# ruotianluo/ImageCaptioning.pytorch

Hardware: NVIDIA H100
Metric: captions/sec at beam=5 seq_len=20 (higher is better)
Workload: dtype f32 (fp32-grade: split-fp16 x3 tensor-core passes, fp32 accumulate)

## Files before the change

imagecaptioning.pytorch_b200/csrc/aoa_engine.cu:

```cuda
#include <vector>

#include "../../include/capb200.h"
#include "common.cuh"
#include "engine_common.cuh"
#include "kernels.cuh"
#include "train_common.cuh"

using namespace capb200;

namespace capb200 {
__global__ void capb_add_vec_kernel(const float* a, const float* b, float* o, int n) {
    const int i = blockIdx.x * blockDim.x + threadIdx.x;
    if (i < n) o[i] = a[i] + b[i];
}
__global__ void capb_interleave_gates_kernel(const float* src, float* dst, int H) {
    const int i = blockIdx.x * blockDim.x + threadIdx.x;
    if (i < 4 * H) dst[i] = src[(i & 3) * H + (i >> 2)];
}
}

struct capb200_aoa_engine {
    capb200_aoa_cfg cfg{};
    capb200_aoa_weights w{};
    int V1 = 0, E = 0, H = 0, heads = 0, dk = 0, F = 0, T = 0, mode = 0;
// ... 377 lines not shown
    {
        const long ldE = round_up(E, 8);
        char* tmp = nullptr;
        const size_t tmp_bytes = (size_t)V1 * ldE * (sizeof(float) + (e->tc ? 2 * sizeof(__half) : 0)) + 1024;
        CAPB_CHECK_CUDA(cudaMallocAsync(&tmp, tmp_bytes, st));
        CAPB_CHECK_CUDA(cudaMemsetAsync(tmp, 0, tmp_bytes, st));
        ActView ev;
        ev.ld = ldE;
        ev.f = reinterpret_cast<float*>(tmp);
        if (e->tc) { ev.hi = reinterpret_cast<__half*>(tmp + (size_t)V1 * ldE * sizeof(float)); ev.lo = ev.hi + (size_t)V1 * ldE; }
        int rc = 0;
        if (ldE == E) rc = relu_copy_launch(w->embed, (long)V1 * E, ev, st);
        else {
            for (int v = 0; v < V1 && !rc; ++v) {
                ActView rv = ev;
                rv.f += (long)v * ldE; if (rv.hi) { rv.hi += (long)v * ldE; rv.lo += (long)v * ldE; }
                rc = relu_copy_launch(w->embed + (long)v * E, E, rv, st);
            }
        }
        GemmProblem g;
        g.M = V1; g.N = 4 * H; g.nseg = 1;
        g.seg[0] = seg_of(ev, w->att_lstm_w_ih, E + H, e->p_ih_x, E);
        g.epi.C = e->xgate; g.epi.ldc = e->ld_xgate;
        if (!rc) {
            if (!e->tc) rc = gemm_simt_launch(g, st);
            else {
                GemmTcPlan* plan = gemm_tc_plan_create(g, e->mode == CAPB200_MODE_TC_F16X3 ? 3 : 1);
                rc = plan ? gemm_tc_plan_launch(plan, nullptr, 0, st) : 1;
                if (plan) gemm_tc_plan_destroy(plan);
            }
        }
        e->launches += 2;
        cudaFreeAsync(tmp, st);
        if (rc) return 1;
    }
    if (e->tc && !e->bound) {
        CAPB_CHECK_CUDA(cudaStreamSynchronize(st));
        CAPB_CHECK_RANGE();
    }
    e->bound = true;
    return 0;
}

int capb200_aoa_decode_beam(capb200_aoa_engine* e, const float* att, const float* mask, int B, int R, const capb200_beam_opts* opts, long long* seq,
                            float* seq_logprobs, long long* done_seq, int* done_len, float* done_p, float* done_raw, void* stream) {
    if (check_ready(e)) return 1;
    cudaStream_t st = static_cast<cudaStream_t>(stream);
    CAPB_REQUIRE(opts != nullptr && att != nullptr && seq != nullptr && B >= 1 && R >= 1, "bad argument");
    const int beam = opts->beam_size, keep = opts->sample_n;
    CAPB_REQUIRE(beam >= 1 && beam <= 16 && beam <= e->V1, "beam_size must be in 1..16 and <= V+1");
    CAPB_REQUIRE(keep == 1 || keep == beam, "sample_n must be 1 or beam_size (AttModel.py:223)");
    if (aoa_decode_workspace(e, B, B * beam, R, beam, st)) return 1;
    if (aoa_decode_prepare(e, att, mask, B, R, st)) return 1;
    auto core = [&](int nrows, int live, const int* tokens, const int* src_row, int , float* logits, long ld) {
        return aoa_decode_core(e, nrows, live, tokens, src_row, logits, ld, R, mask, st);
    };
    return beam_decode_driver(e->d, e->V1, e->T, B, beam, keep, opts->penalty_kind, opts->penalty_alpha, seq, seq_logprobs, done_seq, done_len, done_p,
                              done_raw, core, &e->launches, st, loop_graph_key(e->ws, e->wblock, mask, R, 9), to_edits(opts->edits), opts->temperature);
}

int capb200_aoa_decode_beam_diverse(capb200_aoa_engine* e, const float* att, const float* mask, int B, int R, const capb200_diverse_opts* opts,
                                    long long* seq, float* seq_logprobs, long long* done_seq, int* done_len, float* done_p, float* done_raw, void* stream) {
    if (check_ready(e)) return 1;
    cudaStream_t st = static_cast<cudaStream_t>(stream);
    CAPB_REQUIRE(opts != nullptr && att != nullptr && seq != nullptr && B >= 1 && R >= 1, "bad argument");
    if (opts->group_size == 1) return capb200_aoa_decode_beam(e, att, mask, B, R, &opts->base, seq, seq_logprobs, done_seq, done_len, done_p, done_raw, stream);
    const int beam = opts->base.beam_size;
    CAPB_REQUIRE(beam >= 2 && beam <= 16 && beam <= e->V1, "beam_size must be in 2..16 and <= V+1");
    if (aoa_decode_workspace(e, B, B * beam, R, beam, st)) return 1;
    if (aoa_decode_prepare(e, att, mask, B, R, st)) return 1;
    auto core = [&](int nrows, int rpi, const int* tokens, const int* src_row, int , float* logits, long ld) {
        return aoa_decode_core(e, nrows, rpi, tokens, src_row, logits, ld, R, mask, st);
    };
    return diverse_beam_decode_driver(e->d, e->V1, e->T, B, beam, opts->group_size, opts->diversity_lambda, opts->base.sample_n, opts->base.penalty_kind,
                                      opts->base.penalty_alpha, seq, seq_logprobs, done_seq, done_len, done_p, done_raw, core, &e->launches, st,
                                      loop_graph_key(e->ws, e->wblock, mask, R, 9), to_edits(opts->base.edits), opts->base.temperature);
}

int capb200_aoa_beam_record_logprobs(capb200_aoa_engine* e, int image, int rank, float* dst, void* stream) {
    if (check_ready(e)) return 1;
    return beam_record_logprobs(e->d, e->V1, e->T, image, rank, dst, static_cast<cudaStream_t>(stream));
}

int capb200_aoa_decode_sample(capb200_aoa_engine* e, const float* att, const float* mask, int B, int R, const capb200_sample_opts* opts,
                              const long long* tokens_in, long ld_tok, long long* seq, float* seq_logprobs, float* picked, void* stream) {
    if (check_ready(e)) return 1;
    cudaStream_t st = static_cast<cudaStream_t>(stream);
    CAPB_REQUIRE(opts != nullptr && att != nullptr && seq_logprobs != nullptr && B >= 1 && R >= 1, "bad argument");
    const int n = opts->sample_n, method = opts->method;
    CAPB_REQUIRE(n >= 1 && method >= 0 && method <= 5, "bad sampling options");
    if (method == CAPB200_SAMPLE_FORCED || method == CAPB200_SAMPLE_TEACHER) CAPB_REQUIRE(tokens_in != nullptr && ld_tok >= 1, "token matrix required");
    if (method != CAPB200_SAMPLE_TEACHER) CAPB_REQUIRE(seq != nullptr, "seq output required");
    if (method == CAPB200_SAMPLE_MULTINOMIAL) CAPB_REQUIRE(opts->temperature > 0.f, "temperature must be positive");
    const int rows = B * n;
    const int steps = (method == CAPB200_SAMPLE_TEACHER) ? opts->steps : e->T;
    const long t_out = (method == CAPB200_SAMPLE_TEACHER) ? ld_tok : e->T;
    CAPB_REQUIRE(steps >= 0 && steps <= t_out, "steps out of range");
    if (aoa_decode_workspace(e, B, rows, R, 1, st)) return 1;
    if (aoa_decode_prepare(e, att, mask, B, R, st)) return 1;
    auto core = [&](int nrows, int , const int* tokens, const int* src_row, int , float* logits, long ld) {
        return aoa_decode_core(e, nrows, n, tokens, src_row, logits, ld, R, mask, st);
    };
    return sample_decode_driver(e->d, e->V1, e->T, rows, method, opts->temperature, opts->seed, steps, tokens_in, ld_tok, seq, seq_logprobs, picked,
                                core, &e->launches, st, to_edits(opts->edits), opts->top);
}

}
// ... 252 lines not shown
```

imagecaptioning.pytorch_b200/csrc/beam.cu:

```cuda
#include "common.cuh"
#include "kernels.cuh"

namespace capb200 {

namespace {

constexpr int MAXB = 16;

__device__ __forceinline__ double apply_penalty(int kind, float alpha, int length, double p) {
    if (kind == 1) return p / (pow(5.0 + length, (double)alpha) / pow(6.0, (double)alpha));
    if (kind == 2) return p / (double)length;
    return p;
}

__device__ __forceinline__ void select_step(const BeamState& s, int img, int t, int live, int kl, int row0, int hist0, const float* __restrict__ top_val,
                                            const int* __restrict__ top_idx, const int* pen, int n_pen, float lambda, int penalty_kind,
                                            float penalty_alpha, double* __restrict__ done_p) {
    const int lane = threadIdx.x;
    const int b = s.beam, T = s.T;
    const int ncand = live * kl;
    float cv[8];
    int cf[8];
#pragma unroll
    for (int u = 0; u < 8; ++u) {
        const int c = lane + 32 * u;
        cv[u] = -INFINITY;
        cf[u] = 0x7fffffff;
        if (c < ncand) {
            const int pb = c / kl, k = c % kl;
            const long row = (long)row0 + pb;
            const int w = top_idx[row * kl + k];
            float v = top_val[row * kl + k];
            int cnt = 0;
            for (int q = 0; q < n_pen; ++q) cnt += (pen[q] == w);
            if (cnt) v = __fsub_rn(v, __fmul_rn((float)cnt, lambda));
            cv[u] = s.sums[(long)img * b + pb] + v;
            cf[u] = pb * s.V1 + w;
        }
    }
    const int* seq_old = (t & 1) ? s.seq_b : s.seq_a;
    int* seq_new = (t & 1) ? s.seq_a : s.seq_b;
    const int* hist_old = (t & 1) ? s.hist_b : s.hist_a;
    int* hist_new = (t & 1) ? s.hist_a : s.hist_b;

    float my_v = -INFINITY;
    int my_f = 0;
    for (int j = 0; j < b; ++j) {
        float bv = -INFINITY;
        int bf = 0x7fffffff, bu = -1;
#pragma unroll
        for (int u = 0; u < 8; ++u)
            if (cv[u] > bv || (cv[u] == bv && cf[u] < bf)) { bv = cv[u]; bf = cf[u]; bu = u; }
        float wv = bv;
        int wf = bf;
// ... 6 lines not shown
        if (bu >= 0 && bf == wf && bv == wv) {
#pragma unroll
            for (int u = 0; u < 8; ++u) if (u == bu) { cv[u] = -INFINITY; cf[u] = 0x7fffffff; }
        }
        if (lane == j) { my_v = wv; my_f = wf; }
    }
    __shared__ int sh_parent[MAXB], sh_word[MAXB], sh_slot[MAXB];
    const bool has = lane < b;
    const int parent = has ? my_f / s.V1 : 0;
    const int word = has ? my_f % s.V1 : 0;
    const bool ended = has && ((word == 0) || (t == T - 1));
    const unsigned em = __ballot_sync(0xffffffffu, ended);
    const int cnt0 = s.done_cnt[img];
    const int slot = cnt0 + __popc(em & ((1u << lane) - 1u));
    if (has) { sh_parent[lane] = parent; sh_word[lane] = word; sh_slot[lane] = ended ? slot : -1; }
    __syncwarp();
    for (int idx = lane; idx < b * t; idx += 32) {
        const int j = idx / t, q = idx - j * t;
        const long dst = ((long)img * b + j) * T, src = ((long)img * b + sh_parent[j]) * T;
        seq_new[dst + q] = seq_old[src + q];
        hist_new[dst + q] = hist_old[src + q];
    }
    if (em != 0u) {
        for (int idx = lane; idx < b * (t + 1); idx += 32) {
            const int j = idx / (t + 1), q = idx - j * (t + 1);
            if (sh_slot[j] < 0) continue;
            const long rec = ((long)img * b * T + sh_slot[j]) * T, src = ((long)img * b + sh_parent[j]) * T;
            s.done_seq[rec + q] = (q < t) ? seq_old[src + q] : sh_word[j];
            s.done_hist[rec + q] = (q < t) ? hist_old[src + q] : hist0 + sh_parent[j];
        }
    }
    if (has) {
        const long dst = ((long)img * b + lane) * T;
        seq_new[dst + t] = word;
        hist_new[dst + t] = hist0 + parent;
        float new_sum = my_v;
        if (ended) {
            const long rec = (long)img * b * T + slot;
            s.done_len[rec] = t + 1;
            s.done_raw[rec] = new_sum;
            done_p[rec] = apply_penalty(penalty_kind, penalty_alpha, t + 1, (double)new_sum);
            new_sum -= 1000.0f;
        }
        s.sums[(long)img * b + lane] = new_sum;
        s.tokens[(long)img * b + lane] = word;
        s.src_row[(long)img * b + lane] = row0 + parent;
    }
    if (lane == 0 && em != 0u) s.done_cnt[img] = cnt0 + __popc(em);
}

__global__ void __launch_bounds__(32) beam_step_kernel(BeamState s, int t, int live, const float* __restrict__ top_val,
                                                       const int* __restrict__ top_idx, int penalty_kind, float penalty_alpha,
                                                       double* __restrict__ done_p) {
    const int img = blockIdx.x;
    select_step(s, img, t, live, s.beam, img * live, img * live, top_val, top_idx, nullptr, 0, 0.f, penalty_kind, penalty_alpha, done_p);
}

__global__ void __launch_bounds__(32) diverse_beam_step_kernel(BeamState s, int G, int t, int k, const float* __restrict__ top_val,
                                                               const int* __restrict__ top_idx, float lambda, int rows_total, int penalty_kind,
                                                               float penalty_alpha, double* __restrict__ done_p) {
    const int i = blockIdx.x, lane = threadIdx.x;
    const int b = s.beam, T = s.T;
    __shared__ int sh_pen[MAXB];
    for (int g = 0; g < G && g <= t; ++g) {
        const int lt = t - g;
        if (lt >= T) continue;
        const int n_pen = g * b;
        __syncwarp();
        if (lane < n_pen) {
            const int pg = lane / b, j = lane - pg * b;
            const int last = min(t - pg, T - 1);
            const int* seq_pg = (last & 1) ? s.seq_a : s.seq_b;
            sh_pen[lane] = seq_pg[((long)(i * G + pg) * b + j) * T + lt];
        }
        __syncwarp();
        const int vimg = i * G + g;
        select_step(s, vimg, lt, lt == 0 ? 1 : b, k, vimg * b, g * rows_total + vimg * b, top_val, top_idx, sh_pen, n_pen, lambda, penalty_kind,
                    penalty_alpha, done_p);
    }
}

__global__ void __launch_bounds__(32) beam_finalize_kernel(BeamState s, int keep, const double* __restrict__ done_p, long long* __restrict__ out_seq,
                                                           int* __restrict__ out_len, float* __restrict__ out_p, float* __restrict__ out_raw,
                                                           int* __restrict__ out_hist) {
    const int img = blockIdx.x, lane = threadIdx.x;
    const int b = s.beam, T = s.T;
    const int cnt = s.done_cnt[img];
    const long base = (long)img * b * T;
    __shared__ unsigned char taken[MAXB * 64];
    for (int i = lane; i < cnt; i += 32) taken[i] = 0;
    __syncwarp();
    for (int k = 0; k < keep; ++k) {
        double bv = -INFINITY;
        int bi = 0x7fffffff;
        for (int i = lane; i < cnt; i += 32) {
            if (!taken[i]) {
                const double v = done_p[base + i];
                if (v > bv || (v == bv && i < bi)) { bv = v; bi = i; }
            }
        }
#pragma unroll
        for (int o = 16; o > 0; o >>= 1) {
            const double ov = __shfl_xor_sync(0xffffffffu, bv, o);
            const int oi = __shfl_xor_sync(0xffffffffu, bi, o);
            if (ov > bv || (ov == bv && oi < bi)) { bv = ov; bi = oi; }
        }
// ... 93 lines not shown
        if (vec4) {
            const float4* s4 = reinterpret_cast<const float4*>(src);
            float4* d4 = reinterpret_cast<float4*>(d);
            for (int v = threadIdx.x; v < V1 / 4; v += blockDim.x) {
                const float4 x = __ldg(s4 + v);
                float4 o;
                o.x = (x.x - mx) - lsum; o.y = (x.y - mx) - lsum; o.z = (x.z - mx) - lsum; o.w = (x.w - mx) - lsum;
                if (twice) { o.x = (o.x - m2) - l2; o.y = (o.y - m2) - l2; o.z = (o.z - m2) - l2; o.w = (o.w - m2) - l2; }
                d4[v] = o;
            }
        } else {
            for (int v = threadIdx.x; v < V1; v += blockDim.x) {
                const float lp = (src[v] - mx) - lsum;
                d[v] = twice ? (lp - m2) - l2 : lp;
            }
        }
        apply_edits();
        return;
    }
    const bool vec = ((V1 & 3) == 0) && ((ld_slab & 3) == 0) && ((step_stride & 3) == 0) && ((reinterpret_cast<uintptr_t>(slab) & 15) == 0) &&
                     ((reinterpret_cast<uintptr_t>(dst) & 15) == 0);
    if (vec) {
        const float4* s4 = reinterpret_cast<const float4*>(src);
        float4* d4 = reinterpret_cast<float4*>(d);
        for (int v = threadIdx.x; v < V1 / 4; v += blockDim.x) d4[v] = __ldg(s4 + v);
    } else {
        for (int v = threadIdx.x; v < V1; v += blockDim.x) d[v] = src[v];
    }
    apply_edits();
}

}

int beam_edit_launch(int rows, int k_in, int beam, int t, const DecodeEdits& ed, const int* prev_tokens, const float* val_in, const int* idx_in,
                     float* val_out, int* idx_out, cudaStream_t stream, int first_beam, int first_group_rows, int first_group) {
    CAPB_REQUIRE(k_in >= beam && k_in <= MAXB, "beam_size + number of active decode edits must be <= 16");
    if (rows <= 0) return 0;
    beam_edit_kernel<<<cdiv(rows, 128), 128, 0, stream>>>(rows, k_in, beam, t, ed, prev_tokens, val_in, idx_in, val_out, idx_out, first_beam,
                                                          first_group_rows, first_group);
    CAPB_CHECK_CUDA(cudaGetLastError());
    return 0;
}

int scale_rows_launch(float* x, long ld, int rows, int cols, float factor, cudaStream_t stream, int skip_beam, int skip_group_rows, int skip_group) {
    if (rows <= 0 || cols <= 0) return 0;
    long blocks = ((long)rows * cols + 255) / 256;
    if (blocks > sm_count() * 16) blocks = sm_count() * 16;
    scale_rows_kernel<<<(int)blocks, 256, 0, stream>>>(x, ld, rows, cols, factor, skip_beam, skip_group_rows, skip_group);
    CAPB_CHECK_CUDA(cudaGetLastError());
    return 0;
}

int beam_step_launch(const BeamState& s, int t, int live, const float* top_val, const int* top_idx, int penalty_kind, float penalty_alpha,
                     cudaStream_t stream) {
    CAPB_REQUIRE(s.beam >= 1 && s.beam <= MAXB, "beam size 1..16");
    CAPB_REQUIRE(s.beam * s.T <= MAXB * 64, "beam*T record capacity");
    beam_step_kernel<<<s.B, 32, 0, stream>>>(s, t, live, top_val, top_idx, penalty_kind, penalty_alpha, s.done_p);
    CAPB_CHECK_CUDA(cudaGetLastError());
    return 0;
}

int diverse_beam_step_launch(const BeamState& s, int G, int t, int k, const float* top_val, const int* top_idx, float lambda, int rows_total,
                             int penalty_kind, float penalty_alpha, cudaStream_t stream) {
    CAPB_REQUIRE(G >= 2 && s.beam >= 1 && G * s.beam <= MAXB, "group_size * beams per group must be in 2..16");
    CAPB_REQUIRE(k >= s.beam && k <= MAXB && s.beam * k <= 256, "candidate list width");
    CAPB_REQUIRE(s.beam * s.T <= MAXB * 64, "beam*T record capacity");
    CAPB_REQUIRE(lambda >= 0.f, "diversity_lambda must be >= 0 (the candidate lists rely on the penalty only lowering values)");
    diverse_beam_step_kernel<<<s.B / G, 32, 0, stream>>>(s, G, t, k, top_val, top_idx, lambda, rows_total, penalty_kind, penalty_alpha, s.done_p);
    CAPB_CHECK_CUDA(cudaGetLastError());
    return 0;
}

int beam_finalize_launch(const BeamState& s, int keep, long long* out_seq, int* out_len, float* out_p, float* out_raw, int* out_hist,
                         cudaStream_t stream) {
    CAPB_REQUIRE(keep >= 1 && keep <= s.beam, "keep must be in 1..beam");
    beam_finalize_kernel<<<s.B, 32, 0, stream>>>(s, keep, s.done_p, out_seq, out_len, out_p, out_raw, out_hist);
    CAPB_CHECK_CUDA(cudaGetLastError());
    return 0;
}

int gather_logprob_rows_launch(const float* slab, long step_stride, long ld_slab, const int* hist, int nseq, int T, int V1, float* dst,
                               const float2* stats, long stats_stride, cudaStream_t stream, const long long* seqs, const DecodeEdits* ed) {
    if (nseq <= 0) return 0;
    gather_rows_kernel<<<nseq * T, 256, 0, stream>>>(slab, step_stride, ld_slab, hist, T, V1, dst, stats, stats_stride, seqs, ed ? *ed : DecodeEdits());
    CAPB_CHECK_CUDA(cudaGetLastError());
    return 0;
}

}
```

imagecaptioning.pytorch_b200/csrc/common.cuh:

```cuda
#pragma once
#include <atomic>
#include <cstdint>
#include <cstdio>
#include <cstring>
#include <string>
#include <cuda.h>
#include <cuda_fp16.h>
#include <cuda_runtime.h>

namespace capb200 {

void set_error(const std::string& msg);
#define CAPB_CHECK_CUDA(expr)                                                                          \
    do {                                                                                               \
        cudaError_t _e = (expr);                                                                       \
        if (_e != cudaSuccess) {                                                                       \
            capb200::set_error(std::string(#expr) + " failed: " + cudaGetErrorString(_e) + " at " +    \
                               __FILE__ + ":" + std::to_string(__LINE__));                            \
            return 1;                                                                                  \
        }                                                                                              \
    } while (0)
#define CAPB_REQUIRE(cond, msg)                                                                        \
    do {                                                                                               \
        if (!(cond)) {                                                                                 \
            capb200::set_error(std::string("requirement failed: ") + #cond + " -- " + (msg));          \
            return 1;                                                                                  \
        }                                                                                              \
    } while (0)

inline int cdiv(int a, int b) { return (a + b - 1) / b; }
inline long round_up(long a, long b) { return (a + b - 1) / b * b; }

inline bool first_use_on_device(std::atomic<unsigned long long>& mask) {
    int dev = 0;
    if (cudaGetDevice(&dev) != cudaSuccess || dev < 0 || dev > 63) return true;
    const unsigned long long bit = 1ull << dev;
    return (mask.fetch_or(bit) & bit) == 0;
}

inline int sm_count() {
    static std::atomic<int> cache[64];
    int dev = 0;
    if (cudaGetDevice(&dev) != cudaSuccess || dev < 0 || dev > 63) dev = 0;
    int n = cache[dev].load();
    if (n == 0) {
        if (cudaDeviceGetAttribute(&n, cudaDevAttrMultiProcessorCount, dev) != cudaSuccess || n < 1) n = 132;
        cache[dev].store(n);
    }
    return n;
}

__device__ __forceinline__ void split_f32(float x, __half& hi, __half& lo) {
    hi = __float2half_rn(x);
    lo = __float2half_rn(x - __half2float(hi));
}

constexpr int kMaxSeg = 3;
struct GemmSeg {
    const float* A = nullptr;
    long lda = 0;
    const float* W = nullptr;
    long ldw = 0;
    const __half* A_hi = nullptr;
    const __half* A_lo = nullptr;
    long lda_h = 0;
    const __half* W_hi = nullptr;
    const __half* W_lo = nullptr;
    long ldw_h = 0;
    int K = 0;
};
struct GemmEpilogue {
    const float* bias = nullptr;
    const float* row_bias = nullptr;
    long ld_row_bias = 0;
    int rows_per_group = 1;
    const float* residual = nullptr;
    long ld_res = 0;
    int relu = 0;
    float* C = nullptr;
    long ldc = 0;
    __half* C_hi = nullptr;
    __half* C_lo = nullptr;
    long ldcs = 0;
    int lstm = 0;
    int H = 0;
    const float* c_prev = nullptr;
    long ld_cprev = 0;
    const int* src_row = nullptr;
    float* c_out = nullptr;
    long ld_cout = 0;
    const float* gather_bias = nullptr;
    long ld_gb = 0;
    const int* gather_idx = nullptr;
    float* h_f = nullptr;
    __half* h_hi = nullptr;
    __half* h_lo = nullptr;
    long ld_h = 0;
    unsigned long long* trace = nullptr;
};

__device__ __forceinline__ float fast_sigmoid(float x) { return __fdividef(1.0f, 1.0f + __expf(-x)); }
__device__ __forceinline__ float fast_tanh(float x) {
    const float e = __expf(2.0f * x);
    return 1.0f - __fdividef(2.0f, 1.0f + e);
}
__device__ __forceinline__ void fast_tanh4(const float (&x)[4], float (&t)[4]) {
    float y[4];
#pragma unroll
    for (int i = 0; i < 4; ++i) y[i] = 1.0f + __expf(fminf(2.0f * x[i], 20.0f));
    const float p01 = y[0] * y[1], p23 = y[2] * y[3];
    const float r = __fdividef(1.0f, p01 * p23);
    const float r01 = r * p23, r23 = r * p01;
    t[0] = fmaf(-2.0f, r01 * y[1], 1.0f);
    t[1] = fmaf(-2.0f, r01 * y[0], 1.0f);
    t[2] = fmaf(-2.0f, r23 * y[3], 1.0f);
    t[3] = fmaf(-2.0f, r23 * y[2], 1.0f);
}
struct GemmProblem {
    int M = 0, N = 0, nseg = 0;
    GemmSeg seg[kMaxSeg];
    GemmEpilogue epi;
};

enum NumericMode : int {
    kModeSimtFp32 = 0,
    kModeTcF16x3 = 1,
    kModeTcF16x1 = 2,
};

int gemm_simt_launch(const GemmProblem& p, cudaStream_t stream);

struct GemmTcPlan;
GemmTcPlan* gemm_tc_plan_create(const GemmProblem& p, int passes);
int gemm_tc_tile_n(int M, int N);
int gemm_tc_tile_m(int M, int N, int bn);
void gemm_tc_plan_destroy(GemmTcPlan* plan);
int gemm_tc_plan_launch(GemmTcPlan* plan, const GemmEpilogue* epi_override, int M_override, cudaStream_t stream);
bool gemm_tc_supported(const GemmProblem& p, std::string* why);

int split_planes_launch(const float* x, long ldx, int rows, int cols, __half* hi, __half* lo, long ldh, cudaStream_t stream);
int* range_flag_ptr();
int range_flag_read(int reset);
#define CAPB_CHECK_RANGE()                                                                                              \
    do {                                                                                                                \
        if (capb200::range_flag_read(0)) {                                                                              \
            capb200::set_error("a value with |x| >= 65504 (or inf/nan) reached a split-fp16 conversion in an earlier call: results of the "   \
                               "tensor-core modes are invalid for such inputs/weights (DESIGN.md section 3); capb200_range_status(1) clears the flag"); \
            return 1;                                                                                                   \
        }                                                                                                               \
    } while (0)
int split_planes_interleave_launch(const float* x, long ldx, int H, int cols, __half* hi, __half* lo, long ldh, cudaStream_t stream);

}
```

imagecaptioning.pytorch_b200/csrc/engine.cu:

```cuda
#include <map>
#include <mutex>
#include <vector>

#include "../../include/capb200.h"
#include "common.cuh"
#include "kernels.cuh"
#include "engine_common.cuh"
#include "train_common.cuh"

namespace capb200 {

static thread_local std::string g_last_error;
void set_error(const std::string& msg) { g_last_error = msg; }
const char* last_error_cstr() { return g_last_error.c_str(); }

__global__ void capb_fill_int_kernel(int* p, int n, int v) {
    const int i = blockIdx.x * blockDim.x + threadIdx.x;
    if (i < n) p[i] = v;
}
__global__ void capb_load_token_column_kernel(const long long* src, long ld, int col, int n, int* dst) {
    const int i = blockIdx.x * blockDim.x + threadIdx.x;
    if (i < n) dst[i] = (int)src[(long)i * ld + col];
}
__global__ void capb_store_token_column_kernel(const int* src, int n, long long* dst, long ld, int col) {
// ... 159 lines not shown
    const bool attn = attends(e);
    const bool tc = e->tc;
    if (tc) {
        e->in_fc = carve_planes(a, B, e->cfg.fc_feat_size);
        if (attn) e->in_att = carve_planes(a, (long)B * R, e->cfg.att_feat_size);
    }
    e->fc_e.carve(a, B, updown ? H : E, tc);
    if (attn) {
        e->att_e.carve(a, (long)B * R, H, tc);
        e->p_att.carve(a, (long)B * R, A, false);
        e->att_res.carve(a, rows, H, tc);
        e->att_h.carve(a, rows, A, false);
    }
    if (updown) {
        e->g_fc.carve(a, B, 4 * H, false);
        e->h1_in.carve(a, rows, H, tc);
        e->h1_out.carve(a, rows, H, tc);
    }
    e->xt.carve(a, rows, E, tc);
    e->h0_in.carve(a, rows, H, tc);
    e->h0_out.carve(a, rows, H, tc);
    e->gates.carve(a, rows, 5 * H, false);
    e->ld_c = round_up(H, 8);
    for (int i = 0; i < 2; ++i) {
        e->c0[i] = a.take<float>((long)rows * e->ld_c);
        e->c1[i] = a.take<float>((long)rows * e->ld_c);
    }
    e->img_of_row = a.take<int>(rows);
    e->att_score = a.take<float>((long)rows * (R > 0 ? R : 1));
    e->d.carve(a, B, rows, beam, T);
}

int ensure_workspace(capb200_engine* e, int B, int rows, int R, int beam, cudaStream_t st) {
    if (B <= e->capB && rows <= e->capRows && R <= e->capR && beam <= e->capBeam && e->ws != nullptr) return 0;
    const int nB = B > e->capB ? B : e->capB, nRows = rows > e->capRows ? rows : e->capRows;
    const int nR = R > e->capR ? R : e->capR, nBeam = beam > e->capBeam ? beam : e->capBeam;
    Arena dry;
    layout_workspace(e, dry, nB, nRows, nR, nBeam);
    const size_t need = dry.off + 256;
    CAPB_CHECK_CUDA(cudaStreamSynchronize(st));
    destroy_plans(e);
    if (e->ws) CAPB_CHECK_CUDA(cudaFree(e->ws));
    e->ws = nullptr;
    CAPB_CHECK_CUDA(cudaMalloc(&e->ws, need));
    e->ws_bytes = need;
    Arena real;
    real.base = e->ws;
    layout_workspace(e, real, nB, nRows, nR, nBeam);
    e->capB = nB; e->capRows = nRows; e->capR = nR; e->capBeam = nBeam;
    CAPB_CHECK_CUDA(cudaMemsetAsync(e->ws, 0, need, st));
    return fill_int_launch(e->d.neg1, nRows, -1, st);
}

int run_gemm_inner(capb200_engine* e, int id, GemmProblem& g, int plan_rows, cudaStream_t st) {
    e->launches++;
    if (!e->tc) return gemm_simt_launch(g, st);
    if (e->plans[id] == nullptr) {
        GemmProblem planned = g;
        planned.M = plan_rows;
        e->plans[id] = gemm_tc_plan_create(planned, e->mode == CAPB200_MODE_TC_F16X3 ? 3 : 1);
        if (e->plans[id] == nullptr) return 1;
    }
    return gemm_tc_plan_launch(e->plans[id], &g.epi, g.M, st);
}

int run_gemm(capb200_engine* e, int id, GemmProblem& g, int plan_rows, cudaStream_t st) {
    if (!e->profiling) return run_gemm_inner(e, id, g, plan_rows, st);
    if (e->ev_used + 2 > e->ev_pool.size()) {
        for (int i = 0; i < 64; ++i) {
            cudaEvent_t ev;
            CAPB_CHECK_CUDA(cudaEventCreate(&ev));
            e->ev_pool.push_back(ev);
        }
    }
    double k_total = 0;
    for (int s = 0; s < g.nseg; ++s) k_total += g.seg[s].K;
    CAPB_CHECK_CUDA(cudaEventRecord(e->ev_pool[e->ev_used], st));
    const int rc = run_gemm_inner(e, id, g, plan_rows, st);
    CAPB_CHECK_CUDA(cudaEventRecord(e->ev_pool[e->ev_used + 1], st));
    e->ev_used += 2;
    e->ev_ids.push_back(id);
    e->ev_flops.push_back(2.0 * g.M * g.N * k_total);
    return rc;
}

int prepare(capb200_engine* e, const float* fc, const float* att, const float* mask, int B, int R, cudaStream_t st) {
    CAPB_NVTX("capb200 prepare_feature (fc_embed, att_embed, ctx2att)");
    const int H = e->H, E = e->E, A = e->A;
    const bool updown = e->cfg.family == CAPB200_FAMILY_UPDOWN;
    const capb200_weights& w = e->w;
    ActView fc_in;  fc_in.f = const_cast<float*>(fc);  fc_in.ld = e->cfg.fc_feat_size;
    if (e->tc && e->cfg.family != CAPB200_FAMILY_ATT2IN2) {
        e->launches++;
        if (split_planes_launch(fc, e->cfg.fc_feat_size, B, e->cfg.fc_feat_size, e->in_fc.hi, e->in_fc.lo, e->in_fc.ld, st)) return 1;
    }
    if (e->cfg.family != CAPB200_FAMILY_ATT2IN2) {
        GemmProblem g;
        g.M = B; g.N = updown ? H : E; g.nseg = 1;
        g.seg[0] = seg_of(fc_in, w.fc_embed_w, e->cfg.fc_feat_size, e->p_fc, e->cfg.fc_feat_size);
        g.seg[0].A_hi = e->in_fc.hi; g.seg[0].A_lo = e->in_fc.lo; g.seg[0].lda_h = e->in_fc.ld;
        g.epi.bias = w.fc_embed_b; g.epi.relu = updown ? 1 : 0;
        g.epi.C = e->fc_e.v.f; g.epi.ldc = e->fc_e.v.ld; g.epi.C_hi = e->fc_e.v.hi; g.epi.C_lo = e->fc_e.v.lo; g.epi.ldcs = e->fc_e.v.ld;
        if (run_gemm(e, G_FC, g, e->capB, st)) return 1;
    }
    if (!attends(e)) return 0;
    ActView att_in; att_in.f = const_cast<float*>(att); att_in.ld = e->cfg.att_feat_size;
    if (e->tc) {
        e->launches++;
        if (split_planes_launch(att, e->cfg.att_feat_size, B * R, e->cfg.att_feat_size, e->in_att.hi, e->in_att.lo, e->in_att.ld, st)) return 1;
    }
    {
        GemmProblem g;
        g.M = B * R; g.N = H; g.nseg = 1;
        g.seg[0] = seg_of(att_in, w.att_embed_w, e->cfg.att_feat_size, e->p_attw, e->cfg.att_feat_size);
        g.seg[0].A_hi = e->in_att.hi; g.seg[0].A_lo = e->in_att.lo; g.seg[0].lda_h = e->in_att.ld;
        g.epi.bias = w.att_embed_b; g.epi.relu = 1;
        g.epi.C = e->att_e.v.f; g.epi.ldc = e->att_e.v.ld; g.epi.C_hi = e->att_e.v.hi; g.epi.C_lo = e->att_e.v.lo; g.epi.ldcs = e->att_e.v.ld;
        if (run_gemm(e, G_ATT, g, e->capB * e->capR, st)) return 1;
    }
    if (mask != nullptr) {
        e->launches++;
        if (mask_rows_launch(e->att_e.v, B, R, H, mask, R, st)) return 1;
    }
    {
        GemmProblem g;
        g.M = B * R; g.N = A; g.nseg = 1;
        g.seg[0] = seg_of(e->att_e.v, w.ctx2att_w, H, e->p_ctx, H);
        g.epi.bias = w.ctx2att_b;
        g.epi.C = e->p_att.v.f; g.epi.ldc = e->p_att.v.ld;
        if (run_gemm(e, G_CTX, g, e->capB * e->capR, st)) return 1;
    }
    if (!updown) return 0;
    {
        GemmProblem g;
        g.M = B; g.N = 4 * H; g.nseg = 1;
        g.seg[0] = seg_of(e->fc_e.v, w.att_lstm_w_ih + H, E + 2 * H, e->p_a_ih_fc, H);
        g.epi.bias = e->tc ? e->bsum_att_il : e->bsum_att;
        g.epi.C = e->g_fc.v.f; g.epi.ldc = e->g_fc.v.ld;
        if (run_gemm(e, G_GFC, g, e->capB, st)) return 1;
    }
    return 0;
}

int core_step(capb200_engine* e, int rows, int rpi, const int* tokens, const int* src_row, float* logits, long ld_logits, int n_images, int R,
              const float* mask, cudaStream_t st) {
    const int H = e->H, E = e->E, A = e->A, V1 = e->V1;
    const capb200_weights& w = e->w;
    if (e->cfg.family == CAPB200_FAMILY_UPDOWN) {
        StateCopy s0, s1;
        s0.src = e->h0_out.v.f; s0.ld_src = e->h0_out.v.ld; s0.dst = e->h0_in.v;
        s1.src = e->h1_out.v.f; s1.ld_src = e->h1_out.v.ld; s1.dst = e->h1_in.v;
        const bool xg = e->use_xgate;
        e->launches++;
        if (state_gather_embed_launch(rows, tokens, src_row, w.embed, E, xg ? 0 : E, 1, e->xt.v, H, 2, s0, s1, st)) return 1;
        const int cur = e->core_cur, nxt = cur ^ 1;
        {
            GemmProblem g;
            g.M = rows; g.N = 4 * H;
            g.seg[0] = seg_of(e->h1_in.v, w.att_lstm_w_ih, E + 2 * H, e->p_a_ih_h, H);
            g.seg[1] = seg_of(e->h0_in.v, w.att_lstm_w_hh, H, e->p_a_hh, H);
            g.nseg = 2;
            if (!xg) { g.seg[2] = seg_of(e->xt.v, w.att_lstm_w_ih + 2 * H, E + 2 * H, e->p_a_ih_x, E); g.nseg = 3; }
            g.epi.row_bias = e->g_fc.v.f; g.epi.ld_row_bias = e->g_fc.v.ld; g.epi.rows_per_group = rpi;
            if (e->tc) {
                g.epi.lstm = 1; g.epi.H = H;
                g.epi.c_prev = e->c0[cur]; g.epi.ld_cprev = e->ld_c; g.epi.src_row = src_row;
                g.epi.c_out = e->c0[nxt]; g.epi.ld_cout = e->ld_c;
                g.epi.gather_bias = xg ? e->xgate : nullptr; g.epi.ld_gb = e->ld_xgate; g.epi.gather_idx = tokens;
                g.epi.h_f = e->h0_out.v.f; g.epi.h_hi = e->h0_out.v.hi; g.epi.h_lo = e->h0_out.v.lo; g.epi.ld_h = e->h0_out.v.ld;
            } else {
                g.epi.C = e->gates.v.f; g.epi.ldc = e->gates.v.ld;
            }
            if (run_gemm(e, G_LSTM1, g, e->capRows, st)) return 1;
        }
        if (!e->tc) {
            e->launches++;
            if (lstm_pointwise_launch(rows, H, e->gates.v.f, e->gates.v.ld, src_row, e->c0[cur], e->ld_c, e->c0[nxt], e->ld_c, e->h0_out.v,
                                      xg ? e->xgate : nullptr, e->ld_xgate, tokens, st)) return 1;
        }
        {
            GemmProblem g;
            g.M = rows; g.N = A; g.nseg = 1;
            g.seg[0] = seg_of(e->h0_out.v, w.h2att_w, H, e->p_h2att, H);
            g.epi.bias = w.h2att_b;
            g.epi.C = e->att_h.v.f; g.epi.ldc = e->att_h.v.ld;
            if (run_gemm(e, G_H2ATT, g, e->capRows, st)) return 1;
        }
        const bool split = e->split_lang && e->tc && e->side != nullptr;
        if (split) {
            CAPB_CHECK_CUDA(cudaEventRecord(e->ev_fork, st));
            CAPB_CHECK_CUDA(cudaStreamWaitEvent(e->side, e->ev_fork, 0));
            GemmProblem g;
            g.M = rows; g.N = 4 * H; g.nseg = 2;
            g.seg[0] = seg_of(e->h0_out.v, w.lang_lstm_w_ih + H, 2 * H, e->p_l_ih_h, H);
            g.seg[1] = seg_of(e->h1_in.v, w.lang_lstm_w_hh, H, e->p_l_hh, H);
            g.epi.bias = e->bsum_lang_il;
            g.epi.C = e->gates.v.f; g.epi.ldc = e->gates.v.ld;
            if (run_gemm(e, G_LSTM2A, g, e->capRows, e->side)) return 1;
            CAPB_CHECK_CUDA(cudaEventRecord(e->ev_join, e->side));
        }
        e->launches += 2;
        if (additive_attention_launch(n_images, rpi, R, A, H, e->att_h.v.f, e->att_h.v.ld, e->p_att.v.f, e->p_att.v.ld, e->att_e.v.f, e->att_e.v.ld,
                                      mask, R, w.alpha_w, w.alpha_b, e->att_score, e->att_res.v, st)) return 1;
        if (split) {
            CAPB_CHECK_CUDA(cudaStreamWaitEvent(st, e->ev_join, 0));
            GemmProblem g;
            g.M = rows; g.N = 4 * H; g.nseg = 1;
            g.seg[0] = seg_of(e->att_res.v, w.lang_lstm_w_ih, 2 * H, e->p_l_ih_a, H);
            g.epi.residual = e->gates.v.f; g.epi.ld_res = e->gates.v.ld;
            g.epi.lstm = 1; g.epi.H = H;
            g.epi.c_prev = e->c1[cur]; g.epi.ld_cprev = e->ld_c; g.epi.src_row = src_row;
            g.epi.c_out = e->c1[nxt]; g.epi.ld_cout = e->ld_c;
            g.epi.h_f = e->h1_out.v.f; g.epi.h_hi = e->h1_out.v.hi; g.epi.h_lo = e->h1_out.v.lo; g.epi.ld_h = e->h1_out.v.ld;
            if (run_gemm(e, G_LSTM2B, g, e->capRows, st)) return 1;
        } else {
            GemmProblem g;
            g.M = rows; g.N = 4 * H; g.nseg = 3;
            g.seg[0] = seg_of(e->att_res.v, w.lang_lstm_w_ih, 2 * H, e->p_l_ih_a, H);
            g.seg[1] = seg_of(e->h0_out.v, w.lang_lstm_w_ih + H, 2 * H, e->p_l_ih_h, H);
            g.seg[2] = seg_of(e->h1_in.v, w.lang_lstm_w_hh, H, e->p_l_hh, H);
            if (e->tc) {
                g.epi.bias = e->bsum_lang_il;
                g.epi.lstm = 1; g.epi.H = H;
                g.epi.c_prev = e->c1[cur]; g.epi.ld_cprev = e->ld_c; g.epi.src_row = src_row;
                g.epi.c_out = e->c1[nxt]; g.epi.ld_cout = e->ld_c;
                g.epi.h_f = e->h1_out.v.f; g.epi.h_hi = e->h1_out.v.hi; g.epi.h_lo = e->h1_out.v.lo; g.epi.ld_h = e->h1_out.v.ld;
            } else {
                g.epi.bias = e->bsum_lang;
                g.epi.C = e->gates.v.f; g.epi.ldc = e->gates.v.ld;
            }
            if (run_gemm(e, G_LSTM2, g, e->capRows, st)) return 1;
        }
        if (!e->tc) {
            e->launches++;
            if (lstm_pointwise_launch(rows, H, e->gates.v.f, e->gates.v.ld, src_row, e->c1[cur], e->ld_c, e->c1[nxt], e->ld_c, e->h1_out.v,
                                      nullptr, 0, nullptr, st)) return 1;
        }
        e->core_cur = nxt;
        {
            GemmProblem g;
            g.M = rows; g.N = V1; g.nseg = 1;
            g.seg[0] = seg_of(e->h1_out.v, w.logit_w, H, e->p_logit, H);
            g.epi.bias = w.logit_b;
            g.epi.C = logits; g.epi.ldc = ld_logits;
            if (run_gemm(e, G_LOGIT, g, e->capRows, st)) return 1;
        }
        return 0;
    }
    if (e->cfg.family == CAPB200_FAMILY_ATT2IN2) {
        StateCopy s0, s1;
        s0.src = e->h0_out.v.f; s0.ld_src = e->h0_out.v.ld; s0.dst = e->h0_in.v;
        e->launches++;
        if (state_gather_embed_launch(rows, tokens, src_row, w.embed, E, E, 1, e->xt.v, H, 1, s0, s1, st)) return 1;
        const int cur = e->core_cur, nxt = cur ^ 1;
        {
            GemmProblem g;
            g.M = rows; g.N = A; g.nseg = 1;
            g.seg[0] = seg_of(e->h0_in.v, w.h2att_w, H, e->p_h2att, H);
            g.epi.bias = w.h2att_b;
            g.epi.C = e->att_h.v.f; g.epi.ldc = e->att_h.v.ld;
            if (run_gemm(e, G_H2ATT, g, e->capRows, st)) return 1;
        }
        e->launches += 2;
        if (additive_attention_launch(n_images, rpi, R, A, H, e->att_h.v.f, e->att_h.v.ld, e->p_att.v.f, e->p_att.v.ld, e->att_e.v.f, e->att_e.v.ld,
                                      mask, R, w.alpha_w, w.alpha_b, e->att_score, e->att_res.v, st)) return 1;
        {
            GemmProblem g;
            g.M = rows; g.N = 5 * H; g.nseg = 2;
            g.seg[0] = seg_of(e->xt.v, w.i2h_w, E, e->p_i2h, E);
            g.seg[1] = seg_of(e->h0_in.v, w.h2h_w, H, e->p_h2h, H);
            g.epi.bias = e->bsum_core;
            g.epi.C = e->gates.v.f; g.epi.ldc = e->gates.v.ld;
            if (run_gemm(e, G_CORE, g, e->capRows, st)) return 1;
        }
        {
            GemmProblem g;
            g.M = rows; g.N = 2 * H; g.nseg = 1;
            g.seg[0] = seg_of(e->att_res.v, w.a2c_w, H, e->p_a2c, H);
            g.epi.residual = e->gates.v.f + 3 * H; g.epi.ld_res = e->gates.v.ld;
            g.epi.C = e->gates.v.f + 3 * H; g.epi.ldc = e->gates.v.ld;
            if (run_gemm(e, G_A2C, g, e->capRows, st)) return 1;
        }
        e->launches++;
        if (maxout_pointwise_launch(rows, H, e->gates.v.f, e->gates.v.ld, src_row, e->c0[cur], e->ld_c, e->c0[nxt], e->ld_c, e->h0_out.v, st)) return 1;
        e->core_cur = nxt;
        GemmProblem g;
        g.M = rows; g.N = V1; g.nseg = 1;
        g.seg[0] = seg_of(e->h0_out.v, w.logit_w, H, e->p_logit, H);
        g.epi.bias = w.logit_b;
        g.epi.C = logits; g.epi.ldc = ld_logits;
        return run_gemm(e, G_LOGIT, g, e->capRows, st);
    }
    const bool fresh = (src_row == e->d.neg1);
    for (int pass = fresh ? 0 : 1; pass < 2; ++pass) {
        StateCopy s0, s1;
        s0.src = e->h0_out.v.f; s0.ld_src = e->h0_out.v.ld; s0.dst = e->h0_in.v;
        const int* srcs = (pass == 0) ? e->d.neg1 : (fresh ? nullptr : src_row);
        e->launches++;
// ... 8 lines not shown
        g.seg[0] = seg_of(e->xt.v, w.i2h_w, E, e->p_i2h, E);
        g.seg[1] = seg_of(e->h0_in.v, w.h2h_w, H, e->p_h2h, H);
        g.epi.bias = e->bsum_core;
        g.epi.C = e->gates.v.f; g.epi.ldc = e->gates.v.ld;
        if (run_gemm(e, G_CORE, g, e->capRows, st)) return 1;
        e->launches++;
        if (maxout_pointwise_launch(rows, H, e->gates.v.f, e->gates.v.ld, srcs, e->c0[cur], e->ld_c, e->c0[nxt], e->ld_c, e->h0_out.v, st)) return 1;
        e->core_cur = nxt;
    }
    GemmProblem g;
    g.M = rows; g.N = V1; g.nseg = 1;
    g.seg[0] = seg_of(e->h0_out.v, w.logit_w, H, e->p_logit, H);
    g.epi.bias = w.logit_b;
    g.epi.C = logits; g.epi.ldc = ld_logits;
    return run_gemm(e, G_LOGIT, g, e->capRows, st);
}

int check_ready(capb200_engine* e) {
    CAPB_REQUIRE(e != nullptr, "null engine");
    CAPB_REQUIRE(e->bound, "capb200_engine_bind_weights has not been called");
    CAPB_CHECK_RANGE();
    return 0;
}

}

namespace capb200 {

int lstm_member_info(capb200_engine* e, MemberInfo* m) {
    if (check_ready(e)) return 1;
    m->family = e->cfg.family;
    m->V1 = e->V1; m->T = e->T;
    m->attends = attends(e);
    m->graph_ok = !e->profiling;
    m->ws = e->ws; m->wblock = e->wblock;
    m->fresh = e->d.neg1;
    m->launches = &e->launches;
    return 0;
}

int lstm_decode_workspace(capb200_engine* e, int B, int rows, int R, int beam, int rows_per_image, cudaStream_t st) {
    if (ensure_workspace(e, B, rows, R, beam, st)) return 1;
    if (!attends(e)) { iota_div_kernel<<<cdiv(rows, 256), 256, 0, st>>>(e->img_of_row, rows, rows_per_image); e->launches++; }
    return 0;
}

int lstm_decode_prepare(capb200_engine* e, const float* fc, const float* att, const float* mask, int B, int R, cudaStream_t st) {
    if (prepare(e, fc, att, mask, B, R, st)) return 1;
    e->core_cur = 0;
    return 0;
}

int lstm_decode_core(capb200_engine* e, int rows, int rpi, const int* tokens, const int* src_row, float* logits, long ld, int B, int R,
                     const float* mask, cudaStream_t st) {
    return core_step(e, rows, rpi, tokens, src_row, logits, ld, B, R, mask, st);
}

}

extern "C" {

const char* capb200_last_error(void) { return g_last_error.c_str(); }
int capb200_abi_version(void) { return CAPB200_ABI_VERSION; }
int capb200_range_status(int reset) { return range_flag_read(reset); }

capb200_engine* capb200_engine_create(const capb200_model_cfg* cfg) {
    if (cfg == nullptr) { set_error("null cfg"); return nullptr; }
    if (cfg->family != CAPB200_FAMILY_UPDOWN && cfg->family != CAPB200_FAMILY_NEWFC && cfg->family != CAPB200_FAMILY_ATT2IN2) {
        set_error("unknown model family");
        return nullptr;
    }
    if (cfg->numeric_mode < 0 || cfg->numeric_mode > 2) { set_error("unknown numeric mode"); return nullptr; }
    if (cfg->seq_length < 1 || cfg->seq_length > 64) { set_error("seq_length must be in 1..64"); return nullptr; }
    int ndev = 0;
    if (cudaGetDeviceCount(&ndev) != cudaSuccess || ndev == 0) {
        set_error("no CUDA device: the capb200 engine has no CPU fallback");
        return nullptr;
    }
    capb200_engine* e = new capb200_engine();
    e->cfg = *cfg;
    e->V1 = cfg->vocab_size + 1;
    e->E = cfg->input_encoding_size;
    e->H = cfg->rnn_size;
    e->A = cfg->att_hid_size;
    e->T = cfg->seq_length;
    e->mode = cfg->numeric_mode;
    e->tc = cfg->numeric_mode != CAPB200_MODE_SIMT_FP32;
    if (e->tc && getenv("CAPB200_SPLIT_LANG") != nullptr && atoi(getenv("CAPB200_SPLIT_LANG")) != 0) {
        if (create_side_stream(&e->side) == cudaSuccess &&
            cudaEventCreateWithFlags(&e->ev_fork, cudaEventDisableTiming) == cudaSuccess &&
            cudaEventCreateWithFlags(&e->ev_join, cudaEventDisableTiming) == cudaSuccess) e->split_lang = true;
        else (void)cudaGetLastError();
    }
    return e;
}

void capb200_engine_destroy(capb200_engine* e) {
    if (e == nullptr) return;
    destroy_plans(e);
    for (cudaEvent_t ev : e->ev_pool) cudaEventDestroy(ev);
    cudaFree(e->wblock);
    cudaFree(e->ws);
    e->d.release();
    cudaFree(e->tape);
    e->sg.destroy();
    tf32_context_destroy(e->tf32);
    if (e->ev_fork) cudaEventDestroy(e->ev_fork);
    if (e->ev_join) cudaEventDestroy(e->ev_join);
// ... 124 lines not shown
        }
        int rc = 0;
        if (ldE == E) {
            rc = relu_copy_launch(w->embed, n, ev, st);
        } else {
            CAPB_CHECK_CUDA(cudaMemsetAsync(tmp, 0, tmp_bytes, st));
            for (int v = 0; v < V1 && !rc; ++v) {
                ActView rv = ev;
                rv.f += (long)v * ldE; if (rv.hi) { rv.hi += (long)v * ldE; rv.lo += (long)v * ldE; }
                rc = relu_copy_launch(w->embed + (long)v * E, E, rv, st);
            }
        }
        GemmProblem g;
        g.M = V1; g.N = 4 * H; g.nseg = 1;
        g.seg[0] = seg_of(ev, w->att_lstm_w_ih + 2 * H, E + 2 * H, e->p_a_ih_x, E);
        g.epi.C = e->xgate; g.epi.ldc = e->ld_xgate;
        if (!rc) {
            if (!e->tc) {
                rc = gemm_simt_launch(g, st);
            } else {
                GemmTcPlan* plan = gemm_tc_plan_create(g, e->mode == CAPB200_MODE_TC_F16X3 ? 3 : 1);
                rc = plan ? gemm_tc_plan_launch(plan, nullptr, 0, st) : 1;
                if (plan) gemm_tc_plan_destroy(plan);
            }
        }
        e->launches += 2;
        cudaFreeAsync(tmp, st);
        if (rc) return 1;
    }
    if (e->tc && !e->bound) {
        CAPB_CHECK_CUDA(cudaStreamSynchronize(st));
        CAPB_CHECK_RANGE();
    }
    e->bound = true;
    return 0;
}

int capb200_decode_beam(capb200_engine* e, const float* fc, const float* att, const float* mask, int B, int R, const capb200_beam_opts* opts,
                        long long* seq, float* seq_logprobs, long long* done_seq, int* done_len, float* done_p, float* done_raw, void* stream) {
    if (check_ready(e)) return 1;
    cudaStream_t st = static_cast<cudaStream_t>(stream);
    CAPB_REQUIRE(opts != nullptr && (fc != nullptr || e->cfg.family == CAPB200_FAMILY_ATT2IN2) && seq != nullptr, "null argument");
    const int beam = opts->beam_size, keep = opts->sample_n;
    CAPB_REQUIRE(beam >= 1 && beam <= 16 && beam <= e->V1, "beam_size must be in 1..16 and <= V+1");
    CAPB_REQUIRE(keep == 1 || keep == beam, "sample_n must be 1 or beam_size (AttModel.py:223)");
    CAPB_REQUIRE(B >= 1, "empty batch");
    const bool attn = attends(e);
    if (attn) CAPB_REQUIRE(att != nullptr && R >= 1, "attention features required");
    if (!attn) R = 1;
    const int T = e->T, V1 = e->V1;
    const int rows = B * beam;
    if (lstm_decode_workspace(e, B, rows, R, beam, 1, st)) return 1;
    if (lstm_decode_prepare(e, fc, att, mask, B, R, st)) return 1;
    auto core = [&](int nrows, int live, const int* tokens, const int* src_row, int , float* logits, long ld) {
        return lstm_decode_core(e, nrows, live, tokens, src_row, logits, ld, B, R, mask, st);
    };
    return beam_decode_driver(e->d, V1, T, B, beam, keep, opts->penalty_kind, opts->penalty_alpha, seq, seq_logprobs, done_seq, done_len, done_p,
                              done_raw, core, &e->launches, st, e->profiling ? 0ull : loop_graph_key(e->ws, e->wblock, mask, R, (int)e->cfg.family),
                              to_edits(opts->edits), opts->temperature);
}

int capb200_decode_beam_diverse(capb200_engine* e, const float* fc, const float* att, const float* mask, int B, int R, const capb200_diverse_opts* opts,
                                long long* seq, float* seq_logprobs, long long* done_seq, int* done_len, float* done_p, float* done_raw, void* stream) {
    if (check_ready(e)) return 1;
    cudaStream_t st = static_cast<cudaStream_t>(stream);
    CAPB_REQUIRE(opts != nullptr && (fc != nullptr || e->cfg.family == CAPB200_FAMILY_ATT2IN2) && seq != nullptr, "null argument");
    CAPB_REQUIRE(attends(e), "diverse beam search runs on UpDown and Att2in2 (NewFC's fresh-state pass is chosen per call, not per row)");
    if (opts->group_size == 1) return capb200_decode_beam(e, fc, att, mask, B, R, &opts->base, seq, seq_logprobs, done_seq, done_len, done_p, done_raw, stream);
    const int beam = opts->base.beam_size;
    CAPB_REQUIRE(beam >= 2 && beam <= 16 && beam <= e->V1, "beam_size must be in 2..16 and <= V+1");
    CAPB_REQUIRE(B >= 1, "empty batch");
    CAPB_REQUIRE(att != nullptr && R >= 1, "attention features required");
    const int rows = B * beam;
    if (lstm_decode_workspace(e, B, rows, R, beam, 1, st)) return 1;
    if (lstm_decode_prepare(e, fc, att, mask, B, R, st)) return 1;
    auto core = [&](int nrows, int rpi, const int* tokens, const int* src_row, int , float* logits, long ld) {
        return lstm_decode_core(e, nrows, rpi, tokens, src_row, logits, ld, B, R, mask, st);
    };
    return diverse_beam_decode_driver(e->d, e->V1, e->T, B, beam, opts->group_size, opts->diversity_lambda, opts->base.sample_n, opts->base.penalty_kind,
                                      opts->base.penalty_alpha, seq, seq_logprobs, done_seq, done_len, done_p, done_raw, core, &e->launches, st,
                                      e->profiling ? 0ull : loop_graph_key(e->ws, e->wblock, mask, R, (int)e->cfg.family), to_edits(opts->base.edits),
                                      opts->base.temperature);
}

int capb200_beam_record_logprobs(capb200_engine* e, int image, int rank, float* dst, void* stream) {
    if (check_ready(e)) return 1;
    return beam_record_logprobs(e->d, e->V1, e->T, image, rank, dst, static_cast<cudaStream_t>(stream));
}

int capb200_decode_sample(capb200_engine* e, const float* fc, const float* att, const float* mask, int B, int R, const capb200_sample_opts* opts,
                          const long long* tokens_in, long ld_tok, long long* seq, float* seq_logprobs, float* picked, void* stream) {
    if (check_ready(e)) return 1;
    cudaStream_t st = static_cast<cudaStream_t>(stream);
    CAPB_REQUIRE(opts != nullptr && (fc != nullptr || e->cfg.family == CAPB200_FAMILY_ATT2IN2) && seq_logprobs != nullptr, "null argument");
    const int n = opts->sample_n;
    CAPB_REQUIRE(n >= 1 && B >= 1, "empty batch");
    const bool attn = attends(e);
    if (attn) CAPB_REQUIRE(att != nullptr && R >= 1, "attention features required");
    if (!attn) R = 1;
    const int method = opts->method;
    CAPB_REQUIRE(method >= 0 && method <= 5, "unknown sampling method");
    if (method == CAPB200_SAMPLE_FORCED || method == CAPB200_SAMPLE_TEACHER) CAPB_REQUIRE(tokens_in != nullptr && ld_tok >= 1, "token matrix required");
    if (method != CAPB200_SAMPLE_TEACHER) CAPB_REQUIRE(seq != nullptr, "seq output required");
    if (method == CAPB200_SAMPLE_MULTINOMIAL || method >= CAPB200_SAMPLE_TOPK) CAPB_REQUIRE(opts->temperature > 0.f, "temperature must be positive");
    const int T = e->T, V1 = e->V1;
    const int rows = B * n;
    const int steps = (method == CAPB200_SAMPLE_TEACHER) ? opts->steps : T;
    const long t_out = (method == CAPB200_SAMPLE_TEACHER) ? ld_tok : T;
// ... 815 lines not shown
```

imagecaptioning.pytorch_b200/csrc/engine_common.cuh:

```cuda
#pragma once
#include <cstdio>
#include <cstdlib>
#include <cstring>

#include "../../include/capb200.h"
#include "common.cuh"
#include "kernels.cuh"
#include "nvtx.cuh"

struct capb200_cider_table {
    capb200::CiderTable* t = nullptr;
};

namespace capb200 {

struct Planes {
    __half* hi = nullptr;
    __half* lo = nullptr;
    long ld = 0;
};

struct Arena {
    char* base = nullptr;
    size_t off = 0;
// ... 165 lines not shown
int run_beam_loop(DecodeBuffers& d, const unsigned long long (&key)[8], bool use_graph, long* launches, cudaStream_t st, Loop run_loop) {
    static const bool graphs_off = getenv("CAPB200_NO_GRAPH") != nullptr;
    const bool debug = getenv("CAPB200_GRAPH_DEBUG") != nullptr;
    const bool try_graph = use_graph && !graphs_off && !d.graph_broken;
    if (try_graph && d.loop_exec != nullptr && memcmp(key, d.loop_key, sizeof(key)) == 0) {
        CAPB_CHECK_CUDA(cudaGraphLaunch(d.loop_exec, st));
        *launches += d.loop_launches;
        if (debug) fprintf(stderr, "capb200: beam loop replayed from its CUDA graph\n");
    } else if (try_graph && memcmp(key, d.seen_key, sizeof(key)) == 0) {
        if (d.loop_exec != nullptr) { cudaGraphExecDestroy(d.loop_exec); d.loop_exec = nullptr; }
        const long l0 = *launches;
        cudaGraph_t graph = nullptr;
        bool ok = cudaStreamBeginCapture(st, cudaStreamCaptureModeThreadLocal) == cudaSuccess;
        const int rc = ok ? run_loop() : 1;
        if (ok) ok = cudaStreamEndCapture(st, &graph) == cudaSuccess && graph != nullptr && rc == 0;
        if (ok) ok = cudaGraphInstantiate(&d.loop_exec, graph, 0) == cudaSuccess;
        if (graph != nullptr) cudaGraphDestroy(graph);
        if (!ok) {
            (void)cudaGetLastError();
            d.loop_exec = nullptr;
            d.graph_broken = true;
            *launches = l0;
            if (run_loop()) return 1;
        } else {
            d.loop_launches = *launches - l0;
            memcpy(d.loop_key, key, sizeof(key));
            CAPB_CHECK_CUDA(cudaGraphLaunch(d.loop_exec, st));
            if (debug) fprintf(stderr, "capb200: beam loop captured into a CUDA graph (%ld launches)\n", d.loop_launches);
        }
    } else {
        memcpy(d.seen_key, key, sizeof(key));
        if (run_loop()) return 1;
    }
    return 0;
}

template <class CoreFn>
int beam_decode_driver(DecodeBuffers& d, int V1, int T, int B, int beam, int keep, int penalty_kind, float penalty_alpha, long long* seq,
                       float* seq_logprobs, long long* done_seq, int* done_len, float* done_p, float* done_raw, CoreFn core, long* launches,
                       cudaStream_t st, unsigned long long graph_key = 0, const DecodeEdits& ed = DecodeEdits(), float temperature = 1.0f) {
    const int rows = B * beam;
    const bool edits = ed.any();
    const int k_in = beam + ed.kinds();
    CAPB_REQUIRE(!ed.trigrams, "block_trigrams applies to _sample only (AttModel.py:306)");
    CAPB_REQUIRE(k_in <= 16, "beam_size + number of active decode edits (decoding_constraint, remove_bad_endings, UNK suppression) must be <= 16");
    if (temperature == 0.f) temperature = 1.0f;
    CAPB_REQUIRE(temperature > 0.f, "temperature must be positive");
    if (grow_buffer(reinterpret_cast<void**>(&d.slab), &d.slab_bytes, (size_t)T * rows * V1 * sizeof(float), st)) return 1;
    d.slab_step_stride = (long)rows * V1;
    d.last_B = B;
    d.last_beam = beam;
    BeamState s = d.bs;
    s.B = B; s.beam = beam; s.T = T; s.V1 = V1;
    auto run_loop = [&]() -> int {
        CAPB_NVTX("capb200 beam loop (T steps: core, vocab stats, beam step)");
        CAPB_CHECK_CUDA(cudaMemsetAsync(s.sums, 0, sizeof(float) * B * beam, st));
        CAPB_CHECK_CUDA(cudaMemsetAsync(s.done_cnt, 0, sizeof(int) * B, st));
        CAPB_CHECK_CUDA(cudaMemsetAsync(d.tokens, 0, sizeof(int) * rows, st));
        for (int t = 0; t < T; ++t) {
            const int live = (t == 0) ? 1 : beam;
            const int nrows = B * live;
            float* logits = d.slab + (long)t * d.slab_step_stride;
            if (core(nrows, live, d.tokens, t == 0 ? d.neg1 : d.src_row, t, logits, (long)V1)) return 1;
            if (t > 0 && temperature != 1.0f) {
                if (scale_rows_launch(logits, V1, nrows, V1, 1.0f / temperature, st)) return 1;
                *launches += 1;
            }
            VocabStepArgs va;
            va.rows = nrows; va.V1 = V1; va.logits = logits; va.ld = V1;
            va.twice = (t > 0) ? 1 : 0;
            va.topk = edits ? k_in : beam; va.top_val = d.top_val; va.top_idx = d.top_idx;
            va.stats = d.slab_stats + (long)t * rows;
            if (vocab_step_launch(va, st)) return 1;
            const float* tv = d.top_val;
            const int* ti = d.top_idx;
            if (edits) {
                if (beam_edit_launch(nrows, k_in, beam, t, ed, d.tokens, d.top_val, d.top_idx, d.top_val_e, d.top_idx_e, st)) return 1;
                tv = d.top_val_e; ti = d.top_idx_e;
                *launches += 1;
            }
            if (beam_step_launch(s, t, live, tv, ti, penalty_kind, penalty_alpha, st)) return 1;
            *launches += 2;
        }
        return 0;
    };
    unsigned long long key[8] = {graph_key, (unsigned long long)B, (unsigned long long)beam, (unsigned long long)T, (unsigned long long)V1,
                                 (unsigned long long)penalty_kind, 0ull, (unsigned long long)reinterpret_cast<uintptr_t>(d.slab)};
    memcpy(&key[6], &penalty_alpha, sizeof(float));
    memcpy(reinterpret_cast<char*>(&key[6]) + 4, &temperature, sizeof(float));
    key[5] ^= ((unsigned long long)(ed.constraint & 1) << 8) ^ ((unsigned long long)(unsigned)(ed.unk_col + 1) << 16) ^ ((unsigned long long)ed.n_bad << 48);
    key[0] ^= (unsigned long long)reinterpret_cast<uintptr_t>(ed.bad) * 0x9E3779B97F4A7C15ull;
    d.last_edits = ed;
    d.last_stats = d.slab_stats;
    if (run_beam_loop(d, key, graph_key != 0, launches, st, run_loop)) return 1;
    CAPB_NVTX("capb200 beam finalize + log-prob rows");
    if (beam_finalize_launch(s, beam, d.rec_seq, d.rec_len, d.rec_p, d.rec_raw, d.rec_hist, st)) return 1;
    *launches += 1;
    if (keep == beam) {
        CAPB_CHECK_CUDA(cudaMemcpyAsync(seq, d.rec_seq, sizeof(long long) * B * beam * T, cudaMemcpyDeviceToDevice, st));
        if (seq_logprobs) {
            *launches += 1;
            if (gather_logprob_rows_launch(d.slab, d.slab_step_stride, V1, d.rec_hist, B * beam, T, V1, seq_logprobs, d.slab_stats, rows, st, d.rec_seq, &ed)) return 1;
        }
    } else {
        *launches += 1;
        if (beam_finalize_launch(s, 1, seq, d.tmp_len, d.tmp_p, d.tmp_raw, d.out_hist, st)) return 1;
        if (seq_logprobs) {
            *launches += 1;
            if (gather_logprob_rows_launch(d.slab, d.slab_step_stride, V1, d.out_hist, B, T, V1, seq_logprobs, d.slab_stats, rows, st, seq, &ed)) return 1;
        }
    }
    if (done_seq) CAPB_CHECK_CUDA(cudaMemcpyAsync(done_seq, d.rec_seq, sizeof(long long) * B * beam * T, cudaMemcpyDeviceToDevice, st));
    if (done_len) CAPB_CHECK_CUDA(cudaMemcpyAsync(done_len, d.rec_len, sizeof(int) * B * beam, cudaMemcpyDeviceToDevice, st));
    if (done_p) CAPB_CHECK_CUDA(cudaMemcpyAsync(done_p, d.rec_p, sizeof(float) * B * beam, cudaMemcpyDeviceToDevice, st));
    if (done_raw) CAPB_CHECK_CUDA(cudaMemcpyAsync(done_raw, d.rec_raw, sizeof(float) * B * beam, cudaMemcpyDeviceToDevice, st));
    return 0;
}

template <class CoreFn>
int diverse_beam_decode_driver(DecodeBuffers& d, int V1, int T, int B, int beam, int G, float lambda, int keep, int penalty_kind, float penalty_alpha,
                               long long* seq, float* seq_logprobs, long long* done_seq, int* done_len, float* done_p, float* done_raw, CoreFn core,
                               long* launches, cudaStream_t st, unsigned long long graph_key, const DecodeEdits& ed, float temperature) {
    CAPB_REQUIRE(G >= 2 && beam % G == 0, "diverse beam search needs group_size >= 2 dividing beam_size");
    CAPB_REQUIRE(lambda >= 0.f, "diversity_lambda must be >= 0");
    const int bdash = beam / G, rows = B * beam, steps = T + G - 1;
    CAPB_REQUIRE(keep == 1 || keep == bdash, "sample_n must be 1 or beam_size / group_size (AttModel.py:223)");
    const bool edits = ed.any();
    const int k_in = beam + ed.kinds();
    CAPB_REQUIRE(!ed.trigrams, "block_trigrams applies to _sample only (AttModel.py:306)");
    CAPB_REQUIRE(k_in <= 16, "beam_size + number of active decode edits (decoding_constraint, remove_bad_endings, UNK suppression) must be <= 16");
    if (temperature == 0.f) temperature = 1.0f;
    CAPB_REQUIRE(temperature > 0.f, "temperature must be positive");
    if (grow_buffer(reinterpret_cast<void**>(&d.slab), &d.slab_bytes, (size_t)steps * rows * V1 * sizeof(float), st)) return 1;
    if (grow_buffer(reinterpret_cast<void**>(&d.dbs_stats), &d.dbs_stats_bytes, (size_t)steps * rows * sizeof(float2), st)) return 1;
    if (grow_buffer(reinterpret_cast<void**>(&d.dbs_done_cnt), &d.dbs_done_bytes, (size_t)B * G * sizeof(int), st)) return 1;
    d.slab_step_stride = (long)rows * V1;
    d.last_B = B;
    d.last_beam = beam;
    d.last_edits = ed;
    d.last_stats = d.dbs_stats;
    BeamState s = d.bs;
    s.B = B * G; s.beam = bdash; s.T = T; s.V1 = V1;
// ... 75 lines not shown
                         cudaStream_t st, const DecodeEdits& ed = DecodeEdits(), float top = 0.f) {
    const bool teacher = method == 3, forced = method == 2;
    CAPB_NVTX("capb200 sample / teacher-forcing loop");
    CAPB_REQUIRE(ed.unk_col < 0, "UNK suppression is a beam-search option (CaptionModel.py:159-162)");
    if (method == 4) CAPB_REQUIRE(top >= 1.f, "top-k sampling needs k >= 1");
    if (method == 5) CAPB_REQUIRE(top > 0.f && top < 1.f, "nucleus sampling needs 0 < p < 1");
    const long t_out = teacher ? ld_tok : T;
    CAPB_CHECK_CUDA(cudaMemsetAsync(d.tokens, 0, sizeof(int) * rows, st));
    for (int t = 0; t < steps; ++t) {
        if (teacher) { if (load_token_column_launch(tokens_in, ld_tok, t, rows, d.tokens, st)) return 1; *launches += 1; }
        else if (forced) { if (load_token_column_launch(tokens_in, ld_tok, t, rows, d.forced, st)) return 1; *launches += 1; }
        float* logits = seq_logprobs + (long)t * V1;
        if (core(rows, 0, d.tokens, t == 0 ? d.neg1 : nullptr, t, logits, t_out * V1)) return 1;
        VocabStepArgs va;
        va.rows = rows; va.V1 = V1; va.logits = logits; va.ld = t_out * V1;
        va.twice = 0;
        if (!teacher) {
            va.select = (method == 0) ? 1 : (method == 1 ? 2 : (method == 2 ? 3 : method));
            va.top = top;
            va.edits = ed;
            va.prev_tokens = d.tokens;
            va.temperature = temperature;
            va.seed = seed;
            va.step = (unsigned long long)t;
            va.forced = d.forced;
            va.unfinished = d.unfinished;
            va.first_step = (t == 0);
            va.tokens_out = d.tokens;
            va.seq_out = seq; va.ld_seq = T; va.t = t;
            va.picked_lp = picked ? picked + t : nullptr;
            va.ld_picked = T;
        }
        *launches += 1;
        if (vocab_step_launch(va, st)) return 1;
    }
    return 0;
}

struct MemberInfo {
    int family = 0;
    int V1 = 0, T = 0;
    bool attends = true;
    bool graph_ok = true;
    const void* ws = nullptr;
    const void* wblock = nullptr;
    const int* fresh = nullptr;
    long* launches = nullptr;
};

int lstm_member_info(capb200_engine* e, MemberInfo* m);
int lstm_decode_workspace(capb200_engine* e, int B, int rows, int R, int beam, int rows_per_image, cudaStream_t st);
int lstm_decode_prepare(capb200_engine* e, const float* fc, const float* att, const float* mask, int B, int R, cudaStream_t st);
int lstm_decode_core(capb200_engine* e, int rows, int rpi, const int* tokens, const int* src_row, float* logits, long ld, int B, int R,
                     const float* mask, cudaStream_t st);
int aoa_member_info(capb200_aoa_engine* e, MemberInfo* m);
int aoa_decode_workspace(capb200_aoa_engine* e, int B, int rows, int R, int beam, cudaStream_t st);
int aoa_decode_prepare(capb200_aoa_engine* e, const float* att, const float* mask, int B, int R, cudaStream_t st);
int aoa_decode_core(capb200_aoa_engine* e, int rows, int rpi, const int* tokens, const int* src_row, float* logits, long ld, int R,
                    const float* mask, cudaStream_t st);

struct StepGraph {
    cudaGraphExec_t exec = nullptr;
    unsigned long long key = 0, seen = 0, cap_seed = 0;
    long launches = 0, replays = 0;
    char* stage = nullptr;
    size_t stage_bytes = 0;
    bool broken = false;
    cudaStream_t stream = nullptr;
    cudaEvent_t ev_in = nullptr, ev_out = nullptr;
    cudaStream_t enter(cudaStream_t caller) {
        if (stream == nullptr) {
            if (cudaStreamCreateWithFlags(&stream, cudaStreamNonBlocking) != cudaSuccess || cudaEventCreateWithFlags(&ev_in, cudaEventDisableTiming) != cudaSuccess ||
                cudaEventCreateWithFlags(&ev_out, cudaEventDisableTiming) != cudaSuccess) { (void)cudaGetLastError(); broken = true; return caller; }
        }
        if (cudaEventRecord(ev_in, caller) != cudaSuccess || cudaStreamWaitEvent(stream, ev_in, 0) != cudaSuccess) { (void)cudaGetLastError(); broken = true; return caller; }
        return stream;
    }
    int leave(cudaStream_t caller, cudaStream_t used) {
        if (used == caller) return 0;
        CAPB_CHECK_CUDA(cudaEventRecord(ev_out, used));
        CAPB_CHECK_CUDA(cudaStreamWaitEvent(caller, ev_out, 0));
        return 0;
    }
    static bool enabled() { static const bool v = !(getenv("CAPB200_SCST_GRAPH") != nullptr && atoi(getenv("CAPB200_SCST_GRAPH")) == 0); return v; }
    void reset() { if (exec) cudaGraphExecDestroy(exec); exec = nullptr; key = 0; }
    void destroy() {
        if (getenv("CAPB200_GRAPH_DEBUG") != nullptr && (exec || replays)) fprintf(stderr, "capb200: step graph replayed %ld times\n", replays);
        reset(); if (stage) cudaFree(stage); stage = nullptr; stage_bytes = 0;
        if (ev_in) cudaEventDestroy(ev_in);
        if (ev_out) cudaEventDestroy(ev_out);
        if (stream) cudaStreamDestroy(stream);
        ev_in = ev_out = nullptr; stream = nullptr;
    }
    int stage_inputs(int n, const void* const* src, const size_t* bytes, size_t* off, cudaStream_t st) {
        size_t need = 256;
        for (int i = 0; i < n; ++i) { off[i] = need; need += (bytes[i] + 255) & ~size_t(255); }
        if (need > stage_bytes) {
            CAPB_CHECK_CUDA(cudaStreamSynchronize(st));
            reset();
            if (stage) CAPB_CHECK_CUDA(cudaFree(stage));
            stage = nullptr;
            CAPB_CHECK_CUDA(cudaMalloc(&stage, need));
            stage_bytes = need;
        }
        for (int i = 0; i < n; ++i)
            if (src[i] != nullptr && bytes[i]) CAPB_CHECK_CUDA(cudaMemcpyAsync(stage + off[i], src[i], bytes[i], cudaMemcpyDeviceToDevice, st));
        return 0;
// ... 103 lines not shown
```

imagecaptioning.pytorch_b200/csrc/ensemble.cu:

```cuda
#include <cmath>

#include "../../include/capb200.h"
#include "common.cuh"
#include "engine_common.cuh"
#include "kernels.cuh"

using namespace capb200;

struct capb200_ensemble {
    char* ws = nullptr;
    int capB = 0, capRows = 0, capBeam = 0, capT = 0;
    DecodeBuffers d;
    float* mix = nullptr;
    size_t mix_bytes = 0;
    int V1 = 0, T = 0;
    long launches = 0;
};

namespace capb200 {

constexpr int kMixThreads = 256;

struct MixWeights {
    float w[CAPB200_ENSEMBLE_MAX_MEMBERS];
// ... 162 lines not shown
    return mix_launch(s->mix, member_stride, rows, V1, E.mw, logits, ld, st);
}

unsigned long long graph_key(const capb200_ensemble* s, const Members& E, const float* mask) {
    unsigned long long h = 1469598103934665603ull;
    auto mix = [&](unsigned long long v) { h ^= v; h *= 1099511628211ull; };
    mix(reinterpret_cast<uintptr_t>(s->ws)); mix(reinterpret_cast<uintptr_t>(s->mix)); mix((unsigned long long)E.K);
    for (int k = 0; k < E.K; ++k) {
        const Member& m = E.m[k];
        if (!m.info.graph_ok) return 0;
        unsigned bits = 0;
        memcpy(&bits, &E.mw.w[k], sizeof(float));
        mix(loop_graph_key(m.info.ws, m.info.wblock, mask, m.R, m.family));
        mix((unsigned long long)bits);
    }
    return h | 1ull;
}

}
}

extern "C" {

capb200_ensemble* capb200_ensemble_create(void) { return new capb200_ensemble(); }

void capb200_ensemble_destroy(capb200_ensemble* s) {
    if (s == nullptr) return;
    if (s->ws != nullptr || s->mix != nullptr) {
        s->d.release();
        cudaFree(s->ws);
        cudaFree(s->mix);
    }
    delete s;
}

long capb200_ensemble_launch_count(const capb200_ensemble* s) { return s ? s->launches : 0; }

int capb200_ensemble_decode_beam(capb200_ensemble* s, const capb200_ensemble_member* members, int K, const float* fc, const float* att,
                                 const float* mask, int B, int R, const capb200_beam_opts* opts, long long* seq, float* seq_logprobs,
                                 long long* done_seq, int* done_len, float* done_p, float* done_raw, void* stream) {
    CAPB_REQUIRE(s != nullptr && opts != nullptr && seq != nullptr, "null argument");
    Members E;
    if (resolve(members, K, fc, att, R, E)) return 1;
    cudaStream_t st = static_cast<cudaStream_t>(stream);
    const int V1 = E.m[0].info.V1, T = E.m[0].info.T;
    const int beam = opts->beam_size, keep = opts->sample_n;
    CAPB_REQUIRE(beam >= 1 && beam <= 16 && beam <= V1, "beam_size must be in 1..16 and <= V+1");
    CAPB_REQUIRE(keep == 1 || keep == beam, "sample_n must be 1 or beam_size (AttModel.py:223)");
    CAPB_REQUIRE(B >= 1, "empty batch");
    const int rows = B * beam;
    if (setup(s, E, fc, att, mask, B, rows, beam, 1, st)) return 1;
    s->V1 = V1; s->T = T;
    const long stride = (long)rows * V1;
    auto core = [&](int nrows, int live, const int* tokens, const int* src_row, int , float* logits, long ld) {
        return step(s, E, nrows, live, tokens, src_row, logits, ld, stride, B, mask, st);
    };
    return beam_decode_driver(s->d, V1, T, B, beam, keep, opts->penalty_kind, opts->penalty_alpha, seq, seq_logprobs, done_seq, done_len, done_p,
                              done_raw, core, &s->launches, st, graph_key(s, E, mask), to_edits(opts->edits), opts->temperature);
}

int capb200_ensemble_beam_record_logprobs(capb200_ensemble* s, int image, int rank, float* dst, void* stream) {
    CAPB_REQUIRE(s != nullptr && dst != nullptr, "null argument");
    return beam_record_logprobs(s->d, s->V1, s->T, image, rank, dst, static_cast<cudaStream_t>(stream));
}

int capb200_ensemble_decode_sample(capb200_ensemble* s, const capb200_ensemble_member* members, int K, const float* fc, const float* att,
                                   const float* mask, int B, int R, const capb200_sample_opts* opts, const long long* tokens_in, long ld_tok,
                                   long long* seq, float* seq_logprobs, float* picked, void* stream) {
    CAPB_REQUIRE(s != nullptr && opts != nullptr && seq_logprobs != nullptr, "null argument");
    Members E;
    if (resolve(members, K, fc, att, R, E)) return 1;
    cudaStream_t st = static_cast<cudaStream_t>(stream);
    const int V1 = E.m[0].info.V1, T = E.m[0].info.T;
    const int n = opts->sample_n, method = opts->method;
    CAPB_REQUIRE(n >= 1 && B >= 1, "empty batch");
    CAPB_REQUIRE(method >= 0 && method <= 5, "unknown sampling method");
    if (method == CAPB200_SAMPLE_FORCED || method == CAPB200_SAMPLE_TEACHER) CAPB_REQUIRE(tokens_in != nullptr && ld_tok >= 1, "token matrix required");
    if (method != CAPB200_SAMPLE_TEACHER) CAPB_REQUIRE(seq != nullptr, "seq output required");
    if (method == CAPB200_SAMPLE_MULTINOMIAL || method >= CAPB200_SAMPLE_TOPK) CAPB_REQUIRE(opts->temperature > 0.f, "temperature must be positive");
    const int rows = B * n;
    const int steps = (method == CAPB200_SAMPLE_TEACHER) ? opts->steps : T;
    const long t_out = (method == CAPB200_SAMPLE_TEACHER) ? ld_tok : T;
    CAPB_REQUIRE(steps >= 0 && steps <= t_out, "steps out of range");
    if (setup(s, E, fc, att, mask, B, rows, 1, n, st)) return 1;
    const long stride = (long)rows * V1;
    auto core = [&](int nrows, int , const int* tokens, const int* src_row, int , float* logits, long ld) {
        return step(s, E, nrows, n, tokens, src_row, logits, ld, stride, B, mask, st);
    };
    return sample_decode_driver(s->d, V1, T, rows, method, opts->temperature, opts->seed, steps, tokens_in, ld_tok, seq, seq_logprobs, picked, core,
                                &s->launches, st, to_edits(opts->edits), opts->top);
}

}
```

imagecaptioning.pytorch_b200/csrc/gemm_tc.cu:

```cuda
#include <cstdlib>
#include <cstring>

#include "common.cuh"
#include "ptx.cuh"

namespace capb200 {

namespace {

constexpr int BM = 128;
constexpr int BK = 64;
constexpr int kConsumers = 2;
constexpr int kThreads = 128 * (1 + kConsumers);

struct TcParams {
    CUtensorMap a_hi[kMaxSeg];
    CUtensorMap a_lo[kMaxSeg];
    CUtensorMap w_hi[kMaxSeg];
    CUtensorMap w_lo[kMaxSeg];
    int kblocks[kMaxSeg];
    int nseg;
    int M, N;
    float* C;
    long ldc;
// ... 132 lines not shown
        for (int i = 0; i < BN / 8; ++i) {
            const int du = 8 * (i / 4) + i % 4;
            cp[i] = (cprev != nullptr && u0 + du < p.H) ? cprev[du] : 0.0f;
        }
    }
    if (TRACE && slot >= 0) {
        float s = 0.0f;
#pragma unroll
        for (int i = 0; i < BN / 8; ++i) s += cp[i];
        asm volatile("" ::"f"(s));
        CAPB_TRACE(slot);
    }
    __syncwarp();
#pragma unroll
    for (int j = 0; j < BN / 8; ++j) {
        float* v = acc + 4 * j;
        const float s0 = __shfl_xor_sync(0xffffffffu, odd ? v[0] : v[2], 1);
        const float s1 = __shfl_xor_sync(0xffffffffu, odd ? v[1] : v[3], 1);
        const float gi = odd ? s0 : v[0], gf = odd ? s1 : v[1], gg = odd ? v[2] : s0, go = odd ? v[3] : s1;
        v[0] = gi; v[1] = gf; v[2] = gg; v[3] = go;
    }
#pragma unroll
    for (int k = 0; k < kRuns; ++k) {
#pragma unroll
        for (int t = 0; t < 2; ++t) {
            float* x = acc + 4 * (4 * k + t);
            float* y = acc + 4 * (4 * k + 2 + t);
#pragma unroll
            for (int g = 0; g < 4; ++g) {
                const float keep = upper ? y[g] : x[g];
                const float recv = __shfl_xor_sync(0xffffffffu, upper ? x[g] : y[g], 2);
                x[g] = upper ? recv : keep;
                y[g] = upper ? keep : recv;
            }
        }
    }
    float cn[BN / 8], hn[BN / 8];
#pragma unroll
    for (int i = 0; i < BN / 8; ++i) {
        const int k = i / 4, o = i % 4;
        const float* g = acc + 4 * (4 * k + (o >> 1) + 2 * (o & 1));
        cn[i] = fast_sigmoid(g[1]) * cp[i] + fast_sigmoid(g[0]) * fast_tanh(g[2]);
        hn[i] = fast_sigmoid(g[3]) * fast_tanh(cn[i]);
    }
    if (TRACE && slot >= 0) {
        float s = 0.0f;
#pragma unroll
        for (int i = 0; i < BN / 8; ++i) s += hn[i];
        asm volatile("" ::"f"(s));
        CAPB_TRACE(slot + 1);
    }
    if (row_ok) {
        float* const c_out = p.c_out + (long)row * p.ld_cout + u0;
        float* const h_f = p.h_f + (long)row * p.ld_h + u0;
        __half* const h_hi = p.h_hi + (long)row * p.ld_h + u0;
        __half* const h_lo = p.h_lo + (long)row * p.ld_h + u0;
        const bool planes = p.h_hi != nullptr;
        const uintptr_t a16 = reinterpret_cast<uintptr_t>(c_out) | reinterpret_cast<uintptr_t>(h_f);
        const uintptr_t a8 = planes ? reinterpret_cast<uintptr_t>(h_hi) | reinterpret_cast<uintptr_t>(h_lo) : 0;
        if (full && (a16 & 15) == 0 && (a8 & 7) == 0) {
#pragma unroll
            for (int k = 0; k < kRuns; ++k) {
                const float* c = cn + 4 * k;
                const float* h = hn + 4 * k;
                *reinterpret_cast<float4*>(c_out + 8 * k) = make_float4(c[0], c[1], c[2], c[3]);
                *reinterpret_cast<float4*>(h_f + 8 * k) = make_float4(h[0], h[1], h[2], h[3]);
                if (planes) {
                    __half hh[4], hl[4];
#pragma unroll
                    for (int o = 0; o < 4; ++o) split_f32(h[o], hh[o], hl[o]);
                    const __half2 hi01 = __halves2half2(hh[0], hh[1]), hi23 = __halves2half2(hh[2], hh[3]);
                    const __half2 lo01 = __halves2half2(hl[0], hl[1]), lo23 = __halves2half2(hl[2], hl[3]);
                    *reinterpret_cast<uint2*>(h_hi + 8 * k) = make_uint2(*reinterpret_cast<const uint32_t*>(&hi01), *reinterpret_cast<const uint32_t*>(&hi23));
                    *reinterpret_cast<uint2*>(h_lo + 8 * k) = make_uint2(*reinterpret_cast<const uint32_t*>(&lo01), *reinterpret_cast<const uint32_t*>(&lo23));
                }
            }
        } else {
#pragma unroll
            for (int i = 0; i < BN / 8; ++i) {
                const int du = 8 * (i / 4) + i % 4;
                if (u0 + du < p.H) {
                    c_out[du] = cn[i];
                    h_f[du] = hn[i];
                    if (planes) {
                        __half hh, hl;
                        split_f32(hn[i], hh, hl);
                        h_hi[du] = hh;
                        h_lo[du] = hl;
                    }
                }
            }
        }
    }
    if (TRACE && slot >= 0) CAPB_TRACE(slot + 2);
}

template <int BN, bool PLANES>
__device__ __forceinline__ void epi_store(const TcParams& p, const float* acc, int r0, int c0) {
    const int ncol = p.N - c0;
#pragma unroll
    for (int h = 0; h < 2; ++h) {
        const int row = r0 + 8 * h;
        if (row >= p.M) continue;
        if (p.C != nullptr) {
            float* const dst = p.C + (long)row * p.ldc + c0;
            if (ncol >= BN && (reinterpret_cast<uintptr_t>(dst) & 7) == 0) {
#pragma unroll
                for (int j = 0; j < BN / 8; ++j) *reinterpret_cast<float2*>(dst + 8 * j) = make_float2(acc[4 * j + 2 * h], acc[4 * j + 2 * h + 1]);
            } else {
#pragma unroll
                for (int j = 0; j < BN / 8; ++j) {
                    if (8 * j < ncol) dst[8 * j] = acc[4 * j + 2 * h];
                    if (8 * j + 1 < ncol) dst[8 * j + 1] = acc[4 * j + 2 * h + 1];
                }
            }
        }
        if (PLANES) {
            __half* const dh = p.C_hi + (long)row * p.ldcs + c0;
            __half* const dl = p.C_lo + (long)row * p.ldcs + c0;
            if (ncol >= BN && ((reinterpret_cast<uintptr_t>(dh) | reinterpret_cast<uintptr_t>(dl)) & 3) == 0) {
#pragma unroll
                for (int j = 0; j < BN / 8; ++j) {
                    __half h0, l0, h1, l1;
                    split_f32(acc[4 * j + 2 * h], h0, l0);
                    split_f32(acc[4 * j + 2 * h + 1], h1, l1);
                    *reinterpret_cast<__half2*>(dh + 8 * j) = __halves2half2(h0, h1);
                    *reinterpret_cast<__half2*>(dl + 8 * j) = __halves2half2(l0, l1);
                }
            } else {
#pragma unroll
                for (int j = 0; j < BN / 8; ++j) {
#pragma unroll
                    for (int e = 0; e < 2; ++e) {
                        __half hi, lo;
                        split_f32(acc[4 * j + 2 * h + e], hi, lo);
                        if (8 * j + e < ncol) { dh[8 * j + e] = hi; dl[8 * j + e] = lo; }
                    }
                }
            }
        }
    }
}

template <int BN, int EPI, bool TRACE>
__device__ __forceinline__ void epilogue_tile(const TcParams& p, float* acc, int m0, int n0, int tid, int slot) {
    const int warp = tid >> 5, lane = tid & 31;
    const int r0 = m0 + warp * 16 + (lane >> 2);
    const int c0 = n0 + 2 * (lane & 3);
    epi_adds<BN>(p, acc, r0, c0);
    if (EPI == kEpiLstm) epi_lstm<BN, TRACE>(p, acc, r0, c0, lane, slot);
    else epi_store<BN, EPI == kEpiPlanes>(p, acc, r0, c0);
}

template <int BN, int EPI, bool TRACE>
__device__ __forceinline__ void epilogue_rows128(const TcParams& p, float* acc0, const float* acc1, int m0, int n0, int tid, int slot) {
#pragma unroll 1
    for (int h = 0; h < 2; ++h) {
        epilogue_tile<BN, EPI, TRACE>(p, acc0, m0 + 64 * h, n0, tid, h == 0 ? slot : -1);
#pragma unroll
        for (int i = 0; i < BN / 2; ++i) acc0[i] = acc1[i];
    }
}

template <int PASSES>
__device__ __forceinline__ void init_ring(const TcParams& p, uint64_t* full_bar, uint64_t* empty_bar, int stages, int readers) {
    for (int s = 0; s < p.nseg; ++s) {
        ptx::prefetch_tmap(&p.a_hi[s]);
        ptx::prefetch_tmap(&p.w_hi[s]);
        if (PASSES == 3) {
            ptx::prefetch_tmap(&p.a_lo[s]);
            ptx::prefetch_tmap(&p.w_lo[s]);
        }
    }
    for (int i = 0; i < stages; ++i) {
        ptx::mbar_init(&full_bar[i], 1);
        ptx::mbar_init(&empty_bar[i], readers);
    }
}

template <typename Cfg>
__device__ __forceinline__ void fill_stage(const TcParams& p, uint8_t* st, uint64_t* bar, int s, int kb, int m0, int n0) {
    uint8_t* a_hi = st;
    uint8_t* a_lo = st + Cfg::kABytes;
    uint8_t* w_hi = st + Cfg::kABytes * Cfg::kPlanes;
    uint8_t* w_lo = w_hi + Cfg::kWBytes;
    ptx::mbar_arrive_expect_tx(bar, Cfg::kStageBytes);
#pragma unroll
    for (int r = 0; r < Cfg::kTileM; r += BM) ptx::tma_load_2d(a_hi + r * BK * 2, &p.a_hi[s], bar, kb * BK, m0 + r);
    ptx::tma_load_2d(w_hi, &p.w_hi[s], bar, kb * BK, n0);
    if (Cfg::kPasses == 3) {
#pragma unroll
        for (int r = 0; r < Cfg::kTileM; r += BM) ptx::tma_load_2d(a_lo + r * BK * 2, &p.a_lo[s], bar, kb * BK, m0 + r);
        ptx::tma_load_2d(w_lo, &p.w_lo[s], bar, kb * BK, n0);
    }
}

template <int BN, int PASSES>
__device__ __forceinline__ void mma_kblock(float* acc0, float* acc1, uint32_t a_hi, uint32_t a_lo, uint32_t w_hi, uint32_t w_lo) {
    constexpr uint32_t kHalf = 64 * 128;
#pragma unroll
    for (int i = 0; i < BN / 2; ++i) { ptx::reg_fence(acc0[i]); ptx::reg_fence(acc1[i]); }
    ptx::wgmma_fence();
#pragma unroll
    for (int k = 0; k < BK / 16; ++k) {
        const uint32_t koff = k * 32;
        const uint64_t dwh = ptx::make_smem_desc_sw128(w_hi + koff);
        if (PASSES == 3) {
            const uint64_t dwl = ptx::make_smem_desc_sw128(w_lo + koff);
            wgmma_f16<BN>(acc0, ptx::make_smem_desc_sw128(a_hi + koff), dwl, 1);
            wgmma_f16<BN>(acc1, ptx::make_smem_desc_sw128(a_hi + kHalf + koff), dwl, 1);
            wgmma_f16<BN>(acc0, ptx::make_smem_desc_sw128(a_lo + koff), dwh, 1);
            wgmma_f16<BN>(acc1, ptx::make_smem_desc_sw128(a_lo + kHalf + koff), dwh, 1);
            wgmma_f16<BN>(acc0, ptx::make_smem_desc_sw128(a_hi + koff), dwh, 1);
            wgmma_f16<BN>(acc1, ptx::make_smem_desc_sw128(a_hi + kHalf + koff), dwh, 1);
        } else {
            wgmma_f16<BN>(acc0, ptx::make_smem_desc_sw128(a_hi + koff), dwh, 1);
            wgmma_f16<BN>(acc1, ptx::make_smem_desc_sw128(a_hi + kHalf + koff), dwh, 1);
        }
    }
    ptx::wgmma_commit();
    ptx::wgmma_wait<0>();
#pragma unroll
    for (int i = 0; i < BN / 2; ++i) { ptx::reg_fence(acc0[i]); ptx::reg_fence(acc1[i]); }
}

template <int BN, int PASSES, int EPI, bool TRACE = false>
__global__ void __launch_bounds__(kThreads, 1) gemm_tc_kernel(const __grid_constant__ TcParams p) {
    using Cfg = TcCfg<BN, PASSES>;
    extern __shared__ uint8_t smem_raw[];
    uint8_t* smem = reinterpret_cast<uint8_t*>((reinterpret_cast<uintptr_t>(smem_raw) + 1023) & ~uintptr_t(1023));
    uint64_t* full_bar = reinterpret_cast<uint64_t*>(smem + Cfg::kStages * Cfg::kStageBytes);
    uint64_t* empty_bar = full_bar + Cfg::kStages;
    uint64_t* turn_bar = empty_bar + Cfg::kStages;

    const int wg = threadIdx.x >> 7;
    const int n_tiles = p.tiles_m * p.tiles_n;

    if (threadIdx.x == 0) {
        init_ring<PASSES>(p, full_bar, empty_bar, Cfg::kStages, 1);
        for (int c = 0; c < kConsumers; ++c) ptx::mbar_init(&turn_bar[c], 1);
        ptx::fence_mbar_init();
    }
    __syncthreads();
    if (threadIdx.x == 0) CAPB_TRACE(0);

    if (wg == 0) {
        ptx::setmaxnreg_dec<40>();
        if (threadIdx.x == 0) {
            int stage = 0;
            uint32_t phase = 0;
            for (int t = blockIdx.x; t < n_tiles; t += gridDim.x) {
                const int m0 = (t % p.tiles_m) * BM;
                const int n0 = (t / p.tiles_m) * BN;
                for (int s = 0; s < p.nseg; ++s) {
                    for (int kb = 0; kb < p.kblocks[s]; ++kb) {
                        ptx::mbar_wait(&empty_bar[stage], phase ^ 1);
                        fill_stage<Cfg>(p, smem + stage * Cfg::kStageBytes, &full_bar[stage], s, kb, m0, n0);
                        if (++stage == Cfg::kStages) { stage = 0; phase ^= 1; }
                    }
                }
            }
        }
    } else {
        ptx::setmaxnreg_inc<232>();
        const int cw = wg - 1;
        const int tid = threadIdx.x & 127;
        int kb_tile = 0;
        for (int s = 0; s < p.nseg; ++s) kb_tile += p.kblocks[s];
        int mine = 0;
        for (int it = cw, t = blockIdx.x + cw * gridDim.x; t < n_tiles; it += 2, t += 2 * gridDim.x, ++mine) {
            const int m0 = (t % p.tiles_m) * BM;
            const int n0 = (t / p.tiles_m) * BN;
            if (it > 0) ptx::mbar_wait(&turn_bar[cw], (cw == 1 ? mine : mine - 1) & 1);
            if (TRACE && it == 1 && tid == 0) CAPB_TRACE(4);
            const long g0 = (long)it * kb_tile;
            int stage = (int)(g0 % Cfg::kStages);
            uint32_t phase = (uint32_t)(g0 / Cfg::kStages) & 1;
            float acc0[BN / 2], acc1[BN / 2];
#pragma unroll
            for (int i = 0; i < BN / 2; ++i) { acc0[i] = 0.0f; acc1[i] = 0.0f; }
            for (int s = 0; s < p.nseg; ++s) {
                for (int kb = 0; kb < p.kblocks[s]; ++kb) {
                    ptx::mbar_wait(&full_bar[stage], phase);
                    if (TRACE && it == 0 && s == 0 && kb == 0 && tid == 0) CAPB_TRACE(1);
                    const uint32_t st = ptx::smem_u32(smem + stage * Cfg::kStageBytes);
                    const uint32_t w_hi = st + Cfg::kABytes * Cfg::kPlanes;
                    mma_kblock<BN, PASSES>(acc0, acc1, st, st + Cfg::kABytes, w_hi, w_hi + Cfg::kWBytes);
                    if (tid == 0) ptx::mbar_arrive(&empty_bar[stage]);
                    if (++stage == Cfg::kStages) { stage = 0; phase ^= 1; }
                }
            }
            if (tid == 0) ptx::mbar_arrive(&turn_bar[cw ^ 1]);
            if (TRACE && it < 2 && tid == 0) CAPB_TRACE(2 + it);
            epilogue_rows128<BN, EPI, TRACE>(p, acc0, acc1, m0, n0, tid, (TRACE && it < 2 && tid == 0) ? 9 + 3 * it : -1);
            if (TRACE && it < 2 && tid == 0) CAPB_TRACE(6 + it);
        }
    }
    __syncthreads();
    if (threadIdx.x == 0) CAPB_TRACE(8);
}

template <int BN, int PASSES, int EPI, bool TRACE = false>
__global__ void __launch_bounds__(kThreads, 1) gemm_tc256_kernel(const __grid_constant__ TcParams p) {
    using Cfg = TcCfg<BN, PASSES, 2 * BM>;
    extern __shared__ uint8_t smem_raw[];
    uint8_t* smem = reinterpret_cast<uint8_t*>((reinterpret_cast<uintptr_t>(smem_raw) + 1023) & ~uintptr_t(1023));
    uint64_t* full_bar = reinterpret_cast<uint64_t*>(smem + Cfg::kStages * Cfg::kStageBytes);
    uint64_t* empty_bar = full_bar + Cfg::kStages;

    const int wg = threadIdx.x >> 7;
    const int n_tiles = p.tiles_m * p.tiles_n;

    if (threadIdx.x == 0) {
        init_ring<PASSES>(p, full_bar, empty_bar, Cfg::kStages, kConsumers);
        ptx::fence_mbar_init();
    }
    __syncthreads();
    if (threadIdx.x == 0) CAPB_TRACE(0);

    if (wg == 0) {
        ptx::setmaxnreg_dec<40>();
        if (threadIdx.x == 0) {
            int stage = 0;
            uint32_t phase = 0;
            for (int t = blockIdx.x; t < n_tiles; t += gridDim.x) {
                const int m0 = (t % p.tiles_m) * Cfg::kTileM;
                const int n0 = (t / p.tiles_m) * BN;
                for (int s = 0; s < p.nseg; ++s) {
                    for (int kb = 0; kb < p.kblocks[s]; ++kb) {
                        ptx::mbar_wait(&empty_bar[stage], phase ^ 1);
                        fill_stage<Cfg>(p, smem + stage * Cfg::kStageBytes, &full_bar[stage], s, kb, m0, n0);
                        if (++stage == Cfg::kStages) { stage = 0; phase ^= 1; }
                    }
                }
                if (TRACE && t == (int)blockIdx.x) CAPB_TRACE(5);
            }
        }
    } else {
        ptx::setmaxnreg_inc<232>();
        const int cw = wg - 1;
        const int tid = threadIdx.x & 127;
        const uint32_t a_rows = cw * BM * BK * 2;
        int stage = 0;
        uint32_t phase = 0;
        for (int it = 0, t = blockIdx.x; t < n_tiles; ++it, t += gridDim.x) {
            const int m0 = (t % p.tiles_m) * Cfg::kTileM + BM * cw;
            const int n0 = (t / p.tiles_m) * BN;
            float acc0[BN / 2], acc1[BN / 2];
#pragma unroll
            for (int i = 0; i < BN / 2; ++i) { acc0[i] = 0.0f; acc1[i] = 0.0f; }
            for (int s = 0; s < p.nseg; ++s) {
                for (int kb = 0; kb < p.kblocks[s]; ++kb) {
                    ptx::mbar_wait(&full_bar[stage], phase);
                    if (TRACE && it == 0 && s == 0 && kb == 0 && cw == 0 && tid == 0) CAPB_TRACE(1);
                    const uint32_t st = ptx::smem_u32(smem + stage * Cfg::kStageBytes);
                    const uint32_t w_hi = st + Cfg::kABytes * Cfg::kPlanes;
                    mma_kblock<BN, PASSES>(acc0, acc1, st + a_rows, st + Cfg::kABytes + a_rows, w_hi, w_hi + Cfg::kWBytes);
                    if (tid == 0) ptx::mbar_arrive(&empty_bar[stage]);
                    if (++stage == Cfg::kStages) { stage = 0; phase ^= 1; }
                }
            }
            if (TRACE && it == 0 && tid == 0) CAPB_TRACE(2 + cw);
            epilogue_rows128<BN, EPI, TRACE>(p, acc0, acc1, m0, n0, tid, (TRACE && it == 0 && tid == 0) ? 9 + 3 * cw : -1);
            if (TRACE && it == 0 && tid == 0) CAPB_TRACE(6 + cw);
        }
    }
    __syncthreads();
    if (threadIdx.x == 0) CAPB_TRACE(8);
}

typedef CUresult (*EncodeTiledFn)(CUtensorMap*, CUtensorMapDataType, cuuint32_t, void*, const cuuint64_t*, const cuuint64_t*,
                                  const cuuint32_t*, const cuuint32_t*, CUtensorMapInterleave, CUtensorMapSwizzle,
                                  CUtensorMapL2promotion, CUtensorMapFloatOOBfill);

EncodeTiledFn get_encode_fn() {
    static EncodeTiledFn fn = nullptr;
    if (fn == nullptr) {
        void* sym = nullptr;
        cudaDriverEntryPointQueryResult qres;
        if (cudaGetDriverEntryPoint("cuTensorMapEncodeTiled", &sym, cudaEnableDefault, &qres) != cudaSuccess || sym == nullptr) {
            return nullptr;
        }
        fn = reinterpret_cast<EncodeTiledFn>(sym);
    }
    return fn;
}

bool encode_plane(CUtensorMap* map, const __half* base, long rows, long K, long pitch, int box_rows, std::string* err) {
    EncodeTiledFn fn = get_encode_fn();
    if (fn == nullptr) { *err = "cuTensorMapEncodeTiled entry point not available"; return false; }
    cuuint64_t gdim[2] = {static_cast<cuuint64_t>(K), static_cast<cuuint64_t>(rows)};
    cuuint64_t gstride[1] = {static_cast<cuuint64_t>(pitch) * 2};
    cuuint32_t box[2] = {static_cast<cuuint32_t>(BK), static_cast<cuuint32_t>(box_rows)};
    cuuint32_t estr[2] = {1, 1};
    CUresult r = fn(map, CU_TENSOR_MAP_DATA_TYPE_FLOAT16, 2, const_cast<__half*>(base), gdim, gstride, box, estr,
                    CU_TENSOR_MAP_INTERLEAVE_NONE, CU_TENSOR_MAP_SWIZZLE_128B, CU_TENSOR_MAP_L2_PROMOTION_L2_256B,
                    CU_TENSOR_MAP_FLOAT_OOB_FILL_NONE);
    if (r != CUDA_SUCCESS) { *err = "cuTensorMapEncodeTiled failed with CUresult " + std::to_string((int)r); return false; }
    return true;
}

template <int BN, int PASSES, int EPI, bool TRACE, int TM>
int launch_cfg(const TcParams& prm, cudaStream_t stream) {
    using Cfg = TcCfg<BN, PASSES, TM>;
    void (*kernel)(TcParams);
    if constexpr (TM == BM) kernel = gemm_tc_kernel<BN, PASSES, EPI, TRACE>;
    else kernel = gemm_tc256_kernel<BN, PASSES, EPI, TRACE>;
    static std::atomic<unsigned long long> attr_set{0};
    if (first_use_on_device(attr_set)) {
        CAPB_CHECK_CUDA(cudaFuncSetAttribute(kernel, cudaFuncAttributeMaxDynamicSharedMemorySize, Cfg::kSmemBytes));
    }
    TcParams prm2 = prm;
    prm2.tiles_n = cdiv(prm.N, BN);
    prm2.tiles_m = cdiv(prm.M, TM);
    const int n_tiles = prm2.tiles_n * prm2.tiles_m;
    const int sms = sm_count();
    kernel<<<n_tiles < sms ? n_tiles : sms, kThreads, Cfg::kSmemBytes, stream>>>(prm2);
    CAPB_CHECK_CUDA(cudaGetLastError());
    return 0;
}

template <int EPI, int TM>
int launch_width(int bn, int passes, const TcParams& prm, cudaStream_t stream) {
    if (prm.trace != nullptr) {
        if (bn == 160) return launch_cfg<160, 3, EPI, true, TM>(prm, stream);
        if constexpr (TM == BM) if (bn == 64) return launch_cfg<64, 3, EPI, true, TM>(prm, stream);
        return launch_cfg<128, 3, EPI, true, TM>(prm, stream);
    }
    if (bn == 160) return passes == 3 ? launch_cfg<160, 3, EPI, false, TM>(prm, stream) : launch_cfg<160, 1, EPI, false, TM>(prm, stream);
    if constexpr (TM == BM) {
        if (bn == 64) return passes == 3 ? launch_cfg<64, 3, EPI, false, TM>(prm, stream) : launch_cfg<64, 1, EPI, false, TM>(prm, stream);
    }
    return passes == 3 ? launch_cfg<128, 3, EPI, false, TM>(prm, stream) : launch_cfg<128, 1, EPI, false, TM>(prm, stream);
}

template <int EPI>
int launch_kind(int bm, int bn, int passes, const TcParams& prm, cudaStream_t stream) {
    return bm == 2 * BM ? launch_width<EPI, 2 * BM>(bn, passes, prm, stream) : launch_width<EPI, BM>(bn, passes, prm, stream);
}

}

struct GemmTcPlan {
    TcParams prm;
    int passes;
    int bn;
};

static void fill_epilogue(TcParams& t, const GemmEpilogue& e) {
    t.C = e.C; t.ldc = e.ldc;
    t.C_hi = e.C_hi; t.C_lo = e.C_lo; t.ldcs = e.ldcs;
    t.bias = e.bias; t.row_bias = e.row_bias; t.ld_row_bias = e.ld_row_bias;
    t.rows_per_group = e.rows_per_group < 1 ? 1 : e.rows_per_group;
    t.relu = e.relu;
    t.residual = e.residual; t.ld_res = e.ld_res;
    t.lstm = e.lstm; t.H = e.H;
    t.c_prev = e.c_prev; t.ld_cprev = e.ld_cprev; t.src_row = e.src_row;
    t.c_out = e.c_out; t.ld_cout = e.ld_cout;
    t.gather_bias = e.gather_bias; t.ld_gb = e.ld_gb; t.gather_idx = e.gather_idx;
    t.h_f = e.h_f; t.h_hi = e.h_hi; t.h_lo = e.h_lo; t.ld_h = e.ld_h;
    t.trace = e.trace;
}

bool gemm_tc_supported(const GemmProblem& p, std::string* why) {
    auto bad = [&](const char* m) { if (why) *why = m; return false; };
    if (p.nseg < 1 || p.nseg > kMaxSeg) return bad("1..3 K-segments");
    for (int s = 0; s < p.nseg; ++s) {
        const GemmSeg& g = p.seg[s];
        if (g.A_hi == nullptr || g.W_hi == nullptr) return bad("split planes missing");
        if ((g.lda_h & 7) || (g.ldw_h & 7)) return bad("plane pitch must be a multiple of 8 elements (16 bytes)");
        if ((reinterpret_cast<uintptr_t>(g.A_hi) & 15) || (reinterpret_cast<uintptr_t>(g.W_hi) & 15)) return bad("plane base must be 16-byte aligned");
        if (g.K < 1) return bad("empty K-segment");
    }
    return true;
}

int gemm_tc_tile_n(int M, int N) {
    const int sms = sm_count();
    const int tiles_m = cdiv(M, BM);
    if (tiles_m * cdiv(N, 128) < sms / 2 && N > 64) return 64;
    const long cost128 = (long)cdiv(tiles_m * cdiv(N, 128), sms) * 128;
    const long cost160 = (long)cdiv(tiles_m * cdiv(N, 160), sms) * 160;
    return cost160 < cost128 ? 160 : 128;
}

int gemm_tc_tile_m(int M, int N, int bn) {
    if (bn == 64) return BM;
    const char* force = getenv("CAPB200_GEMM_BM");
    if (force != nullptr && strcmp(force, "128") == 0) return BM;
    if (force != nullptr && strcmp(force, "256") == 0) return 2 * BM;
    const int sms = sm_count();
    const int tiles_n = cdiv(N, bn);
    return cdiv(M, 2 * BM) * tiles_n <= sms && cdiv(M, BM) * tiles_n > sms ? 2 * BM : BM;
}

GemmTcPlan* gemm_tc_plan_create(const GemmProblem& p, int passes) {
    std::string why;
    if (!gemm_tc_supported(p, &why)) { set_error("gemm_tc: unsupported problem: " + why); return nullptr; }
    if (passes != 1 && passes != 3) { set_error("gemm_tc: passes must be 1 or 3"); return nullptr; }
    GemmTcPlan* plan = new GemmTcPlan();
    memset(&plan->prm, 0, sizeof(TcParams));
    plan->passes = passes;
    plan->bn = gemm_tc_tile_n(p.M, p.N);
    TcParams& t = plan->prm;
    t.nseg = p.nseg;
    t.M = p.M;
    t.N = p.N;
    std::string err;
    for (int s = 0; s < p.nseg; ++s) {
        const GemmSeg& g = p.seg[s];
        t.kblocks[s] = cdiv(g.K, BK);
        bool ok = encode_plane(&t.a_hi[s], g.A_hi, p.M, g.K, g.lda_h, BM, &err) &&
                  encode_plane(&t.w_hi[s], g.W_hi, p.N, g.K, g.ldw_h, plan->bn, &err);
        if (ok && passes == 3) {
            if (g.A_lo == nullptr || g.W_lo == nullptr) { err = "lo planes missing for 3-pass mode"; ok = false; }
            ok = ok && encode_plane(&t.a_lo[s], g.A_lo, p.M, g.K, g.lda_h, BM, &err) &&
                 encode_plane(&t.w_lo[s], g.W_lo, p.N, g.K, g.ldw_h, plan->bn, &err);
        }
        if (!ok) { set_error("gemm_tc: " + err); delete plan; return nullptr; }
    }
    fill_epilogue(t, p.epi);
    return plan;
}

void gemm_tc_plan_destroy(GemmTcPlan* plan) { delete plan; }

int gemm_tc_plan_launch(GemmTcPlan* plan, const GemmEpilogue* epi_override, int M_override, cudaStream_t stream) {
    if (M_override > plan->prm.M) { set_error("gemm_tc: M override exceeds the planned row count"); return 1; }
    const int M = M_override > 0 ? M_override : plan->prm.M;
    TcParams prm = plan->prm;
    if (epi_override != nullptr) fill_epilogue(prm, *epi_override);
    prm.M = M;
    if (prm.lstm && (prm.N != 4 * prm.H || prm.c_out == nullptr || prm.h_f == nullptr)) {
        set_error("gemm_tc: fused LSTM epilogue needs N == 4H, c_out and h_f");
        return 1;
    }
    if (prm.M <= 0 || prm.N <= 0) return 0;
    const int kind = prm.lstm ? kEpiLstm : prm.C_hi != nullptr ? kEpiPlanes : kEpiStore;
    if (prm.trace != nullptr && plan->passes != 3) { set_error("gemm_tc: the traced kernel is the 3-pass one"); return 1; }
    const int bm = gemm_tc_tile_m(prm.M, prm.N, plan->bn);
    if (kind == kEpiLstm) return launch_kind<kEpiLstm>(bm, plan->bn, plan->passes, prm, stream);
    if (kind == kEpiPlanes) return launch_kind<kEpiPlanes>(bm, plan->bn, plan->passes, prm, stream);
    return launch_kind<kEpiStore>(bm, plan->bn, plan->passes, prm, stream);
}

}
```

imagecaptioning.pytorch_b200/csrc/kernels.cuh:

```cuda
#pragma once
#include "common.cuh"

namespace capb200 {

struct ActView {
    float* f = nullptr;
    __half* hi = nullptr;
    __half* lo = nullptr;
    long ld = 0;
};

struct StateCopy {
    const float* src = nullptr;
    long ld_src = 0;
    ActView dst;
};

int state_gather_embed_launch(int rows, const int* tokens, const int* src_row, const float* emb, long ld_emb, int E, int relu,
                              ActView xt, int H, int nstate, StateCopy sc0, StateCopy sc1, cudaStream_t stream);
int lstm_pointwise_launch(int rows, int H, const float* gates, long ld_g, const int* src_row, const float* c_prev, long ld_cp,
                          float* c_out, long ld_co, ActView h_out, const float* gather_bias, long ld_gb, const int* gather_idx,
                          cudaStream_t stream);
int relu_copy_launch(const float* x, long n, ActView out_flat, cudaStream_t stream);
int lstm_ln_launch(int rows, int H, const float* gates, long ld_g, const float* c_prev, long ld_cp, float* c_out, long ld_co, float* h_out, long ld_h,
                   const float* ln_a, const float* ln_b, float eps, float* ln_out, long ld_ln, cudaStream_t stream);
int maxout_pointwise_launch(int rows, int H, const float* sums, long ld_s, const int* src_row, const float* c_prev, long ld_cp,
                            float* c_out, long ld_co, ActView h_out, cudaStream_t stream);
int additive_attention_launch(int n_images, int rpi, int R, int A, int H, const float* att_h, long ld_ah, const float* p_att, long ld_pa,
                              const float* att, long ld_at, const float* mask, long ld_mask, const float* alpha_w, const float* alpha_b,
                              float* score_scratch , ActView out, cudaStream_t stream, float* alpha_out = nullptr );
int mask_rows_launch(ActView x, int n_images, int R, int cols, const float* mask, long ld_mask, cudaStream_t stream);
int ss_select_launch(int rows, int V1, const float* prev_logp, long ld, const long long* labels, long ld_labels, int col, unsigned long long seed, float prob,
                     int* tok_out, cudaStream_t stream);

struct DecodeEdits {
    int constraint = 0;
    int unk_col = -1;
    int n_bad = 0;
    const int* bad = nullptr;
    int trigrams = 0;
    int trigram_rows = 0;
    __host__ __device__ bool any() const { return constraint != 0 || unk_col >= 0 || n_bad > 0 || trigrams != 0; }
    __host__ __device__ int kinds() const { return (constraint ? 1 : 0) + (unk_col >= 0 ? 1 : 0) + (n_bad > 0 ? 1 : 0); }
};

struct VocabStepArgs {
    int rows = 0;
    int V1 = 0;
    float* logits = nullptr;
    long ld = 0;
    int twice = 0;
    float2* stats = nullptr;
    int topk = 0;
    float* top_val = nullptr;
    int* top_idx = nullptr;
    int select = 0;
    float top = 0.f;
    DecodeEdits edits;
    const int* prev_tokens = nullptr;
    float temperature = 1.0f;
    unsigned long long seed = 0;
    unsigned long long step = 0;
    const int* forced = nullptr;
    int* unfinished = nullptr;
    int first_step = 0;
    int* tokens_out = nullptr;
    long long* seq_out = nullptr;
    long ld_seq = 0;
    int t = 0;
    float* picked_lp = nullptr;
    long ld_picked = 1;
    int first_beam = 0, first_group_rows = 1, first_group = -1;
    __host__ __device__ int row_twice(int r) const {
        return twice && !(first_beam > 0 && (r % first_beam) / first_group_rows == first_group);
    }
};
int vocab_step_launch(const VocabStepArgs& a, cudaStream_t stream);
int beam_edit_launch(int rows, int k_in, int beam, int t, const DecodeEdits& ed, const int* prev_tokens, const float* val_in, const int* idx_in,
                     float* val_out, int* idx_out, cudaStream_t stream, int first_beam = 0, int first_group_rows = 1, int first_group = -1);
int scale_rows_launch(float* x, long ld, int rows, int cols, float factor, cudaStream_t stream, int skip_beam = 0, int skip_group_rows = 1,
                      int skip_group = -1);

struct BeamState {
    int B = 0, beam = 0, T = 0, V1 = 0;
    float* sums = nullptr;
    int* seq_a = nullptr;
    int* seq_b = nullptr;
    int* hist_a = nullptr;
    int* hist_b = nullptr;
    int* done_cnt = nullptr;
    int* done_seq = nullptr;
    int* done_hist = nullptr;
    int* done_len = nullptr;
    double* done_p = nullptr;
    float* done_raw = nullptr;
    int* tokens = nullptr;
    int* src_row = nullptr;
};
int beam_step_launch(const BeamState& s, int t, int live, const float* top_val, const int* top_idx, int penalty_kind, float penalty_alpha,
                     cudaStream_t stream);
int diverse_beam_step_launch(const BeamState& s, int G, int t, int k, const float* top_val, const int* top_idx, float lambda, int rows_total,
                             int penalty_kind, float penalty_alpha, cudaStream_t stream);
int beam_finalize_launch(const BeamState& s, int keep, long long* out_seq, int* out_len, float* out_p, float* out_raw, int* out_hist,
                         cudaStream_t stream);
int gather_logprob_rows_launch(const float* slab, long step_stride, long ld_slab, const int* hist, int nseq, int T, int V1, float* dst,
                               const float2* stats, long stats_stride, cudaStream_t stream, const long long* seqs = nullptr,
                               const DecodeEdits* ed = nullptr);

int layer_norm_launch(int rows, int D, const float* x, long ld_x, const float* a, const float* b, float eps, ActView out, cudaStream_t st);
int embed_pe_launch(int rows, int D, const int* tokens, const float* lut, const float* pe_row, float scale, ActView out, cudaStream_t st);
int enc_self_attention_launch(int B, int R, int heads, int dk, const float* q, const float* k, const float* v, long ld, const float* mask,
                              long ld_mask, ActView out, cudaStream_t st);
int dec_self_attention_launch(int rows, int heads, int dk, int t, const float* qkv, long ld_qkv, float* kcache, float* vcache, long step_stride,
                              long ld_c, const int* anc, long ld_anc, const long long* labels, long ld_lab, ActView out, cudaStream_t st);
int cross_attention_launch(int rows, int rpi, int heads, int dk, int R, const float* q, long ld_q, const float* kk, const float* vv, long ld_kv,
                           const float* mask, long ld_mask, ActView out, cudaStream_t st);

int glu_launch(int rows, int H, const float* t, long ld_t, const float* residual, long ld_res, ActView out, cudaStream_t st);
int masked_mean_launch(int B, int R, int H, const float* x, long ld_x, const float* mask, long ld_mask, ActView out, cudaStream_t st);

int gemm_generic_launch(int ta, int tb, int M, int N, int K, const float* A, long lda, const float* B, long ldb, float* C, long ldc, int accumulate,
                        const float* bias, cudaStream_t st);
int gemm_skinny_launch(int M, int N, int nseg, const float* const* A, const long* lda, const float* const* B, const long* ldb, const int* K, const int* tb,
                       float* C, long ldc, const float* bias, const float* row_bias, long ld_rb, int rpg, int accumulate, float* scratch,
                       size_t scratch_floats, int mode, cudaStream_t st);
int gemm_wgrad_launch(int M, int N, int K, const float* dY, long ld_dy, const float* X, long ld_x, float* G, long ld_g, int accumulate, int mode,
                      cudaStream_t st);
int colsum_launch(int rows, int cols, const float* x, long ld, float* out, int accumulate, cudaStream_t st);
struct Tf32Context;
Tf32Context* tf32_context_create();
void tf32_context_destroy(Tf32Context* c);
void tf32_context_new_step(Tf32Context* c);
long tf32_context_launches(const Tf32Context* c);
bool gemm_tf32_supported(int nseg, const float* const* X, const long* ldx, const float* const* W, const long* ldw, const int* K);
int gemm_tf32_launch(Tf32Context* ctx, int M, int N, int nseg, const float* const* X, const long* ldx, const float* const* W, const long* ldw, const int* K,
                     float* C, long ldc, const float* bias, const float* row_bias, long ld_rb, int rpg, int accumulate, cudaStream_t st);
const float* tf32_transposed(Tf32Context* ctx, const float* src, long ld_src, int rows, int cols, bool per_step, long* ld_dst, cudaStream_t st);
int dropout_apply_launch(float* x, int rows, int cols, long ld, unsigned long long seed, unsigned site, unsigned step, float p, cudaStream_t st);
int dropout_mask_launch(float* m, long n, unsigned long long seed, unsigned site, unsigned step, float p, cudaStream_t st);
int dropout_copy_launch(const float* x, long ld_x, float* y, long ld_y, int rows, int cols, unsigned long long seed, unsigned site, unsigned step, float p,
                        cudaStream_t st);
int embed_relu_dropout_launch(int rows, int E, const int* tokens, const float* emb, float* xt, unsigned long long seed, unsigned step, float p,
                              cudaStream_t st);
int scst_dlogits_launch(const float* logp, long ld_row, const long long* seq, const float* reward, const float* mask_sum, float upstream, int N, int T, int V1,
                        float* dl, cudaStream_t st, const float* row_coef = nullptr);
int scst_drop_worst_launch(const long long* seq, const float* row_loss, int N, int T, int keep, float upstream, float* row_msum, float* row_coef, float* loss,
                           cudaStream_t st);
int xe_loss_backward_launch(const float* logp, long ld_row, const long long* labels, long ld_l, const float* masks, long ld_m, int N, int steps, int Ls, int V1,
                            float smoothing, float upstream, float* mask_sum, float* item_loss, float* dl, float* loss, cudaStream_t st, int keep = 0,
                            float* row_loss = nullptr, float* row_msum = nullptr, float* row_coef = nullptr);
int lstm_cell_backward_launch(int rows, int H, const float* gates, const float* c_prev, const float* c_new, const float* dh, const float* dh_extra,
                              long ld_extra, unsigned drop_site, unsigned drop_step, unsigned long long seed, float p, float* dc_carry, float* dgates,
                              cudaStream_t st);
// ... 82 lines not shown
```

imagecaptioning.pytorch_b200/csrc/pointwise.cu:

```cuda
#include "common.cuh"
#include "kernels.cuh"

namespace capb200 {

static int pw_blocks(long total) {
    long b = (total + 255) / 256;
    return (int)(b > sm_count() * 8 ? sm_count() * 8 : b);
}

namespace {

__device__ __forceinline__ float sigmoidf_(float x) { return fast_sigmoid(x); }

__device__ __forceinline__ void store_act(const ActView& o, long row, int col, float v) {
    o.f[row * o.ld + col] = v;
    if (o.hi != nullptr) {
        __half h, l;
        split_f32(v, h, l);
        o.hi[row * o.ld + col] = h;
        o.lo[row * o.ld + col] = l;
    }
}

__global__ void state_gather_embed_kernel(int rows, const int* __restrict__ tokens, const int* __restrict__ src_row,
                                          const float* __restrict__ emb, long ld_emb, int E, int relu, ActView xt,
                                          int H, int nstate, StateCopy sc0, StateCopy sc1) {
    const int r = blockIdx.x;
    if (r >= rows) return;
    const int tok = tokens[r];
    const float* e = emb + (long)tok * ld_emb;
    for (int c = threadIdx.x; c < E; c += blockDim.x) {
        float v = __ldg(e + c);
        if (relu) v = fmaxf(v, 0.f);
        store_act(xt, r, c, v);
    }
    const int src = src_row ? src_row[r] : r;
    const bool vec = (H & 3) == 0 && (sc0.ld_src & 3) == 0 && (sc0.dst.ld & 3) == 0 && (nstate < 2 || ((sc1.ld_src & 3) == 0 && (sc1.dst.ld & 3) == 0));
    if (vec) {
        for (int c4 = threadIdx.x; c4 < (H >> 2); c4 += blockDim.x) {
            float4 v0 = make_float4(0.f, 0.f, 0.f, 0.f), v1 = v0;
            if (src >= 0) {
                v0 = *reinterpret_cast<const float4*>(sc0.src + (long)src * sc0.ld_src + 4 * c4);
                if (nstate > 1) v1 = *reinterpret_cast<const float4*>(sc1.src + (long)src * sc1.ld_src + 4 * c4);
            }
            for (int s = 0; s < nstate; ++s) {
                const ActView& o = (s == 0) ? sc0.dst : sc1.dst;
                const float4 v = (s == 0) ? v0 : v1;
                *reinterpret_cast<float4*>(o.f + (long)r * o.ld + 4 * c4) = v;
                if (o.hi != nullptr) {
                    __align__(8) __half h[4];
                    __align__(8) __half l[4];
                    split_f32(v.x, h[0], l[0]); split_f32(v.y, h[1], l[1]); split_f32(v.z, h[2], l[2]); split_f32(v.w, h[3], l[3]);
                    *reinterpret_cast<uint2*>(o.hi + (long)r * o.ld + 4 * c4) = *reinterpret_cast<const uint2*>(h);
                    *reinterpret_cast<uint2*>(o.lo + (long)r * o.ld + 4 * c4) = *reinterpret_cast<const uint2*>(l);
                }
            }
        }
        return;
    }
    for (int s = 0; s < nstate; ++s) {
        const StateCopy& sc = (s == 0) ? sc0 : sc1;
        for (int c = threadIdx.x; c < H; c += blockDim.x) {
            const float v = (src < 0) ? 0.f : sc.src[(long)src * sc.ld_src + c];
            store_act(sc.dst, r, c, v);
        }
    }
}

__global__ void lstm_pointwise_kernel(int rows, int H, const float* __restrict__ gates, long ld_g, const int* __restrict__ src_row,
                                      const float* __restrict__ c_prev, long ld_cp, float* __restrict__ c_out, long ld_co, ActView h_out,
                                      const float* __restrict__ gather_bias, long ld_gb, const int* __restrict__ gather_idx) {
    const long total = (long)rows * H;
    for (long i = blockIdx.x * (long)blockDim.x + threadIdx.x; i < total; i += (long)gridDim.x * blockDim.x) {
        const int r = (int)(i / H), c = (int)(i % H);
        const float* g = gates + (long)r * ld_g;
        float gi = g[c], gf = g[H + c], gg = g[2 * H + c], go = g[3 * H + c];
        if (gather_bias != nullptr) {
            const float* gb = gather_bias + (long)gather_idx[r] * ld_gb;
            gi += __ldg(gb + c); gf += __ldg(gb + H + c); gg += __ldg(gb + 2 * H + c); go += __ldg(gb + 3 * H + c);
        }
        const int src = src_row ? src_row[r] : r;
        const float cp = (src < 0 || c_prev == nullptr) ? 0.f : c_prev[(long)src * ld_cp + c];
        const float cn = sigmoidf_(gf) * cp + sigmoidf_(gi) * fast_tanh(gg);
        const float hn = sigmoidf_(go) * fast_tanh(cn);
        c_out[(long)r * ld_co + c] = cn;
        store_act(h_out, r, c, hn);
    }
}

// ... 11 lines not shown
        hv[u] = 0.f;
        if (c < H) {
            const float gi = g[c], gf = g[H + c], gg = g[2 * H + c], go = g[3 * H + c];
            const float cp = c_prev == nullptr ? 0.f : c_prev[(long)r * ld_cp + c];
            const float cn = sigmoidf_(gf) * cp + sigmoidf_(gi) * fast_tanh(gg);
            const float hn = sigmoidf_(go) * fast_tanh(cn);
            c_out[(long)r * ld_co + c] = cn;
            h_out[(long)r * ld_h + c] = hn;
            hv[u] = hn;
            s += hn;
        }
    }
    auto bsum = [&](float v) {
#pragma unroll
        for (int o = 16; o > 0; o >>= 1) v += __shfl_xor_sync(0xffffffffu, v, o);
        __syncthreads();
        if ((threadIdx.x & 31) == 0) sh[threadIdx.x >> 5] = v;
        __syncthreads();
        return ((sh[0] + sh[1]) + (sh[2] + sh[3])) + ((sh[4] + sh[5]) + (sh[6] + sh[7]));
    };
    const float mean = bsum(s) / (float)H;
    float q = 0.f;
#pragma unroll
    for (int u = 0; u < 8; ++u) { const int c = threadIdx.x + 256 * u; if (c < H) { const float d = hv[u] - mean; q = fmaf(d, d, q); } }
    const float stdv = sqrtf(bsum(q) / (float)(H - 1));
    const float inv = 1.0f / (stdv + eps);
#pragma unroll
    for (int u = 0; u < 8; ++u) { const int c = threadIdx.x + 256 * u; if (c < H) ln_out[(long)r * ld_ln + c] = __ldg(ln_a + c) * (hv[u] - mean) * inv + __ldg(ln_b + c); }
}

__global__ void maxout_pointwise_kernel(int rows, int H, const float* __restrict__ sums, long ld_s, const int* __restrict__ src_row,
                                        const float* __restrict__ c_prev, long ld_cp, float* __restrict__ c_out, long ld_co, ActView h_out) {
    const long total = (long)rows * H;
    for (long i = blockIdx.x * (long)blockDim.x + threadIdx.x; i < total; i += (long)gridDim.x * blockDim.x) {
        const int r = (int)(i / H), c = (int)(i % H);
        const float* s = sums + (long)r * ld_s;
        const float gi = sigmoidf_(s[c]), gf = sigmoidf_(s[H + c]), go = sigmoidf_(s[2 * H + c]);
        const float gg = fmaxf(s[3 * H + c], s[4 * H + c]);
        const int src = src_row ? src_row[r] : r;
        const float cp = (src < 0 || c_prev == nullptr) ? 0.f : c_prev[(long)src * ld_cp + c];
        const float cn = gf * cp + gi * gg;
        const float hn = go * fast_tanh(cn);
        c_out[(long)r * ld_co + c] = cn;
        store_act(h_out, r, c, hn);
    }
}

constexpr int ATT_JB = 5;
constexpr int ATT_SW = 8;
template <int NA>
__global__ void __launch_bounds__(ATT_SW * 32, NA <= 16 ? 5 : 2) att_score_kernel(int rpi, int R, int A, const float* __restrict__ att_h, long ld_ah,
                                                                const float* __restrict__ p_att, long ld_pa, const float* __restrict__ alpha_w,
                                                                const float* __restrict__ alpha_b_ptr, float* __restrict__ score) {
    extern __shared__ float s_ah[];
    constexpr int AP = NA * 32;
    float* s_w = s_ah + ATT_JB * AP;
    constexpr float kC = 2.885390081777927f;
    const int img = blockIdx.y;
    const int warp = threadIdx.x >> 5, lane = threadIdx.x & 31;
    const int r = blockIdx.x * ATT_SW + warp;
    const float alpha_b = __ldg(alpha_b_ptr);
    float pv[NA];
    const bool live = r < R;
    const float* pr = p_att + ((long)img * R + (live ? r : 0)) * ld_pa;
    for (int i = threadIdx.x; i < AP; i += ATT_SW * 32) s_w[i] = (i < A) ? __ldg(alpha_w + i) : 0.f;
    __syncthreads();
    float wsum = 0.f;
#pragma unroll
    for (int k = 0; k < NA; ++k) {
        const int a = (NA % 4 == 0) ? 128 * (k >> 2) + 4 * lane + (k & 3) : lane + 32 * k;
        pv[k] = (live && a < A) ? __ldg(pr + a) * kC : 0.f;
        wsum += s_w[a];
    }
    for (int j0 = 0; j0 < rpi; j0 += ATT_JB) {
        const int nj = min(ATT_JB, rpi - j0);
        __syncthreads();
        for (int i = threadIdx.x; i < nj * AP; i += ATT_SW * 32) {
            const int j = i / AP, a = i - j * AP;
            s_ah[i] = (a < A) ? att_h[((long)img * rpi + j0 + j) * ld_ah + a] * kC : 0.f;
        }
        __syncthreads();
        if (live) {
            float part[ATT_JB];
#pragma unroll
            for (int j = 0; j < ATT_JB; ++j) {
                part[j] = 0.f;
                if (j < nj) {
                    if (NA % 4 == 0) {
                        float acc = 0.f;
#pragma unroll
                        for (int g = 0; g < NA / 4; ++g) {
                            const float4 ah = *reinterpret_cast<const float4*>(&s_ah[j * AP + 128 * g + 4 * lane]);
                            const float z[4] = {pv[4 * g] + ah.x, pv[4 * g + 1] + ah.y, pv[4 * g + 2] + ah.z, pv[4 * g + 3] + ah.w};
                            float y[4];
#pragma unroll
                            for (int u = 0; u < 4; ++u) {
                                float e;
                                asm("ex2.approx.ftz.f32 %0, %1;" : "=f"(e) : "f"(fminf(z[u], 28.0f)));
                                y[u] = 1.0f + e;
                            }
                            const float p01 = y[0] * y[1], p23 = y[2] * y[3];
                            float rr;
                            asm("rcp.approx.ftz.f32 %0, %1;" : "=f"(rr) : "f"(p01 * p23));
                            const float r01 = rr * p23, r23 = rr * p01;
                            const float4 w4 = *reinterpret_cast<const float4*>(&s_w[128 * g + 4 * lane]);
                            acc = fmaf(w4.x, r01 * y[1], acc);
                            acc = fmaf(w4.y, r01 * y[0], acc);
                            acc = fmaf(w4.z, r23 * y[3], acc);
                            acc = fmaf(w4.w, r23 * y[2], acc);
                        }
                        part[j] = fmaf(-2.0f, acc, wsum);
                    } else {
#pragma unroll
                        for (int k = 0; k < NA; ++k) {
                            float e;
                            asm("ex2.approx.ftz.f32 %0, %1;" : "=f"(e) : "f"(fminf(pv[k] + s_ah[j * AP + lane + 32 * k], 28.0f)));
                            part[j] = fmaf(s_w[lane + 32 * k], 1.0f - __fdividef(2.0f, 1.0f + e), part[j]);
                        }
                    }
                }
            }
#pragma unroll
            for (int j = 0; j < ATT_JB; ++j) {
                float v = part[j];
#pragma unroll
                for (int o = 16; o > 0; o >>= 1) v += __shfl_xor_sync(0xffffffffu, v, o);
                if (lane == 0 && j < nj) score[((long)img * rpi + j0 + j) * R + r] = v + alpha_b;
            }
        }
    }
}

constexpr int ATT_CT = 256;
__global__ void __launch_bounds__(ATT_CT) att_combine_kernel(int rpi, int R, int H, const float* __restrict__ score, const float* __restrict__ att,
                                                             long ld_at, const float* __restrict__ mask, long ld_mask, ActView out,
                                                             float* __restrict__ alpha_out) {
    extern __shared__ float s_w[];
    const int img = blockIdx.x;
    const int c = blockIdx.y * ATT_CT + threadIdx.x;
    const int warp = threadIdx.x >> 5, lane = threadIdx.x & 31;
    for (int j0 = 0; j0 < rpi; j0 += ATT_JB) {
        const int nj = min(ATT_JB, rpi - j0);
        __syncthreads();
        if (warp < nj) {
            const float* sc = score + ((long)img * rpi + j0 + warp) * R;
            float* w = s_w + warp * R;
            float mx = -INFINITY;
            for (int r = lane; r < R; r += 32) mx = fmaxf(mx, sc[r]);
#pragma unroll
            for (int o = 16; o > 0; o >>= 1) mx = fmaxf(mx, __shfl_xor_sync(0xffffffffu, mx, o));
            float sum = 0.f;
            for (int r = lane; r < R; r += 32) { const float e = expf(sc[r] - mx); w[r] = e; sum += e; }
#pragma unroll
            for (int o = 16; o > 0; o >>= 1) sum += __shfl_xor_sync(0xffffffffu, sum, o);
            const float inv = 1.0f / sum;
            float msum = 0.f;
            for (int r = lane; r < R; r += 32) {
                float v = w[r] * inv;
                if (mask != nullptr) { v *= mask[(long)img * ld_mask + r]; msum += v; }
                w[r] = v;
            }
            if (mask != nullptr) {
#pragma unroll
                for (int o = 16; o > 0; o >>= 1) msum += __shfl_xor_sync(0xffffffffu, msum, o);
                for (int r = lane; r < R; r += 32) w[r] = w[r] / msum;
            }
        }
        __syncthreads();
        if (alpha_out != nullptr && blockIdx.y == 0) {
            for (int i = threadIdx.x; i < nj * R; i += ATT_CT) alpha_out[((long)img * rpi + j0) * R + i] = s_w[i];
        }
        if (c < H) {
            float acc[ATT_JB];
#pragma unroll
            for (int j = 0; j < ATT_JB; ++j) acc[j] = 0.f;
            const float* ap = att + (long)img * R * ld_at + c;
            for (int r = 0; r < R; ++r) {
                const float v = __ldg(ap + (long)r * ld_at);
#pragma unroll
                for (int j = 0; j < ATT_JB; ++j)
                    if (j < nj) acc[j] = fmaf(s_w[j * R + r], v, acc[j]);
            }
#pragma unroll
            for (int j = 0; j < ATT_JB; ++j)
                if (j < nj) store_act(out, (long)img * rpi + j0 + j, c, acc[j]);
        }
    }
}

__global__ void relu_copy_kernel(const float* __restrict__ x, long n, ActView out_flat) {
    for (long i = blockIdx.x * (long)blockDim.x + threadIdx.x; i < n; i += (long)gridDim.x * blockDim.x) {
        const float v = fmaxf(__ldg(x + i), 0.f);
        out_flat.f[i] = v;
        if (out_flat.hi) { __half h, l; split_f32(v, h, l); out_flat.hi[i] = h; out_flat.lo[i] = l; }
    }
}

}

int relu_copy_launch(const float* x, long n, ActView out_flat, cudaStream_t stream) {
    relu_copy_kernel<<<pw_blocks(n), 256, 0, stream>>>(x, n, out_flat);
    CAPB_CHECK_CUDA(cudaGetLastError());
    return 0;
}

int state_gather_embed_launch(int rows, const int* tokens, const int* src_row, const float* emb, long ld_emb, int E, int relu,
                              ActView xt, int H, int nstate, StateCopy sc0, StateCopy sc1, cudaStream_t stream) {
    if (rows <= 0) return 0;
    state_gather_embed_kernel<<<rows, 256, 0, stream>>>(rows, tokens, src_row, emb, ld_emb, E, relu, xt, H, nstate, sc0, sc1);
    CAPB_CHECK_CUDA(cudaGetLastError());
    return 0;
}


int lstm_pointwise_launch(int rows, int H, const float* gates, long ld_g, const int* src_row, const float* c_prev, long ld_cp,
                          float* c_out, long ld_co, ActView h_out, const float* gather_bias, long ld_gb, const int* gather_idx,
                          cudaStream_t stream) {
    if (rows <= 0) return 0;
    lstm_pointwise_kernel<<<pw_blocks((long)rows * H), 256, 0, stream>>>(rows, H, gates, ld_g, src_row, c_prev, ld_cp, c_out, ld_co, h_out,
                                                                          gather_bias, ld_gb, gather_idx);
    CAPB_CHECK_CUDA(cudaGetLastError());
    return 0;
}

int lstm_ln_launch(int rows, int H, const float* gates, long ld_g, const float* c_prev, long ld_cp, float* c_out, long ld_co, float* h_out, long ld_h,
                   const float* ln_a, const float* ln_b, float eps, float* ln_out, long ld_ln, cudaStream_t stream) {
    if (rows <= 0) return 0;
    CAPB_REQUIRE(H <= 2048, "lstm_ln: hidden size above 2048");
    lstm_ln_kernel<<<rows, 256, 0, stream>>>(H, gates, ld_g, c_prev, ld_cp, c_out, ld_co, h_out, ld_h, ln_a, ln_b, eps, ln_out, ld_ln);
    CAPB_CHECK_CUDA(cudaGetLastError());
    return 0;
}

int maxout_pointwise_launch(int rows, int H, const float* sums, long ld_s, const int* src_row, const float* c_prev, long ld_cp,
                            float* c_out, long ld_co, ActView h_out, cudaStream_t stream) {
    if (rows <= 0) return 0;
    maxout_pointwise_kernel<<<pw_blocks((long)rows * H), 256, 0, stream>>>(rows, H, sums, ld_s, src_row, c_prev, ld_cp, c_out, ld_co, h_out);
    CAPB_CHECK_CUDA(cudaGetLastError());
    return 0;
}

int additive_attention_launch(int n_images, int rpi, int R, int A, int H, const float* att_h, long ld_ah, const float* p_att, long ld_pa,
                              const float* att, long ld_at, const float* mask, long ld_mask, const float* alpha_w, const float* alpha_b,
                              float* score_scratch, ActView out, cudaStream_t stream, float* alpha_out) {
    if (n_images <= 0 || rpi <= 0) return 0;
    CAPB_REQUIRE(A <= 1024, "attention: att_hid_size above 1024");
    CAPB_REQUIRE(score_scratch != nullptr, "attention: score scratch missing");
    const int na = cdiv(A, 32);
    dim3 sgrid(cdiv(R, ATT_SW), n_images);
#define CAPB_ATT_CASE(NA_)                                                                                                             \
    att_score_kernel<NA_><<<sgrid, ATT_SW * 32, sizeof(float) * (ATT_JB + 1) * NA_ * 32, stream>>>(rpi, R, A, att_h, ld_ah, p_att, ld_pa, alpha_w, \
                                                                                               alpha_b, score_scratch)
    if (na <= 2) CAPB_ATT_CASE(2);
    else if (na <= 4) CAPB_ATT_CASE(4);
    else if (na <= 8) CAPB_ATT_CASE(8);
    else if (na <= 16) CAPB_ATT_CASE(16);
    else CAPB_ATT_CASE(32);
#undef CAPB_ATT_CASE
    CAPB_CHECK_CUDA(cudaGetLastError());
    const size_t smem = sizeof(float) * (size_t)ATT_JB * R;
    CAPB_REQUIRE(smem <= 48 * 1024, "attention: too many regions");
    dim3 grid(n_images, cdiv(H, ATT_CT));
    att_combine_kernel<<<grid, ATT_CT, smem, stream>>>(rpi, R, H, score_scratch, att, ld_at, mask, ld_mask, out, alpha_out);
    CAPB_CHECK_CUDA(cudaGetLastError());
    return 0;
}

}
```

imagecaptioning.pytorch_b200/csrc/ptx.cuh:

```cuda
#pragma once
#include <cstdint>
#include <cuda.h>
#include <cuda_runtime.h>

namespace capb200 {
namespace ptx {

__device__ __forceinline__ uint32_t smem_u32(const void* p) {
    return static_cast<uint32_t>(__cvta_generic_to_shared(p));
}

__device__ __forceinline__ uint32_t elect_one() {
    uint32_t pred = 0;
    asm volatile(
        "{\n\t"
        ".reg .pred P;\n\t"
        "elect.sync _|P, 0xffffffff;\n\t"
        "selp.b32 %0, 1, 0, P;\n\t"
        "}\n"
        : "=r"(pred));
    return pred;
}

__device__ __forceinline__ void mbar_init(uint64_t* bar, uint32_t count) {
    asm volatile("mbarrier.init.shared::cta.b64 [%0], %1;" ::"r"(smem_u32(bar)), "r"(count) : "memory");
}
__device__ __forceinline__ void fence_mbar_init() {
    asm volatile("fence.mbarrier_init.release.cluster;" ::: "memory");
}
__device__ __forceinline__ void fence_proxy_async_smem() {
    asm volatile("fence.proxy.async.shared::cta;" ::: "memory");
}
__device__ __forceinline__ void mbar_arrive_expect_tx(uint64_t* bar, uint32_t bytes) {
    asm volatile("mbarrier.arrive.expect_tx.shared::cta.b64 _, [%0], %1;" ::"r"(smem_u32(bar)), "r"(bytes) : "memory");
}
__device__ __forceinline__ void mbar_arrive(uint64_t* bar) {
    asm volatile("mbarrier.arrive.shared::cta.b64 _, [%0];" ::"r"(smem_u32(bar)) : "memory");
}
__device__ __forceinline__ bool mbar_try_wait(uint64_t* bar, uint32_t parity) {
    uint32_t ok;
    asm volatile(
        "{\n\t"
        ".reg .pred P;\n\t"
        "mbarrier.try_wait.parity.shared::cta.b64 P, [%1], %2;\n\t"
        "selp.b32 %0, 1, 0, P;\n\t"
        "}\n"
        : "=r"(ok)
        : "r"(smem_u32(bar)), "r"(parity)
        : "memory");
    return ok != 0;
}
__device__ __forceinline__ void mbar_wait(uint64_t* bar, uint32_t parity) {
    uint32_t spins = 0;
    while (!mbar_try_wait(bar, parity)) {
        if (++spins > 200000000u) { __trap(); }
    }
}

template <int N>
__device__ __forceinline__ void setmaxnreg_dec() { asm volatile("setmaxnreg.dec.sync.aligned.u32 %0;" ::"n"(N)); }
template <int N>
__device__ __forceinline__ void setmaxnreg_inc() { asm volatile("setmaxnreg.inc.sync.aligned.u32 %0;" ::"n"(N)); }

__device__ __forceinline__ void prefetch_tmap(const CUtensorMap* m) {
    asm volatile("prefetch.tensormap [%0];" ::"l"(reinterpret_cast<uint64_t>(m)) : "memory");
}
__device__ __forceinline__ void tma_load_2d(void* smem_dst, const CUtensorMap* m, uint64_t* bar, int32_t c_inner, int32_t c_outer) {
    asm volatile(
        "cp.async.bulk.tensor.2d.shared::cluster.global.mbarrier::complete_tx::bytes [%0], [%1, {%3, %4}], [%2];"
        ::"r"(smem_u32(smem_dst)), "l"(reinterpret_cast<uint64_t>(m)), "r"(smem_u32(bar)), "r"(c_inner), "r"(c_outer)
        : "memory");
}

__device__ __forceinline__ void bulk_load_1d(void* smem_dst, const void* gsrc, uint32_t bytes, uint64_t* bar) {
    asm volatile("cp.async.bulk.shared::cluster.global.mbarrier::complete_tx::bytes [%0], [%1], %2, [%3];"
                 ::"r"(smem_u32(smem_dst)), "l"(reinterpret_cast<uint64_t>(gsrc)), "r"(bytes), "r"(smem_u32(bar)) : "memory");
}

__device__ __forceinline__ uint32_t cluster_ctaid_x() { uint32_t v; asm volatile("mov.u32 %0, %%cluster_ctaid.x;" : "=r"(v)); return v; }
__device__ __forceinline__ uint32_t cluster_ctaid_y() { uint32_t v; asm volatile("mov.u32 %0, %%cluster_ctaid.y;" : "=r"(v)); return v; }
__device__ __forceinline__ uint32_t cluster_ctarank() { uint32_t v; asm volatile("mov.u32 %0, %%cluster_ctarank;" : "=r"(v)); return v; }
__device__ __forceinline__ void cluster_sync_all() {
    asm volatile("barrier.cluster.arrive.release.aligned;" ::: "memory");
    asm volatile("barrier.cluster.wait.acquire.aligned;" ::: "memory");
}

__device__ __forceinline__ void wgmma_fence() { asm volatile("wgmma.fence.sync.aligned;" ::: "memory"); }
__device__ __forceinline__ void wgmma_commit() { asm volatile("wgmma.commit_group.sync.aligned;" ::: "memory"); }
template <int N>
__device__ __forceinline__ void wgmma_wait() { asm volatile("wgmma.wait_group.sync.aligned %0;" ::"n"(N) : "memory"); }
__device__ __forceinline__ void reg_fence(float& r) { asm volatile("" : "+f"(r)::"memory"); }

__device__ __forceinline__ uint64_t make_smem_desc_sw128(uint32_t smem_addr) {
    uint64_t d = 0;
    d |= static_cast<uint64_t>((smem_addr & 0x3FFFFu) >> 4);
    d |= static_cast<uint64_t>(1) << 16;
    d |= static_cast<uint64_t>(1024u >> 4) << 32;
    d |= static_cast<uint64_t>(1) << 62;
    return d;
}

__device__ __forceinline__ void wgmma_f16_n32(float* d, uint64_t desc_a, uint64_t desc_b, int scale_d) {
    asm volatile(
        "{\n\t.reg .pred p;\n\tsetp.ne.b32 p, %18, 0;\n\t"
        "wgmma.mma_async.sync.aligned.m64n32k16.f32.f16.f16 "
        "{"
        "%0, %1, %2, %3, %4, %5, %6, %7, %8, %9, %10, %11, %12, %13, %14, %15"
        "}, %16, %17, p, 1, 1, 0, 0;\n\t}\n"
        : "+f"(d[0]), "+f"(d[1]), "+f"(d[2]), "+f"(d[3]), "+f"(d[4]), "+f"(d[5]), "+f"(d[6]), "+f"(d[7]),
          "+f"(d[8]), "+f"(d[9]), "+f"(d[10]), "+f"(d[11]), "+f"(d[12]), "+f"(d[13]), "+f"(d[14]), "+f"(d[15])
        : "l"(desc_a), "l"(desc_b), "r"(scale_d));
}
__device__ __forceinline__ void wgmma_f16_n64(float* d, uint64_t desc_a, uint64_t desc_b, int scale_d) {
    asm volatile(
        "{\n\t.reg .pred p;\n\tsetp.ne.b32 p, %34, 0;\n\t"
        "wgmma.mma_async.sync.aligned.m64n64k16.f32.f16.f16 "
        "{"
        "%0, %1, %2, %3, %4, %5, %6, %7, %8, %9, %10, %11, %12, %13, %14, %15, "
        "%16, %17, %18, %19, %20, %21, %22, %23, %24, %25, %26, %27, %28, %29, %30, %31"
// ... 99 lines not shown
```

imagecaptioning.pytorch_b200/csrc/tfm_engine.cu:

```cuda
#include <vector>

#include "../../include/capb200.h"
#include "common.cuh"
#include "engine_common.cuh"
#include "train_common.cuh"
#include "kernels.cuh"

using namespace capb200;

namespace capb200 {
const char* last_error_cstr();
}

struct capb200_tfm_engine {
    capb200_tfm_cfg cfg{};
    capb200_tfm_weights w{};
    int V1 = 0, D = 0, Dff = 0, H = 0, dk = 0, NE = 0, ND = 0, F = 0, T = 0, mode = 0;
    bool tc = false, bound = false;
    long launches = 0;

    char* wblock = nullptr;
    float *enc_qkv_w[CAPB200_TFM_MAX_LAYERS] = {}, *enc_qkv_b[CAPB200_TFM_MAX_LAYERS] = {};
    float *dec_qkv_w[CAPB200_TFM_MAX_LAYERS] = {}, *dec_qkv_b[CAPB200_TFM_MAX_LAYERS] = {};
    float *dec_skv_w[CAPB200_TFM_MAX_LAYERS] = {}, *dec_skv_b[CAPB200_TFM_MAX_LAYERS] = {};
// ... 254 lines not shown
    e->w = *w;
    const int D = e->D, Dff = e->Dff;
    if (e->wblock == nullptr) {
        Arena dry;
        layout_weights(e, dry);
        CAPB_CHECK_CUDA(cudaMalloc(&e->wblock, dry.off + 256));
        Arena real;
        real.base = e->wblock;
        layout_weights(e, real);
    }
    const long dd = (long)D * D;
    for (int l = 0; l < e->NE; ++l) {
        const capb200_mha_weights& a = w->enc[l].self_attn;
        if (concat_rows(e->enc_qkv_w[l], a.q_w, a.k_w, a.v_w, dd, st) || concat_rows(e->enc_qkv_b[l], a.q_b, a.k_b, a.v_b, D, st)) return 1;
    }
    for (int l = 0; l < e->ND; ++l) {
        const capb200_mha_weights& a = w->dec[l].self_attn;
        const capb200_mha_weights& s = w->dec[l].src_attn;
        if (concat_rows(e->dec_qkv_w[l], a.q_w, a.k_w, a.v_w, dd, st) || concat_rows(e->dec_qkv_b[l], a.q_b, a.k_b, a.v_b, D, st)) return 1;
        if (concat_rows(e->dec_skv_w[l], s.k_w, s.v_w, nullptr, dd, st) || concat_rows(e->dec_skv_b[l], s.k_b, s.v_b, nullptr, D, st)) return 1;
    }
    if (e->tc) {
        int rc = pack(e, w->att_embed_w, D, e->F, e->p_att, st) | pack(e, w->gen_w, e->V1, D, e->p_gen, st);
        for (int l = 0; l < e->NE; ++l) {
            rc |= pack(e, e->enc_qkv_w[l], 3 * D, D, e->pe_qkv[l], st) | pack(e, w->enc[l].self_attn.o_w, D, D, e->pe_o[l], st);
            rc |= pack(e, w->enc[l].w1_w, Dff, D, e->pe_w1[l], st) | pack(e, w->enc[l].w2_w, D, Dff, e->pe_w2[l], st);
        }
        for (int l = 0; l < e->ND; ++l) {
            rc |= pack(e, e->dec_qkv_w[l], 3 * D, D, e->pd_qkv[l], st) | pack(e, w->dec[l].self_attn.o_w, D, D, e->pd_o[l], st);
            rc |= pack(e, w->dec[l].src_attn.q_w, D, D, e->pd_qs[l], st) | pack(e, e->dec_skv_w[l], 2 * D, D, e->pd_skv[l], st);
            rc |= pack(e, w->dec[l].src_attn.o_w, D, D, e->pd_os[l], st);
            rc |= pack(e, w->dec[l].w1_w, Dff, D, e->pd_w1[l], st) | pack(e, w->dec[l].w2_w, D, Dff, e->pd_w2[l], st);
        }
        if (rc) return 1;
        if (!e->bound) {
            CAPB_CHECK_CUDA(cudaStreamSynchronize(st));
            CAPB_CHECK_RANGE();
        }
    }
    e->bound = true;
    return 0;
}

int capb200_tfm_decode_beam(capb200_tfm_engine* e, const float* att, const float* mask, int B, int R, const capb200_beam_opts* opts, long long* seq,
                            float* seq_logprobs, long long* done_seq, int* done_len, float* done_p, float* done_raw, void* stream) {
    if (check_ready(e)) return 1;
    cudaStream_t st = static_cast<cudaStream_t>(stream);
    CAPB_REQUIRE(opts != nullptr && att != nullptr && seq != nullptr && B >= 1 && R >= 1, "bad argument");
    const int beam = opts->beam_size, keep = opts->sample_n;
    CAPB_REQUIRE(beam >= 1 && beam <= 16 && beam <= e->V1, "beam_size must be in 1..16 and <= V+1");
    CAPB_REQUIRE(keep == 1 || keep == beam, "sample_n must be 1 or beam_size (AttModel.py:223)");
    if (ensure_workspace(e, B, B * beam, R, beam, st)) return 1;
    if (prepare(e, att, mask, B, R, st)) return 1;
    auto core = [&](int nrows, int live, const int* tokens, const int* , int t, float* logits, long ld) {
        const int* anc = (t == 0) ? nullptr : beam_ancestors(e->d.bs, t);
        return core_step(e, nrows, live, tokens, anc, nullptr, 0, t, logits, ld, R, mask, st);
    };
    return beam_decode_driver(e->d, e->V1, e->T, B, beam, keep, opts->penalty_kind, opts->penalty_alpha, seq, seq_logprobs, done_seq, done_len, done_p,
                              done_raw, core, &e->launches, st, loop_graph_key(e->ws, e->wblock, mask, R, 7), to_edits(opts->edits), opts->temperature);
}

int capb200_tfm_beam_record_logprobs(capb200_tfm_engine* e, int image, int rank, float* dst, void* stream) {
    if (check_ready(e)) return 1;
    return beam_record_logprobs(e->d, e->V1, e->T, image, rank, dst, static_cast<cudaStream_t>(stream));
}

int capb200_tfm_decode_sample(capb200_tfm_engine* e, const float* att, const float* mask, int B, int R, const capb200_sample_opts* opts,
                              const long long* tokens_in, long ld_tok, long long* seq, float* seq_logprobs, float* picked, void* stream) {
    if (check_ready(e)) return 1;
    cudaStream_t st = static_cast<cudaStream_t>(stream);
    CAPB_REQUIRE(opts != nullptr && att != nullptr && seq_logprobs != nullptr && B >= 1 && R >= 1, "bad argument");
    const int n = opts->sample_n, method = opts->method;
    CAPB_REQUIRE(n >= 1 && method >= 0 && method <= 5, "bad sampling options");
    if (method == CAPB200_SAMPLE_FORCED || method == CAPB200_SAMPLE_TEACHER) CAPB_REQUIRE(tokens_in != nullptr && ld_tok >= 1, "token matrix required");
    if (method != CAPB200_SAMPLE_TEACHER) CAPB_REQUIRE(seq != nullptr, "seq output required");
    if (method == CAPB200_SAMPLE_MULTINOMIAL) CAPB_REQUIRE(opts->temperature > 0.f, "temperature must be positive");
    const int rows = B * n;
    const int steps = (method == CAPB200_SAMPLE_TEACHER) ? opts->steps : e->T;
    const long t_out = (method == CAPB200_SAMPLE_TEACHER) ? ld_tok : e->T;
    CAPB_REQUIRE(steps >= 0 && steps <= t_out && steps <= e->T + 1 && steps <= 31, "steps out of range");
    if (ensure_workspace(e, B, rows, R, 1, st)) return 1;
    if (prepare(e, att, mask, B, R, st)) return 1;
    const long long* labels = (method == CAPB200_SAMPLE_TEACHER) ? tokens_in : nullptr;
    auto core = [&](int nrows, int , const int* tokens, const int* , int t, float* logits, long ld) {
        return core_step(e, nrows, n, tokens, nullptr, labels, ld_tok, t, logits, ld, R, mask, st);
    };
    return sample_decode_driver(e->d, e->V1, e->T, rows, method, opts->temperature, opts->seed, steps, tokens_in, ld_tok, seq, seq_logprobs, picked,
                                core, &e->launches, st, to_edits(opts->edits), opts->top);
}

}


namespace {

constexpr int TML = CAPB200_TFM_MAX_LAYERS;

struct TTape : StepTape {
    float *X[TML + 1], *eln0[TML], *eqkv[TML], *eatt[TML], *xm[TML], *eln1[TML], *ehd[TML], *mem, *skv[TML];
    float *Y[TML + 1], *dln0[TML], *dqkv[TML], *datt[TML], *ym1[TML], *dln1[TML], *dqs[TML], *probs[TML], *dcatt[TML], *ym2[TML], *dln2[TML], *dhd[TML];
    float *yln_tm, *yln_nm;
    int* tok;
    float* key_mask;
    float *d_yln_nm, *dY, *d_tmp, *d_h, *d_ln, *d_att, *d_qs, *d_qkv, *d_skv[TML], *d_mem, *dX, *tmp, *stats;
};

void layout_ttape(TTape& tp, Arena& a, int B, int R, int N, int T, int D, int Dff, int heads, int V1, int NE, int ND, long glp_floats) {
// ... 268 lines not shown
```

imagecaptioning.pytorch_b200/csrc/vocab.cu:

```cuda
#include <cstdlib>

#include "common.cuh"
#include "kernels.cuh"
#include "ptx.cuh"

namespace capb200 {

static __device__ unsigned long long g_vocab_seed_salt = 0ull;
int dropout_salt_set_vocab(unsigned long long salt, cudaStream_t st) {
    return cudaMemcpyToSymbolAsync(g_vocab_seed_salt, &salt, sizeof(salt), 0, cudaMemcpyHostToDevice, st) == cudaSuccess ? 0 : 1;
}

namespace {

constexpr int VT = 256;

template <int NT = VT>
__device__ __forceinline__ float block_max(float v, float* scratch) {
#pragma unroll
    for (int o = 16; o > 0; o >>= 1) v = fmaxf(v, __shfl_xor_sync(0xffffffffu, v, o));
    __syncthreads();
    if ((threadIdx.x & 31) == 0) scratch[threadIdx.x >> 5] = v;
    __syncthreads();
    float r = scratch[0];
// ... 348 lines not shown
                };
                for (int v = threadIdx.x; v < n4; v += VT) {
                    const float4 x = g4[v];
                    consider(x.x, 4 * v); consider(x.y, 4 * v + 1); consider(x.z, 4 * v + 2); consider(x.w, 4 * v + 3);
                }
            }
        }
        if (threadIdx.x == 0) {
            const float lp = (ov - mx) - lsum;
            a.top_val[(long)r * a.topk + k] = a.row_twice(r) ? (lp - m2) - l2 : lp;
            a.top_idx[(long)r * a.topk + k] = oi;
        }
    }
}

constexpr int VT2 = 128;
__device__ __forceinline__ float block_max4(float v, float* scratch) {
#pragma unroll
    for (int o = 16; o > 0; o >>= 1) v = fmaxf(v, __shfl_xor_sync(0xffffffffu, v, o));
    __syncthreads();
    if ((threadIdx.x & 31) == 0) scratch[threadIdx.x >> 5] = v;
    __syncthreads();
    return fmaxf(fmaxf(scratch[0], scratch[1]), fmaxf(scratch[2], scratch[3]));
}
__device__ __forceinline__ float block_sum4(float v, float* scratch) {
#pragma unroll
    for (int o = 16; o > 0; o >>= 1) v += __shfl_xor_sync(0xffffffffu, v, o);
    __syncthreads();
    if ((threadIdx.x & 31) == 0) scratch[threadIdx.x >> 5] = v;
    __syncthreads();
    return (scratch[0] + scratch[1]) + (scratch[2] + scratch[3]);
}
__device__ __forceinline__ void block_argmax4(float v, int i, float* sval, int* sidx, float& out_v, int& out_i) {
#pragma unroll
    for (int o = 16; o > 0; o >>= 1) {
        const float ov = __shfl_xor_sync(0xffffffffu, v, o);
        const int oi = __shfl_xor_sync(0xffffffffu, i, o);
        if (ov > v || (ov == v && oi < i)) { v = ov; i = oi; }
    }
    __syncthreads();
    if ((threadIdx.x & 31) == 0) { sval[threadIdx.x >> 5] = v; sidx[threadIdx.x >> 5] = i; }
    __syncthreads();
    out_v = sval[0];
    out_i = sidx[0];
#pragma unroll
    for (int w = 1; w < VT2 / 32; ++w) {
        const float ov = sval[w];
        const int oi = sidx[w];
        if (ov > out_v || (ov == out_v && oi < out_i)) { out_v = ov; out_i = oi; }
    }
}

__global__ void __launch_bounds__(VT2) vocab_stats_online128_kernel(const VocabStepArgs a) {
    __shared__ float s_red[VT2 / 32];
    __shared__ int s_idx[VT2 / 32];
    const int r = blockIdx.x;
    const int n4 = a.V1 >> 2;
    const float4* g4 = reinterpret_cast<const float4*>(a.logits + (long)r * a.ld);
    constexpr float kL2E = 1.4426950408889634f;
    float t0v = -INFINITY, t1v = -INFINITY;
    int t0i = 0x7fffffff, t1i = 0x7fffffff;
    float m = -INFINITY, mL = -INFINITY, part = 0.f;
    auto consume = [&](const float4 x, int v) {
        const float m4 = fmaxf(fmaxf(x.x, x.y), fmaxf(x.z, x.w));
        if (m4 > m) {
            float sc;
            asm("ex2.approx.ftz.f32 %0, %1;" : "=f"(sc) : "f"((m - m4) * kL2E));
            part = (m == -INFINITY) ? 0.f : part * sc;
            m = m4;
            mL = m4 * kL2E;
        }
        float e0, e1, e2, e3;
        asm("ex2.approx.ftz.f32 %0, %1;" : "=f"(e0) : "f"(fmaf(x.x, kL2E, -mL)));
        asm("ex2.approx.ftz.f32 %0, %1;" : "=f"(e1) : "f"(fmaf(x.y, kL2E, -mL)));
        asm("ex2.approx.ftz.f32 %0, %1;" : "=f"(e2) : "f"(fmaf(x.z, kL2E, -mL)));
        asm("ex2.approx.ftz.f32 %0, %1;" : "=f"(e3) : "f"(fmaf(x.w, kL2E, -mL)));
        part += (e0 + e1) + (e2 + e3);
        if (m4 > t1v) {
            const float xs[4] = {x.x, x.y, x.z, x.w};
#pragma unroll
            for (int u = 0; u < 4; ++u) {
                if (xs[u] > t1v) {
                    if (xs[u] > t0v) { t1v = t0v; t1i = t0i; t0v = xs[u]; t0i = 4 * v + u; }
                    else { t1v = xs[u]; t1i = 4 * v + u; }
                }
            }
        }
    };
    int v = threadIdx.x;
    for (; v + 3 * VT2 < n4; v += 4 * VT2) {
        const float4 x0 = g4[v], x1 = g4[v + VT2], x2 = g4[v + 2 * VT2], x3 = g4[v + 3 * VT2];
        consume(x0, v); consume(x1, v + VT2); consume(x2, v + 2 * VT2); consume(x3, v + 3 * VT2);
    }
    for (; v < n4; v += VT2) consume(g4[v], v);
    const float mx = block_max4(m, s_red);
    float sum = (m == -INFINITY) ? 0.f : part * __expf(m - mx);
    sum = block_sum4(sum, s_red);
    const float lsum = logf(sum);
    const float m2 = (mx - mx) - lsum, l2 = lsum;
    if (threadIdx.x == 0) a.stats[r] = make_float2(mx, lsum);
    int popped = 0;
    for (int k = 0; k < a.topk; ++k) {
        float ov;
        int oi;
        block_argmax4(t0v, t0i, s_red, s_idx, ov, oi);
        if (t0i == oi && oi != 0x7fffffff) {
// ... 174 lines not shown
                    }
                }
            }
            if (threadIdx.x == 0) {
                const float lp = (ov - mx) - lsum;
                a.top_val[(long)r * a.topk + k] = a.row_twice(r) ? (lp - m2) - l2 : lp;
                a.top_idx[(long)r * a.topk + k] = oi;
            }
        }
        __syncthreads();
    }
}

__global__ void __launch_bounds__(VT) ss_select_kernel(int V1, const float* __restrict__ prev_logp, long ld, const long long* __restrict__ labels,
                                                      long ld_labels, int col, unsigned long long seed, float prob, int* __restrict__ tok_out) {
    __shared__ float s_red[VT / 32];
    __shared__ int s_idx[VT / 32];
    const int r = blockIdx.x;
    seed ^= g_vocab_seed_salt;
    const uint32_t k0 = (uint32_t)seed ^ 0x6a09e667u, k1 = (uint32_t)(seed >> 32) ^ 0xbb67ae85u;
    const uint32_t ubits = philox_first(0xffffffffu, (uint32_t)r, (uint32_t)col, 6u, k0, k1);
    const float u_row = ((float)(ubits >> 9) + 0.5f) * (1.0f / 8388608.0f);
    if (!(u_row < prob)) {
        if (threadIdx.x == 0) tok_out[r] = (int)labels[(long)r * ld_labels + col];
        return;
    }
    const float* g = prev_logp + (long)r * ld;
    float bv = -INFINITY;
    int bi = 0x7fffffff;
    for (int v = threadIdx.x; v < V1; v += VT) {
        const uint32_t bits = philox_first((uint32_t)v, (uint32_t)r, (uint32_t)col, 6u, k0, k1);
        const float u = ((float)(bits >> 9) + 0.5f) * (1.0f / 8388608.0f);
        const float x = g[v] - logf(-logf(u));
        if (x > bv) { bv = x; bi = v; }
    }
    float ov;
    int tok;
    block_argmax(bv, bi, s_red, s_idx, ov, tok);
    if (threadIdx.x == 0) tok_out[r] = tok;
}

__global__ void mask_rows_kernel(ActView x, int R, int cols, const float* __restrict__ mask, long ld_mask) {
    const int row = blockIdx.x;
    const int img = row / R, r = row % R;
    if (mask[(long)img * ld_mask + r] != 0.f) return;
    for (int c = threadIdx.x; c < cols; c += blockDim.x) {
        x.f[(long)row * x.ld + c] = 0.f;
        if (x.hi) { x.hi[(long)row * x.ld + c] = __float2half(0.f); x.lo[(long)row * x.ld + c] = __float2half(0.f); }
    }
}

}

int vocab_step_launch(const VocabStepArgs& a, cudaStream_t stream) {
    if (a.rows <= 0) return 0;
    CAPB_REQUIRE(a.topk <= 16, "beam size up to 16");
    if (a.stats != nullptr) {
        CAPB_REQUIRE(a.select == 0 && a.topk > 0, "stats mode is the beam-search epilogue");
        const bool vec = ((a.V1 & 3) == 0) && ((a.ld & 3) == 0) && ((reinterpret_cast<uintptr_t>(a.logits) & 15) == 0);
        const size_t stream_smem = sizeof(float) * 2 * (size_t)a.V1;
        static const char* variant = getenv("CAPB200_VOCAB_STATS");
        const char vsel = variant ? variant[0] : 'o';
        if (vec && vsel == 'o' && !(variant && variant[1] == '2')) {
            vocab_stats_online128_kernel<<<a.rows, VT2, 0, stream>>>(a);
        } else if (vec && vsel == 'o') {
            vocab_stats_online_kernel<<<a.rows, VT, 0, stream>>>(a);
        } else if (vec && vsel == 's' && stream_smem <= 100 * 1024) {
            static std::atomic<unsigned long long> configured{0};
            if (first_use_on_device(configured)) {
                CAPB_CHECK_CUDA(cudaFuncSetAttribute(vocab_stats_stream_kernel, cudaFuncAttributeMaxDynamicSharedMemorySize, (int)(100 * 1024)));
            }
            const int grid = a.rows < 2 * sm_count() ? a.rows : 2 * sm_count();
            vocab_stats_stream_kernel<<<grid, VT, stream_smem, stream>>>(a);
        } else if (vec && vsel == 'r' && a.V1 <= VT * 4 * 10) {
            vocab_stats_reg_kernel<10><<<a.rows, VT, 0, stream>>>(a);
        } else {
            vocab_stats_kernel<<<a.rows, VT, 0, stream>>>(a);
        }
        CAPB_CHECK_CUDA(cudaGetLastError());
        return 0;
    }
    const size_t smem = sizeof(float) * (size_t)a.V1;
    CAPB_REQUIRE(smem <= 200 * 1024, "vocabulary larger than 51200 entries needs the multi-pass variant");
    static std::atomic<unsigned long long> configured{0};
    if (first_use_on_device(configured)) {
        CAPB_CHECK_CUDA(cudaFuncSetAttribute(vocab_step_kernel<2>, cudaFuncAttributeMaxDynamicSharedMemorySize, (int)(200 * 1024)));
        CAPB_CHECK_CUDA(cudaFuncSetAttribute(vocab_step_kernel<8>, cudaFuncAttributeMaxDynamicSharedMemorySize, (int)(200 * 1024)));
        CAPB_CHECK_CUDA(cudaFuncSetAttribute(vocab_step_kernel<16>, cudaFuncAttributeMaxDynamicSharedMemorySize, (int)(200 * 1024)));
    }
    if (a.topk <= 2 && a.select != 0 && a.rows <= 2 * sm_count()) {
        static std::atomic<unsigned long long> configured2{0};
        if (first_use_on_device(configured2)) {
            CAPB_CHECK_CUDA(cudaFuncSetAttribute(vocab_step_kernel<2, 1024>, cudaFuncAttributeMaxDynamicSharedMemorySize, (int)(200 * 1024)));
        }
        vocab_step_kernel<2, 1024><<<a.rows, 1024, smem, stream>>>(a);
    }
    else if (a.topk <= 2) vocab_step_kernel<2><<<a.rows, VT, smem, stream>>>(a);
    else if (a.topk <= 8) vocab_step_kernel<8><<<a.rows, VT, smem, stream>>>(a);
    else vocab_step_kernel<16><<<a.rows, VT, smem, stream>>>(a);
    CAPB_CHECK_CUDA(cudaGetLastError());
    return 0;
}

int ss_select_launch(int rows, int V1, const float* prev_logp, long ld, const long long* labels, long ld_labels, int col, unsigned long long seed, float prob,
                     int* tok_out, cudaStream_t stream) {
    if (rows <= 0) return 0;
    ss_select_kernel<<<rows, VT, 0, stream>>>(V1, prev_logp, ld, labels, ld_labels, col, seed, prob, tok_out);
    CAPB_CHECK_CUDA(cudaGetLastError());
    return 0;
}

int mask_rows_launch(ActView x, int n_images, int R, int cols, const float* mask, long ld_mask, cudaStream_t stream) {
    if (n_images <= 0 || mask == nullptr) return 0;
    mask_rows_kernel<<<n_images * R, 128, 0, stream>>>(x, R, cols, mask, ld_mask);
    CAPB_CHECK_CUDA(cudaGetLastError());
    return 0;
}
// ... 3 lines not shown
```

Measured before the change: 24010.

## Enable programmatic dependent launch across the LSTM beam-decode kernel chain

Launches the per-step decode kernels (state gather, gemm, attention score/combine, vocab stats, beam step) with the programmatic stream serialization attribute, and adds griddepcontrol launch_dependents/wait at kernel entry. The aim is to hide launch and ramp-up latency between the many small kernels in each beam step inside the captured graph. The TC path also switches the state gather to copy the fp16 hi/lo planes directly and stops writing the fp32 h copy, which cuts memory traffic. Correctness relies on every kernel waiting before it reads, and PDL is disabled when the language stream is split.

```diff
diff --git a/imagecaptioning.pytorch_b200/csrc/aoa_engine.cu b/imagecaptioning.pytorch_b200/csrc/aoa_engine.cu
--- a/imagecaptioning.pytorch_b200/csrc/aoa_engine.cu
+++ b/imagecaptioning.pytorch_b200/csrc/aoa_engine.cu
@@ -453,7 +453,7 @@
     CAPB_REQUIRE(keep == 1 || keep == beam, "sample_n must be 1 or beam_size (AttModel.py:223)");
     if (aoa_decode_workspace(e, B, B * beam, R, beam, st)) return 1;
     if (aoa_decode_prepare(e, att, mask, B, R, st)) return 1;
-    auto core = [&](int nrows, int live, const int* tokens, const int* src_row, int , float* logits, long ld) {
+    auto core = [&](int nrows, int live, const int* tokens, const int* src_row, int , float* logits, long ld, bool ) {
         return aoa_decode_core(e, nrows, live, tokens, src_row, logits, ld, R, mask, st);
     };
     return beam_decode_driver(e->d, e->V1, e->T, B, beam, keep, opts->penalty_kind, opts->penalty_alpha, seq, seq_logprobs, done_seq, done_len, done_p,
diff --git a/imagecaptioning.pytorch_b200/csrc/beam.cu b/imagecaptioning.pytorch_b200/csrc/beam.cu
--- a/imagecaptioning.pytorch_b200/csrc/beam.cu
+++ b/imagecaptioning.pytorch_b200/csrc/beam.cu
@@ -1,5 +1,6 @@
 #include "common.cuh"
 #include "kernels.cuh"
+#include "ptx.cuh"
 
 namespace capb200 {
 
@@ -112,6 +113,8 @@
 __global__ void __launch_bounds__(32) beam_step_kernel(BeamState s, int t, int live, const float* __restrict__ top_val,
                                                        const int* __restrict__ top_idx, int penalty_kind, float penalty_alpha,
                                                        double* __restrict__ done_p) {
+    ptx::pdl_trigger();
+    ptx::pdl_wait();
     const int img = blockIdx.x;
     select_step(s, img, t, live, s.beam, img * live, img * live, top_val, top_idx, nullptr, 0, 0.f, penalty_kind, penalty_alpha, done_p);
 }
@@ -311,11 +314,10 @@
 }
 
 int beam_step_launch(const BeamState& s, int t, int live, const float* top_val, const int* top_idx, int penalty_kind, float penalty_alpha,
-                     cudaStream_t stream) {
+                     cudaStream_t stream, bool pdl) {
     CAPB_REQUIRE(s.beam >= 1 && s.beam <= MAXB, "beam size 1..16");
     CAPB_REQUIRE(s.beam * s.T <= MAXB * 64, "beam*T record capacity");
-    beam_step_kernel<<<s.B, 32, 0, stream>>>(s, t, live, top_val, top_idx, penalty_kind, penalty_alpha, s.done_p);
-    CAPB_CHECK_CUDA(cudaGetLastError());
+    CAPB_CHECK_CUDA(launch_kernel(pdl, beam_step_kernel, dim3(s.B), dim3(32), 0, stream, s, t, live, top_val, top_idx, penalty_kind, penalty_alpha, s.done_p));
     return 0;
 }
 
diff --git a/imagecaptioning.pytorch_b200/csrc/common.cuh b/imagecaptioning.pytorch_b200/csrc/common.cuh
--- a/imagecaptioning.pytorch_b200/csrc/common.cuh
+++ b/imagecaptioning.pytorch_b200/csrc/common.cuh
@@ -2,6 +2,7 @@
 #include <atomic>
 #include <cstdint>
 #include <cstdio>
+#include <cstdlib>
 #include <cstring>
 #include <string>
 #include <cuda.h>
@@ -48,6 +49,31 @@
         cache[dev].store(n);
     }
     return n;
+}
+
+constexpr const char* kPdlKernels[] = {
+    "gemm_tc_kernel", "gemm_tc256_kernel", "state_gather_embed_kernel", "att_score_kernel", "att_combine_kernel",
+    "vocab_stats_online128_kernel", "beam_step_kernel",
+};
+inline bool pdl_enabled() { return getenv("CAPB200_NO_PDL") == nullptr; }
+
+template <typename... KArgs, typename... Args>
+inline cudaError_t launch_kernel(bool pdl, void (*kernel)(KArgs...), dim3 grid, dim3 block, size_t smem, cudaStream_t stream, Args... args) {
+    if (!pdl) {
+        kernel<<<grid, block, smem, stream>>>(args...);
+        return cudaGetLastError();
+    }
+    cudaLaunchAttribute attr[1];
+    attr[0].id = cudaLaunchAttributeProgrammaticStreamSerialization;
+    attr[0].val.programmaticStreamSerializationAllowed = 1;
+    cudaLaunchConfig_t cfg = {};
+    cfg.gridDim = grid;
+    cfg.blockDim = block;
+    cfg.dynamicSmemBytes = smem;
+    cfg.stream = stream;
+    cfg.attrs = attr;
+    cfg.numAttrs = 1;
+    return cudaLaunchKernelEx(&cfg, kernel, args...);
 }
 
 __device__ __forceinline__ void split_f32(float x, __half& hi, __half& lo) {
@@ -135,7 +161,7 @@
 int gemm_tc_tile_n(int M, int N);
 int gemm_tc_tile_m(int M, int N, int bn);
 void gemm_tc_plan_destroy(GemmTcPlan* plan);
-int gemm_tc_plan_launch(GemmTcPlan* plan, const GemmEpilogue* epi_override, int M_override, cudaStream_t stream);
+int gemm_tc_plan_launch(GemmTcPlan* plan, const GemmEpilogue* epi_override, int M_override, cudaStream_t stream, bool pdl = false);
 bool gemm_tc_supported(const GemmProblem& p, std::string* why);
 
 int split_planes_launch(const float* x, long ldx, int rows, int cols, __half* hi, __half* lo, long ldh, cudaStream_t stream);
diff --git a/imagecaptioning.pytorch_b200/csrc/engine.cu b/imagecaptioning.pytorch_b200/csrc/engine.cu
--- a/imagecaptioning.pytorch_b200/csrc/engine.cu
+++ b/imagecaptioning.pytorch_b200/csrc/engine.cu
@@ -235,7 +235,7 @@
     return fill_int_launch(e->d.neg1, nRows, -1, st);
 }
 
-int run_gemm_inner(capb200_engine* e, int id, GemmProblem& g, int plan_rows, cudaStream_t st) {
+int run_gemm_inner(capb200_engine* e, int id, GemmProblem& g, int plan_rows, cudaStream_t st, bool pdl = false) {
     e->launches++;
     if (!e->tc) return gemm_simt_launch(g, st);
     if (e->plans[id] == nullptr) {
@@ -244,11 +244,11 @@
         e->plans[id] = gemm_tc_plan_create(planned, e->mode == CAPB200_MODE_TC_F16X3 ? 3 : 1);
         if (e->plans[id] == nullptr) return 1;
     }
-    return gemm_tc_plan_launch(e->plans[id], &g.epi, g.M, st);
-}
-
-int run_gemm(capb200_engine* e, int id, GemmProblem& g, int plan_rows, cudaStream_t st) {
-    if (!e->profiling) return run_gemm_inner(e, id, g, plan_rows, st);
+    return gemm_tc_plan_launch(e->plans[id], &g.epi, g.M, st, pdl);
+}
+
+int run_gemm(capb200_engine* e, int id, GemmProblem& g, int plan_rows, cudaStream_t st, bool pdl = false) {
+    if (!e->profiling) return run_gemm_inner(e, id, g, plan_rows, st, pdl);
     if (e->ev_used + 2 > e->ev_pool.size()) {
         for (int i = 0; i < 64; ++i) {
             cudaEvent_t ev;
@@ -326,16 +326,20 @@
 }
 
 int core_step(capb200_engine* e, int rows, int rpi, const int* tokens, const int* src_row, float* logits, long ld_logits, int n_images, int R,
-              const float* mask, cudaStream_t st) {
+              const float* mask, cudaStream_t st, bool pdl = false) {
     const int H = e->H, E = e->E, A = e->A, V1 = e->V1;
     const capb200_weights& w = e->w;
     if (e->cfg.family == CAPB200_FAMILY_UPDOWN) {
         StateCopy s0, s1;
         s0.src = e->h0_out.v.f; s0.ld_src = e->h0_out.v.ld; s0.dst = e->h0_in.v;
         s1.src = e->h1_out.v.f; s1.ld_src = e->h1_out.v.ld; s1.dst = e->h1_in.v;
+        if (e->tc) {
+            s0.src = nullptr; s0.src_hi = e->h0_out.v.hi; s0.src_lo = e->h0_out.v.lo; s0.dst.f = nullptr;
+            s1.src = nullptr; s1.src_hi = e->h1_out.v.hi; s1.src_lo = e->h1_out.v.lo; s1.dst.f = nullptr;
+        }
         const bool xg = e->use_xgate;
         e->launches++;
-        if (state_gather_embed_launch(rows, tokens, src_row, w.embed, E, xg ? 0 : E, 1, e->xt.v, H, 2, s0, s1, st)) return 1;
+        if (state_gather_embed_launch(rows, tokens, src_row, w.embed, E, xg ? 0 : E, 1, e->xt.v, H, 2, s0, s1, st, pdl)) return 1;
         const int cur = e->core_cur, nxt = cur ^ 1;
         {
             GemmProblem g;
@@ -350,11 +354,11 @@
                 g.epi.c_prev = e->c0[cur]; g.epi.ld_cprev = e->ld_c; g.epi.src_row = src_row;
                 g.epi.c_out = e->c0[nxt]; g.epi.ld_cout = e->ld_c;
                 g.epi.gather_bias = xg ? e->xgate : nullptr; g.epi.ld_gb = e->ld_xgate; g.epi.gather_idx = tokens;
-                g.epi.h_f = e->h0_out.v.f; g.epi.h_hi = e->h0_out.v.hi; g.epi.h_lo = e->h0_out.v.lo; g.epi.ld_h = e->h0_out.v.ld;
+                g.epi.h_hi = e->h0_out.v.hi; g.epi.h_lo = e->h0_out.v.lo; g.epi.ld_h = e->h0_out.v.ld;
             } else {
                 g.epi.C = e->gates.v.f; g.epi.ldc = e->gates.v.ld;
             }
-            if (run_gemm(e, G_LSTM1, g, e->capRows, st)) return 1;
+            if (run_gemm(e, G_LSTM1, g, e->capRows, st, pdl)) return 1;
         }
         if (!e->tc) {
             e->launches++;
@@ -367,9 +371,10 @@
             g.seg[0] = seg_of(e->h0_out.v, w.h2att_w, H, e->p_h2att, H);
             g.epi.bias = w.h2att_b;
             g.epi.C = e->att_h.v.f; g.epi.ldc = e->att_h.v.ld;
-            if (run_gemm(e, G_H2ATT, g, e->capRows, st)) return 1;
+            if (run_gemm(e, G_H2ATT, g, e->capRows, st, pdl)) return 1;
         }
         const bool split = e->split_lang && e->tc && e->side != nullptr;
+        const bool pdl_rest = pdl && !split;
         if (split) {
             CAPB_CHECK_CUDA(cudaEventRecord(e->ev_fork, st));
             CAPB_CHECK_CUDA(cudaStreamWaitEvent(e->side, e->ev_fork, 0));
@@ -384,7 +389,7 @@
         }
         e->launches += 2;
         if (additive_attention_launch(n_images, rpi, R, A, H, e->att_h.v.f, e->att_h.v.ld, e->p_att.v.f, e->p_att.v.ld, e->att_e.v.f, e->att_e.v.ld,
-                                      mask, R, w.alpha_w, w.alpha_b, e->att_score, e->att_res.v, st)) return 1;
+                                      mask, R, w.alpha_w, w.alpha_b, e->att_score, e->att_res.v, st, nullptr, pdl_rest)) return 1;
         if (split) {
             CAPB_CHECK_CUDA(cudaStreamWaitEvent(st, e->ev_join, 0));
             GemmProblem g;
@@ -394,7 +399,7 @@
             g.epi.lstm = 1; g.epi.H = H;
             g.epi.c_prev = e->c1[cur]; g.epi.ld_cprev = e->ld_c; g.epi.src_row = src_row;
             g.epi.c_out = e->c1[nxt]; g.epi.ld_cout = e->ld_c;
-            g.epi.h_f = e->h1_out.v.f; g.epi.h_hi = e->h1_out.v.hi; g.epi.h_lo = e->h1_out.v.lo; g.epi.ld_h = e->h1_out.v.ld;
+            g.epi.h_hi = e->h1_out.v.hi; g.epi.h_lo = e->h1_out.v.lo; g.epi.ld_h = e->h1_out.v.ld;
             if (run_gemm(e, G_LSTM2B, g, e->capRows, st)) return 1;
         } else {
             GemmProblem g;
@@ -407,12 +412,12 @@
                 g.epi.lstm = 1; g.epi.H = H;
                 g.epi.c_prev = e->c1[cur]; g.epi.ld_cprev = e->ld_c; g.epi.src_row = src_row;
                 g.epi.c_out = e->c1[nxt]; g.epi.ld_cout = e->ld_c;
-                g.epi.h_f = e->h1_out.v.f; g.epi.h_hi = e->h1_out.v.hi; g.epi.h_lo = e->h1_out.v.lo; g.epi.ld_h = e->h1_out.v.ld;
+                g.epi.h_hi = e->h1_out.v.hi; g.epi.h_lo = e->h1_out.v.lo; g.epi.ld_h = e->h1_out.v.ld;
             } else {
                 g.epi.bias = e->bsum_lang;
                 g.epi.C = e->gates.v.f; g.epi.ldc = e->gates.v.ld;
             }
-            if (run_gemm(e, G_LSTM2, g, e->capRows, st)) return 1;
+            if (run_gemm(e, G_LSTM2, g, e->capRows, st, pdl_rest)) return 1;
         }
         if (!e->tc) {
             e->launches++;
@@ -426,7 +431,7 @@
             g.seg[0] = seg_of(e->h1_out.v, w.logit_w, H, e->p_logit, H);
             g.epi.bias = w.logit_b;
             g.epi.C = logits; g.epi.ldc = ld_logits;
-            if (run_gemm(e, G_LOGIT, g, e->capRows, st)) return 1;
+            if (run_gemm(e, G_LOGIT, g, e->capRows, st, pdl_rest)) return 1;
         }
         return 0;
     }
@@ -541,8 +546,8 @@
 }
 
 int lstm_decode_core(capb200_engine* e, int rows, int rpi, const int* tokens, const int* src_row, float* logits, long ld, int B, int R,
-                     const float* mask, cudaStream_t st) {
-    return core_step(e, rows, rpi, tokens, src_row, logits, ld, B, R, mask, st);
+                     const float* mask, cudaStream_t st, bool pdl) {
+    return core_step(e, rows, rpi, tokens, src_row, logits, ld, B, R, mask, st, pdl);
 }
 
 }
@@ -773,8 +778,8 @@
     const int rows = B * beam;
     if (lstm_decode_workspace(e, B, rows, R, beam, 1, st)) return 1;
     if (lstm_decode_prepare(e, fc, att, mask, B, R, st)) return 1;
-    auto core = [&](int nrows, int live, const int* tokens, const int* src_row, int , float* logits, long ld) {
-        return lstm_decode_core(e, nrows, live, tokens, src_row, logits, ld, B, R, mask, st);
+    auto core = [&](int nrows, int live, const int* tokens, const int* src_row, int , float* logits, long ld, bool pdl) {
+        return lstm_decode_core(e, nrows, live, tokens, src_row, logits, ld, B, R, mask, st, pdl);
     };
     return beam_decode_driver(e->d, V1, T, B, beam, keep, opts->penalty_kind, opts->penalty_alpha, seq, seq_logprobs, done_seq, done_len, done_p,
                               done_raw, core, &e->launches, st, e->profiling ? 0ull : loop_graph_key(e->ws, e->wblock, mask, R, (int)e->cfg.family),
diff --git a/imagecaptioning.pytorch_b200/csrc/engine_common.cuh b/imagecaptioning.pytorch_b200/csrc/engine_common.cuh
--- a/imagecaptioning.pytorch_b200/csrc/engine_common.cuh
+++ b/imagecaptioning.pytorch_b200/csrc/engine_common.cuh
@@ -241,6 +241,7 @@
     d.last_beam = beam;
     BeamState s = d.bs;
     s.B = B; s.beam = beam; s.T = T; s.V1 = V1;
+    const bool pdl = graph_key != 0 && pdl_enabled();
     auto run_loop = [&]() -> int {
         CAPB_NVTX("capb200 beam loop (T steps: core, vocab stats, beam step)");
         CAPB_CHECK_CUDA(cudaMemsetAsync(s.sums, 0, sizeof(float) * B * beam, st));
@@ -250,7 +251,7 @@
             const int live = (t == 0) ? 1 : beam;
             const int nrows = B * live;
             float* logits = d.slab + (long)t * d.slab_step_stride;
-            if (core(nrows, live, d.tokens, t == 0 ? d.neg1 : d.src_row, t, logits, (long)V1)) return 1;
+            if (core(nrows, live, d.tokens, t == 0 ? d.neg1 : d.src_row, t, logits, (long)V1, pdl)) return 1;
             if (t > 0 && temperature != 1.0f) {
                 if (scale_rows_launch(logits, V1, nrows, V1, 1.0f / temperature, st)) return 1;
                 *launches += 1;
@@ -260,7 +261,7 @@
             va.twice = (t > 0) ? 1 : 0;
             va.topk = edits ? k_in : beam; va.top_val = d.top_val; va.top_idx = d.top_idx;
             va.stats = d.slab_stats + (long)t * rows;
-            if (vocab_step_launch(va, st)) return 1;
+            if (vocab_step_launch(va, st, pdl)) return 1;
             const float* tv = d.top_val;
             const int* ti = d.top_idx;
             if (edits) {
@@ -268,7 +269,7 @@
                 tv = d.top_val_e; ti = d.top_idx_e;
                 *launches += 1;
             }
-            if (beam_step_launch(s, t, live, tv, ti, penalty_kind, penalty_alpha, st)) return 1;
+            if (beam_step_launch(s, t, live, tv, ti, penalty_kind, penalty_alpha, st, pdl)) return 1;
             *launches += 2;
         }
         return 0;
@@ -277,6 +278,7 @@
                                  (unsigned long long)penalty_kind, 0ull, (unsigned long long)reinterpret_cast<uintptr_t>(d.slab)};
     memcpy(&key[6], &penalty_alpha, sizeof(float));
     memcpy(reinterpret_cast<char*>(&key[6]) + 4, &temperature, sizeof(float));
+    key[7] ^= pdl ? 1ull : 0ull;
     key[5] ^= ((unsigned long long)(ed.constraint & 1) << 8) ^ ((unsigned long long)(unsigned)(ed.unk_col + 1) << 16) ^ ((unsigned long long)ed.n_bad << 48);
     key[0] ^= (unsigned long long)reinterpret_cast<uintptr_t>(ed.bad) * 0x9E3779B97F4A7C15ull;
     d.last_edits = ed;
@@ -458,7 +460,7 @@
 int lstm_decode_workspace(capb200_engine* e, int B, int rows, int R, int beam, int rows_per_image, cudaStream_t st);
 int lstm_decode_prepare(capb200_engine* e, const float* fc, const float* att, const float* mask, int B, int R, cudaStream_t st);
 int lstm_decode_core(capb200_engine* e, int rows, int rpi, const int* tokens, const int* src_row, float* logits, long ld, int B, int R,
-                     const float* mask, cudaStream_t st);
+                     const float* mask, cudaStream_t st, bool pdl = false);
 int aoa_member_info(capb200_aoa_engine* e, MemberInfo* m);
 int aoa_decode_workspace(capb200_aoa_engine* e, int B, int rows, int R, int beam, cudaStream_t st);
 int aoa_decode_prepare(capb200_aoa_engine* e, const float* att, const float* mask, int B, int R, cudaStream_t st);
diff --git a/imagecaptioning.pytorch_b200/csrc/ensemble.cu b/imagecaptioning.pytorch_b200/csrc/ensemble.cu
--- a/imagecaptioning.pytorch_b200/csrc/ensemble.cu
+++ b/imagecaptioning.pytorch_b200/csrc/ensemble.cu
@@ -238,7 +238,7 @@
     if (setup(s, E, fc, att, mask, B, rows, beam, 1, st)) return 1;
     s->V1 = V1; s->T = T;
     const long stride = (long)rows * V1;
-    auto core = [&](int nrows, int live, const int* tokens, const int* src_row, int , float* logits, long ld) {
+    auto core = [&](int nrows, int live, const int* tokens, const int* src_row, int , float* logits, long ld, bool ) {
         return step(s, E, nrows, live, tokens, src_row, logits, ld, stride, B, mask, st);
     };
     return beam_decode_driver(s->d, V1, T, B, beam, keep, opts->penalty_kind, opts->penalty_alpha, seq, seq_logprobs, done_seq, done_len, done_p,
diff --git a/imagecaptioning.pytorch_b200/csrc/gemm_tc.cu b/imagecaptioning.pytorch_b200/csrc/gemm_tc.cu
--- a/imagecaptioning.pytorch_b200/csrc/gemm_tc.cu
+++ b/imagecaptioning.pytorch_b200/csrc/gemm_tc.cu
@@ -208,7 +208,8 @@
     }
     if (row_ok) {
         float* const c_out = p.c_out + (long)row * p.ld_cout + u0;
-        float* const h_f = p.h_f + (long)row * p.ld_h + u0;
+        const bool hf = p.h_f != nullptr;
+        float* const h_f = hf ? p.h_f + (long)row * p.ld_h + u0 : nullptr;
         __half* const h_hi = p.h_hi + (long)row * p.ld_h + u0;
         __half* const h_lo = p.h_lo + (long)row * p.ld_h + u0;
         const bool planes = p.h_hi != nullptr;
@@ -220,7 +221,7 @@
                 const float* c = cn + 4 * k;
                 const float* h = hn + 4 * k;
                 *reinterpret_cast<float4*>(c_out + 8 * k) = make_float4(c[0], c[1], c[2], c[3]);
-                *reinterpret_cast<float4*>(h_f + 8 * k) = make_float4(h[0], h[1], h[2], h[3]);
+                if (hf) *reinterpret_cast<float4*>(h_f + 8 * k) = make_float4(h[0], h[1], h[2], h[3]);
                 if (planes) {
                     __half hh[4], hl[4];
 #pragma unroll
@@ -237,7 +238,7 @@
                 const int du = 8 * (i / 4) + i % 4;
                 if (u0 + du < p.H) {
                     c_out[du] = cn[i];
-                    h_f[du] = hn[i];
+                    if (hf) h_f[du] = hn[i];
                     if (planes) {
                         __half hh, hl;
                         split_f32(hn[i], hh, hl);
@@ -335,20 +336,87 @@
 }
 
 template <typename Cfg>
-__device__ __forceinline__ void fill_stage(const TcParams& p, uint8_t* st, uint64_t* bar, int s, int kb, int m0, int n0) {
-    uint8_t* a_hi = st;
-    uint8_t* a_lo = st + Cfg::kABytes;
+__device__ __forceinline__ void fill_w(const TcParams& p, uint8_t* st, uint64_t* bar, int s, int kb, int n0) {
     uint8_t* w_hi = st + Cfg::kABytes * Cfg::kPlanes;
-    uint8_t* w_lo = w_hi + Cfg::kWBytes;
     ptx::mbar_arrive_expect_tx(bar, Cfg::kStageBytes);
-#pragma unroll
-    for (int r = 0; r < Cfg::kTileM; r += BM) ptx::tma_load_2d(a_hi + r * BK * 2, &p.a_hi[s], bar, kb * BK, m0 + r);
     ptx::tma_load_2d(w_hi, &p.w_hi[s], bar, kb * BK, n0);
+    if (Cfg::kPasses == 3) ptx::tma_load_2d(w_hi + Cfg::kWBytes, &p.w_lo[s], bar, kb * BK, n0);
+}
+template <typename Cfg>
+__device__ __forceinline__ void fill_a(const TcParams& p, uint8_t* st, uint64_t* bar, int s, int kb, int m0) {
+#pragma unroll
+    for (int r = 0; r < Cfg::kTileM; r += BM) ptx::tma_load_2d(st + r * BK * 2, &p.a_hi[s], bar, kb * BK, m0 + r);
     if (Cfg::kPasses == 3) {
 #pragma unroll
-        for (int r = 0; r < Cfg::kTileM; r += BM) ptx::tma_load_2d(a_lo + r * BK * 2, &p.a_lo[s], bar, kb * BK, m0 + r);
-        ptx::tma_load_2d(w_lo, &p.w_lo[s], bar, kb * BK, n0);
-    }
+        for (int r = 0; r < Cfg::kTileM; r += BM) ptx::tma_load_2d(st + Cfg::kABytes + r * BK * 2, &p.a_lo[s], bar, kb * BK, m0 + r);
+    }
+}
+
+__device__ __forceinline__ void prefetch_slice(const float* q, int n) {
+    const uint32_t bytes = (uint32_t)(n * 4) & ~15u;
+    if (bytes > 0 && (reinterpret_cast<uintptr_t>(q) & 15) == 0) ptx::prefetch_l2(q, bytes);
+}
+template <int TM, int BN>
+__device__ __forceinline__ void prefetch_lstm_operands(const TcParams& p, int m0, int n0, int lane) {
+    constexpr int kRows = 2;
+    const int units = min(BN / 4, p.H - n0 / 4);
+    const int cols = min(BN, p.N - n0);
+#pragma unroll 1
+    for (int r1 = m0 + lane; r1 < m0 + TM; r1 += 32 * kRows) {
+        int src[kRows], tok[kRows];
+#pragma unroll
+        for (int i = 0; i < kRows; ++i) {
+            const int r = r1 + 32 * i;
+            src[i] = (r < p.M && p.c_prev != nullptr) ? (p.src_row != nullptr ? p.src_row[r] : r) : -1;
+            tok[i] = (r < p.M && p.gather_bias != nullptr) ? p.gather_idx[r] : -1;
+        }
+#pragma unroll
+        for (int i = 0; i < kRows; ++i) {
+            const int r = r1 + 32 * i;
+            if (src[i] >= 0) prefetch_slice(p.c_prev + (long)src[i] * p.ld_cprev + n0 / 4, units);
+            if (tok[i] >= 0) prefetch_slice(p.gather_bias + (long)tok[i] * p.ld_gb + n0, cols);
+            if (r < p.M && p.row_bias != nullptr && (r == m0 || r % p.rows_per_group == 0))
+                prefetch_slice(p.row_bias + (long)(r / p.rows_per_group) * p.ld_row_bias + n0, cols);
+        }
+    }
+}
+
+template <typename Cfg, int BN, int EPI, bool TRACE>
+__device__ __forceinline__ void produce(const TcParams& p, uint8_t* smem, uint64_t* full_bar, uint64_t* empty_bar) {
+    const int lane = threadIdx.x & 31;
+    const int n_tiles = p.tiles_m * p.tiles_n;
+    int pre = 0;
+    if (lane == 0) {
+        const int n0 = ((int)blockIdx.x / p.tiles_m) * BN;
+        for (int s = 0, kb = 0; pre < Cfg::kStages && s < p.nseg; ++pre) {
+            fill_w<Cfg>(p, smem + pre * Cfg::kStageBytes, &full_bar[pre], s, kb, n0);
+            if (++kb == p.kblocks[s]) { kb = 0; ++s; }
+        }
+    }
+    ptx::pdl_wait();
+    int stage = 0, g = 0;
+    uint32_t phase = 0;
+    for (int t = blockIdx.x; t < n_tiles; t += gridDim.x) {
+        const int m0 = (t % p.tiles_m) * Cfg::kTileM;
+        const int n0 = (t / p.tiles_m) * BN;
+        if (lane == 0) {
+            for (int s = 0; s < p.nseg; ++s) {
+                for (int kb = 0; kb < p.kblocks[s]; ++kb, ++g) {
+                    uint8_t* st = smem + stage * Cfg::kStageBytes;
+                    if (g >= pre) {
+                        ptx::mbar_wait(&empty_bar[stage], phase ^ 1);
+                        fill_w<Cfg>(p, st, &full_bar[stage], s, kb, n0);
+                    }
+                    fill_a<Cfg>(p, st, &full_bar[stage], s, kb, m0);
+                    if (++stage == Cfg::kStages) { stage = 0; phase ^= 1; }
+                }
+            }
+            if (TRACE && Cfg::kTileM == 2 * BM && t == (int)blockIdx.x) CAPB_TRACE(5);
+        }
+        __syncwarp();
+        if (EPI == kEpiLstm) prefetch_lstm_operands<Cfg::kTileM, BN>(p, m0, n0, lane);
+    }
+    ptx::pdl_trigger();
 }
 
 template <int BN, int PASSES>
@@ -402,23 +470,10 @@
 
     if (wg == 0) {
         ptx::setmaxnreg_dec<40>();
-        if (threadIdx.x == 0) {
-            int stage = 0;
-            uint32_t phase = 0;
-            for (int t = blockIdx.x; t < n_tiles; t += gridDim.x) {
-                const int m0 = (t % p.tiles_m) * BM;
-                const int n0 = (t / p.tiles_m) * BN;
-                for (int s = 0; s < p.nseg; ++s) {
-                    for (int kb = 0; kb < p.kblocks[s]; ++kb) {
-                        ptx::mbar_wait(&empty_bar[stage], phase ^ 1);
-                        fill_stage<Cfg>(p, smem + stage * Cfg::kStageBytes, &full_bar[stage], s, kb, m0, n0);
-                        if (++stage == Cfg::kStages) { stage = 0; phase ^= 1; }
-                    }
-                }
-            }
-        }
+        if (threadIdx.x < 32) produce<Cfg, BN, EPI, TRACE>(p, smem, full_bar, empty_bar);
     } else {
         ptx::setmaxnreg_inc<232>();
+        ptx::pdl_wait();
         const int cw = wg - 1;
         const int tid = threadIdx.x & 127;
         int kb_tile = 0;
@@ -476,24 +531,10 @@
 
     if (wg == 0) {
         ptx::setmaxnreg_dec<40>();
-        if (threadIdx.x == 0) {
-            int stage = 0;
-            uint32_t phase = 0;
-            for (int t = blockIdx.x; t < n_tiles; t += gridDim.x) {
-                const int m0 = (t % p.tiles_m) * Cfg::kTileM;
-                const int n0 = (t / p.tiles_m) * BN;
-                for (int s = 0; s < p.nseg; ++s) {
-                    for (int kb = 0; kb < p.kblocks[s]; ++kb) {
-                        ptx::mbar_wait(&empty_bar[stage], phase ^ 1);
-                        fill_stage<Cfg>(p, smem + stage * Cfg::kStageBytes, &full_bar[stage], s, kb, m0, n0);
-                        if (++stage == Cfg::kStages) { stage = 0; phase ^= 1; }
-                    }
-                }
-                if (TRACE && t == (int)blockIdx.x) CAPB_TRACE(5);
-            }
-        }
+        if (threadIdx.x < 32) produce<Cfg, BN, EPI, TRACE>(p, smem, full_bar, empty_bar);
     } else {
         ptx::setmaxnreg_inc<232>();
+        ptx::pdl_wait();
         const int cw = wg - 1;
         const int tid = threadIdx.x & 127;
         const uint32_t a_rows = cw * BM * BK * 2;
@@ -557,7 +598,7 @@
 }
 
 template <int BN, int PASSES, int EPI, bool TRACE, int TM>
-int launch_cfg(const TcParams& prm, cudaStream_t stream) {
+int launch_cfg(const TcParams& prm, cudaStream_t stream, bool pdl) {
     using Cfg = TcCfg<BN, PASSES, TM>;
     void (*kernel)(TcParams);
     if constexpr (TM == BM) kernel = gemm_tc_kernel<BN, PASSES, EPI, TRACE>;
@@ -571,28 +612,27 @@
     prm2.tiles_m = cdiv(prm.M, TM);
     const int n_tiles = prm2.tiles_n * prm2.tiles_m;
     const int sms = sm_count();
-    kernel<<<n_tiles < sms ? n_tiles : sms, kThreads, Cfg::kSmemBytes, stream>>>(prm2);
-    CAPB_CHECK_CUDA(cudaGetLastError());
+    CAPB_CHECK_CUDA(launch_kernel(pdl, kernel, dim3(n_tiles < sms ? n_tiles : sms), dim3(kThreads), Cfg::kSmemBytes, stream, prm2));
     return 0;
 }
 
 template <int EPI, int TM>
-int launch_width(int bn, int passes, const TcParams& prm, cudaStream_t stream) {
+int launch_width(int bn, int passes, const TcParams& prm, cudaStream_t stream, bool pdl) {
     if (prm.trace != nullptr) {
-        if (bn == 160) return launch_cfg<160, 3, EPI, true, TM>(prm, stream);
-        if constexpr (TM == BM) if (bn == 64) return launch_cfg<64, 3, EPI, true, TM>(prm, stream);
-        return launch_cfg<128, 3, EPI, true, TM>(prm, stream);
-    }
-    if (bn == 160) return passes == 3 ? launch_cfg<160, 3, EPI, false, TM>(prm, stream) : launch_cfg<160, 1, EPI, false, TM>(prm, stream);
+        if (bn == 160) return launch_cfg<160, 3, EPI, true, TM>(prm, stream, pdl);
+        if constexpr (TM == BM) if (bn == 64) return launch_cfg<64, 3, EPI, true, TM>(prm, stream, pdl);
+        return launch_cfg<128, 3, EPI, true, TM>(prm, stream, pdl);
+    }
+    if (bn == 160) return passes == 3 ? launch_cfg<160, 3, EPI, false, TM>(prm, stream, pdl) : launch_cfg<160, 1, EPI, false, TM>(prm, stream, pdl);
     if constexpr (TM == BM) {
-        if (bn == 64) return passes == 3 ? launch_cfg<64, 3, EPI, false, TM>(prm, stream) : launch_cfg<64, 1, EPI, false, TM>(prm, stream);
-    }
-    return passes == 3 ? launch_cfg<128, 3, EPI, false, TM>(prm, stream) : launch_cfg<128, 1, EPI, false, TM>(prm, stream);
+        if (bn == 64) return passes == 3 ? launch_cfg<64, 3, EPI, false, TM>(prm, stream, pdl) : launch_cfg<64, 1, EPI, false, TM>(prm, stream, pdl);
+    }
+    return passes == 3 ? launch_cfg<128, 3, EPI, false, TM>(prm, stream, pdl) : launch_cfg<128, 1, EPI, false, TM>(prm, stream, pdl);
 }
 
 template <int EPI>
-int launch_kind(int bm, int bn, int passes, const TcParams& prm, cudaStream_t stream) {
-    return bm == 2 * BM ? launch_width<EPI, 2 * BM>(bn, passes, prm, stream) : launch_width<EPI, BM>(bn, passes, prm, stream);
+int launch_kind(int bm, int bn, int passes, const TcParams& prm, cudaStream_t stream, bool pdl) {
+    return bm == 2 * BM ? launch_width<EPI, 2 * BM>(bn, passes, prm, stream, pdl) : launch_width<EPI, BM>(bn, passes, prm, stream, pdl);
 }
 
 }
@@ -681,23 +721,23 @@
 
 void gemm_tc_plan_destroy(GemmTcPlan* plan) { delete plan; }
 
-int gemm_tc_plan_launch(GemmTcPlan* plan, const GemmEpilogue* epi_override, int M_override, cudaStream_t stream) {
+int gemm_tc_plan_launch(GemmTcPlan* plan, const GemmEpilogue* epi_override, int M_override, cudaStream_t stream, bool pdl) {
     if (M_override > plan->prm.M) { set_error("gemm_tc: M override exceeds the planned row count"); return 1; }
     const int M = M_override > 0 ? M_override : plan->prm.M;
     TcParams prm = plan->prm;
     if (epi_override != nullptr) fill_epilogue(prm, *epi_override);
     prm.M = M;
-    if (prm.lstm && (prm.N != 4 * prm.H || prm.c_out == nullptr || prm.h_f == nullptr)) {
-        set_error("gemm_tc: fused LSTM epilogue needs N == 4H, c_out and h_f");
+    if (prm.lstm && (prm.N != 4 * prm.H || prm.c_out == nullptr || (prm.h_f == nullptr && (prm.h_hi == nullptr || prm.h_lo == nullptr)))) {
+        set_error("gemm_tc: fused LSTM epilogue needs N == 4H, c_out and h_f or the h_hi / h_lo planes");
         return 1;
     }
     if (prm.M <= 0 || prm.N <= 0) return 0;
     const int kind = prm.lstm ? kEpiLstm : prm.C_hi != nullptr ? kEpiPlanes : kEpiStore;
     if (prm.trace != nullptr && plan->passes != 3) { set_error("gemm_tc: the traced kernel is the 3-pass one"); return 1; }
     const int bm = gemm_tc_tile_m(prm.M, prm.N, plan->bn);
-    if (kind == kEpiLstm) return launch_kind<kEpiLstm>(bm, plan->bn, plan->passes, prm, stream);
-    if (kind == kEpiPlanes) return launch_kind<kEpiPlanes>(bm, plan->bn, plan->passes, prm, stream);
-    return launch_kind<kEpiStore>(bm, plan->bn, plan->passes, prm, stream);
-}
-
-}
+    if (kind == kEpiLstm) return launch_kind<kEpiLstm>(bm, plan->bn, plan->passes, prm, stream, pdl);
+    if (kind == kEpiPlanes) return launch_kind<kEpiPlanes>(bm, plan->bn, plan->passes, prm, stream, pdl);
+    return launch_kind<kEpiStore>(bm, plan->bn, plan->passes, prm, stream, pdl);
+}
+
+}
diff --git a/imagecaptioning.pytorch_b200/csrc/kernels.cuh b/imagecaptioning.pytorch_b200/csrc/kernels.cuh
--- a/imagecaptioning.pytorch_b200/csrc/kernels.cuh
+++ b/imagecaptioning.pytorch_b200/csrc/kernels.cuh
@@ -14,10 +14,12 @@
     const float* src = nullptr;
     long ld_src = 0;
     ActView dst;
+    const __half* src_hi = nullptr;
+    const __half* src_lo = nullptr;
 };
 
 int state_gather_embed_launch(int rows, const int* tokens, const int* src_row, const float* emb, long ld_emb, int E, int relu,
-                              ActView xt, int H, int nstate, StateCopy sc0, StateCopy sc1, cudaStream_t stream);
+                              ActView xt, int H, int nstate, StateCopy sc0, StateCopy sc1, cudaStream_t stream, bool pdl = false);
 int lstm_pointwise_launch(int rows, int H, const float* gates, long ld_g, const int* src_row, const float* c_prev, long ld_cp,
                           float* c_out, long ld_co, ActView h_out, const float* gather_bias, long ld_gb, const int* gather_idx,
                           cudaStream_t stream);
@@ -28,7 +30,8 @@
                             float* c_out, long ld_co, ActView h_out, cudaStream_t stream);
 int additive_attention_launch(int n_images, int rpi, int R, int A, int H, const float* att_h, long ld_ah, const float* p_att, long ld_pa,
                               const float* att, long ld_at, const float* mask, long ld_mask, const float* alpha_w, const float* alpha_b,
-                              float* score_scratch , ActView out, cudaStream_t stream, float* alpha_out = nullptr );
+                              float* score_scratch , ActView out, cudaStream_t stream, float* alpha_out = nullptr ,
+                              bool pdl = false);
 int mask_rows_launch(ActView x, int n_images, int R, int cols, const float* mask, long ld_mask, cudaStream_t stream);
 int ss_select_launch(int rows, int V1, const float* prev_logp, long ld, const long long* labels, long ld_labels, int col, unsigned long long seed, float prob,
                      int* tok_out, cudaStream_t stream);
@@ -75,7 +78,7 @@
         return twice && !(first_beam > 0 && (r % first_beam) / first_group_rows == first_group);
     }
 };
-int vocab_step_launch(const VocabStepArgs& a, cudaStream_t stream);
+int vocab_step_launch(const VocabStepArgs& a, cudaStream_t stream, bool pdl = false);
 int beam_edit_launch(int rows, int k_in, int beam, int t, const DecodeEdits& ed, const int* prev_tokens, const float* val_in, const int* idx_in,
                      float* val_out, int* idx_out, cudaStream_t stream, int first_beam = 0, int first_group_rows = 1, int first_group = -1);
 int scale_rows_launch(float* x, long ld, int rows, int cols, float factor, cudaStream_t stream, int skip_beam = 0, int skip_group_rows = 1,
@@ -98,7 +101,7 @@
     int* src_row = nullptr;
 };
 int beam_step_launch(const BeamState& s, int t, int live, const float* top_val, const int* top_idx, int penalty_kind, float penalty_alpha,
-                     cudaStream_t stream);
+                     cudaStream_t stream, bool pdl = false);
 int diverse_beam_step_launch(const BeamState& s, int G, int t, int k, const float* top_val, const int* top_idx, float lambda, int rows_total,
                              int penalty_kind, float penalty_alpha, cudaStream_t stream);
 int beam_finalize_launch(const BeamState& s, int keep, long long* out_seq, int* out_len, float* out_p, float* out_raw, int* out_hist,
diff --git a/imagecaptioning.pytorch_b200/csrc/pointwise.cu b/imagecaptioning.pytorch_b200/csrc/pointwise.cu
--- a/imagecaptioning.pytorch_b200/csrc/pointwise.cu
+++ b/imagecaptioning.pytorch_b200/csrc/pointwise.cu
@@ -1,5 +1,6 @@
 #include "common.cuh"
 #include "kernels.cuh"
+#include "ptx.cuh"
 
 namespace capb200 {
 
@@ -25,6 +26,8 @@
 __global__ void state_gather_embed_kernel(int rows, const int* __restrict__ tokens, const int* __restrict__ src_row,
                                           const float* __restrict__ emb, long ld_emb, int E, int relu, ActView xt,
                                           int H, int nstate, StateCopy sc0, StateCopy sc1) {
+    ptx::pdl_trigger();
+    ptx::pdl_wait();
     const int r = blockIdx.x;
     if (r >= rows) return;
     const int tok = tokens[r];
@@ -35,6 +38,24 @@
         store_act(xt, r, c, v);
     }
     const int src = src_row ? src_row[r] : r;
+    if (sc0.src_hi != nullptr) {
+        for (int c4 = threadIdx.x; c4 < (H >> 2); c4 += blockDim.x) {
+            uint2 v[2][2] = {{make_uint2(0u, 0u), make_uint2(0u, 0u)}, {make_uint2(0u, 0u), make_uint2(0u, 0u)}};
+            if (src >= 0) {
+                for (int s = 0; s < nstate; ++s) {
+                    const StateCopy& sc = (s == 0) ? sc0 : sc1;
+                    v[s][0] = *reinterpret_cast<const uint2*>(sc.src_hi + (long)src * sc.ld_src + 4 * c4);
+                    v[s][1] = *reinterpret_cast<const uint2*>(sc.src_lo + (long)src * sc.ld_src + 4 * c4);
+                }
+            }
+            for (int s = 0; s < nstate; ++s) {
+                const ActView& o = (s == 0) ? sc0.dst : sc1.dst;
+                *reinterpret_cast<uint2*>(o.hi + (long)r * o.ld + 4 * c4) = v[s][0];
+                *reinterpret_cast<uint2*>(o.lo + (long)r * o.ld + 4 * c4) = v[s][1];
+            }
+        }
+        return;
+    }
     const bool vec = (H & 3) == 0 && (sc0.ld_src & 3) == 0 && (sc0.dst.ld & 3) == 0 && (nstate < 2 || ((sc1.ld_src & 3) == 0 && (sc1.dst.ld & 3) == 0));
     if (vec) {
         for (int c4 = threadIdx.x; c4 < (H >> 2); c4 += blockDim.x) {
@@ -152,6 +173,8 @@
 __global__ void __launch_bounds__(ATT_SW * 32, NA <= 16 ? 5 : 2) att_score_kernel(int rpi, int R, int A, const float* __restrict__ att_h, long ld_ah,
                                                                 const float* __restrict__ p_att, long ld_pa, const float* __restrict__ alpha_w,
                                                                 const float* __restrict__ alpha_b_ptr, float* __restrict__ score) {
+    ptx::pdl_trigger();
+    ptx::pdl_wait();
     extern __shared__ float s_ah[];
     constexpr int AP = NA * 32;
     float* s_w = s_ah + ATT_JB * AP;
@@ -235,6 +258,8 @@
 __global__ void __launch_bounds__(ATT_CT) att_combine_kernel(int rpi, int R, int H, const float* __restrict__ score, const float* __restrict__ att,
                                                              long ld_at, const float* __restrict__ mask, long ld_mask, ActView out,
                                                              float* __restrict__ alpha_out) {
+    ptx::pdl_trigger();
+    ptx::pdl_wait();
     extern __shared__ float s_w[];
     const int img = blockIdx.x;
     const int c = blockIdx.y * ATT_CT + threadIdx.x;
@@ -305,10 +330,19 @@
 }
 
 int state_gather_embed_launch(int rows, const int* tokens, const int* src_row, const float* emb, long ld_emb, int E, int relu,
-                              ActView xt, int H, int nstate, StateCopy sc0, StateCopy sc1, cudaStream_t stream) {
+                              ActView xt, int H, int nstate, StateCopy sc0, StateCopy sc1, cudaStream_t stream, bool pdl) {
     if (rows <= 0) return 0;
-    state_gather_embed_kernel<<<rows, 256, 0, stream>>>(rows, tokens, src_row, emb, ld_emb, E, relu, xt, H, nstate, sc0, sc1);
-    CAPB_CHECK_CUDA(cudaGetLastError());
+    if (sc0.src_hi != nullptr) {
+        auto aligned = [](const void* p) { return (reinterpret_cast<uintptr_t>(p) & 7) == 0; };
+        for (int s = 0; s < nstate; ++s) {
+            const StateCopy& sc = (s == 0) ? sc0 : sc1;
+            CAPB_REQUIRE(sc.src_hi != nullptr && sc.src_lo != nullptr && sc.dst.hi != nullptr && sc.dst.lo != nullptr, "state planes missing");
+            CAPB_REQUIRE((H & 3) == 0 && (sc.ld_src & 3) == 0 && (sc.dst.ld & 3) == 0 && aligned(sc.src_hi) && aligned(sc.src_lo) &&
+                         aligned(sc.dst.hi) && aligned(sc.dst.lo), "plane copies move four units at a time");
+        }
+    }
+    CAPB_CHECK_CUDA(launch_kernel(pdl, state_gather_embed_kernel, dim3(rows), dim3(256), 0, stream, rows, tokens, src_row, emb, ld_emb, E, relu, xt, H,
+                                  nstate, sc0, sc1));
     return 0;
 }
 
@@ -342,15 +376,15 @@
 
 int additive_attention_launch(int n_images, int rpi, int R, int A, int H, const float* att_h, long ld_ah, const float* p_att, long ld_pa,
                               const float* att, long ld_at, const float* mask, long ld_mask, const float* alpha_w, const float* alpha_b,
-                              float* score_scratch, ActView out, cudaStream_t stream, float* alpha_out) {
+                              float* score_scratch, ActView out, cudaStream_t stream, float* alpha_out, bool pdl) {
     if (n_images <= 0 || rpi <= 0) return 0;
     CAPB_REQUIRE(A <= 1024, "attention: att_hid_size above 1024");
     CAPB_REQUIRE(score_scratch != nullptr, "attention: score scratch missing");
     const int na = cdiv(A, 32);
     dim3 sgrid(cdiv(R, ATT_SW), n_images);
 #define CAPB_ATT_CASE(NA_)                                                                                                             \
-    att_score_kernel<NA_><<<sgrid, ATT_SW * 32, sizeof(float) * (ATT_JB + 1) * NA_ * 32, stream>>>(rpi, R, A, att_h, ld_ah, p_att, ld_pa, alpha_w, \
-                                                                                               alpha_b, score_scratch)
+    CAPB_CHECK_CUDA(launch_kernel(pdl, att_score_kernel<NA_>, sgrid, dim3(ATT_SW * 32), sizeof(float) * (ATT_JB + 1) * NA_ * 32, stream, rpi, R, A, \
+                                  att_h, ld_ah, p_att, ld_pa, alpha_w, alpha_b, score_scratch))
     if (na <= 2) CAPB_ATT_CASE(2);
     else if (na <= 4) CAPB_ATT_CASE(4);
     else if (na <= 8) CAPB_ATT_CASE(8);
@@ -361,9 +395,9 @@
     const size_t smem = sizeof(float) * (size_t)ATT_JB * R;
     CAPB_REQUIRE(smem <= 48 * 1024, "attention: too many regions");
     dim3 grid(n_images, cdiv(H, ATT_CT));
-    att_combine_kernel<<<grid, ATT_CT, smem, stream>>>(rpi, R, H, score_scratch, att, ld_at, mask, ld_mask, out, alpha_out);
-    CAPB_CHECK_CUDA(cudaGetLastError());
-    return 0;
-}
-
-}
+    CAPB_CHECK_CUDA(launch_kernel(pdl, att_combine_kernel, grid, dim3(ATT_CT), smem, stream, rpi, R, H, score_scratch, att, ld_at, mask, ld_mask, out,
+                                  alpha_out));
+    return 0;
+}
+
+}
diff --git a/imagecaptioning.pytorch_b200/csrc/ptx.cuh b/imagecaptioning.pytorch_b200/csrc/ptx.cuh
--- a/imagecaptioning.pytorch_b200/csrc/ptx.cuh
+++ b/imagecaptioning.pytorch_b200/csrc/ptx.cuh
@@ -65,6 +65,11 @@
 __device__ __forceinline__ void prefetch_tmap(const CUtensorMap* m) {
     asm volatile("prefetch.tensormap [%0];" ::"l"(reinterpret_cast<uint64_t>(m)) : "memory");
 }
+__device__ __forceinline__ void prefetch_l2(const void* p, uint32_t bytes) {
+    asm volatile("cp.async.bulk.prefetch.L2.global [%0], %1;" ::"l"(reinterpret_cast<uint64_t>(p)), "r"(bytes) : "memory");
+}
+__device__ __forceinline__ void pdl_wait() { asm volatile("griddepcontrol.wait;" ::: "memory"); }
+__device__ __forceinline__ void pdl_trigger() { asm volatile("griddepcontrol.launch_dependents;" ::: "memory"); }
 __device__ __forceinline__ void tma_load_2d(void* smem_dst, const CUtensorMap* m, uint64_t* bar, int32_t c_inner, int32_t c_outer) {
     asm volatile(
         "cp.async.bulk.tensor.2d.shared::cluster.global.mbarrier::complete_tx::bytes [%0], [%1, {%3, %4}], [%2];"
diff --git a/imagecaptioning.pytorch_b200/csrc/tfm_engine.cu b/imagecaptioning.pytorch_b200/csrc/tfm_engine.cu
--- a/imagecaptioning.pytorch_b200/csrc/tfm_engine.cu
+++ b/imagecaptioning.pytorch_b200/csrc/tfm_engine.cu
@@ -330,7 +330,7 @@
     CAPB_REQUIRE(keep == 1 || keep == beam, "sample_n must be 1 or beam_size (AttModel.py:223)");
     if (ensure_workspace(e, B, B * beam, R, beam, st)) return 1;
     if (prepare(e, att, mask, B, R, st)) return 1;
-    auto core = [&](int nrows, int live, const int* tokens, const int* , int t, float* logits, long ld) {
+    auto core = [&](int nrows, int live, const int* tokens, const int* , int t, float* logits, long ld, bool ) {
         const int* anc = (t == 0) ? nullptr : beam_ancestors(e->d.bs, t);
         return core_step(e, nrows, live, tokens, anc, nullptr, 0, t, logits, ld, R, mask, st);
     };
diff --git a/imagecaptioning.pytorch_b200/csrc/vocab.cu b/imagecaptioning.pytorch_b200/csrc/vocab.cu
--- a/imagecaptioning.pytorch_b200/csrc/vocab.cu
+++ b/imagecaptioning.pytorch_b200/csrc/vocab.cu
@@ -424,6 +424,8 @@
 }
 
 __global__ void __launch_bounds__(VT2) vocab_stats_online128_kernel(const VocabStepArgs a) {
+    ptx::pdl_trigger();
+    ptx::pdl_wait();
     __shared__ float s_red[VT2 / 32];
     __shared__ int s_idx[VT2 / 32];
     const int r = blockIdx.x;
@@ -704,7 +706,7 @@
 
 }
 
-int vocab_step_launch(const VocabStepArgs& a, cudaStream_t stream) {
+int vocab_step_launch(const VocabStepArgs& a, cudaStream_t stream, bool pdl) {
     if (a.rows <= 0) return 0;
     CAPB_REQUIRE(a.topk <= 16, "beam size up to 16");
     if (a.stats != nullptr) {
@@ -714,7 +716,7 @@
         static const char* variant = getenv("CAPB200_VOCAB_STATS");
         const char vsel = variant ? variant[0] : 'o';
         if (vec && vsel == 'o' && !(variant && variant[1] == '2')) {
-            vocab_stats_online128_kernel<<<a.rows, VT2, 0, stream>>>(a);
+            CAPB_CHECK_CUDA(launch_kernel(pdl, vocab_stats_online128_kernel, dim3(a.rows), dim3(VT2), 0, stream, a));
         } else if (vec && vsel == 'o') {
             vocab_stats_online_kernel<<<a.rows, VT, 0, stream>>>(a);
         } else if (vec && vsel == 's' && stream_smem <= 100 * 1024) {
```

New measurement: 24340 (median of 6 runs). 1.4% higher.
